# felipeagc/sycl-ray-tracer

Measured on AMD Instinct MI355X. Metric: Mrays/s, higher is better.
Workload: dtype f32

## Files before the change

### sycl-ray-tracer_amd/csrc/rt_abi.hip

```cpp
#include "bvh_quantise.h"
#include "rt_internal.h"

namespace rtlib {
thread_local std::string g_err;

int copy_out(const rt_renderer* r, int rc, float* rgba_f32, uint8_t* rgba_u8) {
    if (rc != RT_OK) return rc;
    if (rgba_f32 && r->n_local) HIPCHK(hipMemcpy(rgba_f32, r->d_f32, (size_t)r->n_local * 16, hipMemcpyDeviceToHost));
    if (rgba_u8 && r->n_local) HIPCHK(hipMemcpy(rgba_u8, r->d_u8, (size_t)r->n_local * 4, hipMemcpyDeviceToHost));
    return RT_OK;
}
}

extern "C" {

const char* rt_last_error(void) { return g_err.c_str(); }
int rt_abi_version(void) { return RT_ABI_VERSION; }

int rt_device_count(void) {
    int n = 0;
    hipError_t e = hipGetDeviceCount(&n);
    if (e != hipSuccess) return fail(RT_ERR_NO_DEVICE, std::string("hipGetDeviceCount: ") + hipGetErrorString(e));
    return n;
}

int rt_camera_init(rt_camera* out, int32_t width, int32_t height, const float center[3], const float dir_in[3],
                   float focal_length) {
    if (!out || !center || !dir_in || width <= 0 || height <= 0) return fail(RT_ERR_INVALID, "bad camera arguments");
    auto norm = [](const float v[3], float o[3]) {
        float inv = 1.0f / std::sqrt((v[0] * v[0] + v[1] * v[1]) + v[2] * v[2]);
        o[0] = v[0] * inv, o[1] = v[1] * inv, o[2] = v[2] * inv;
    };
    auto cross = [](const float a[3], const float b[3], float o[3]) {
        o[0] = a[1] * b[2] - a[2] * b[1], o[1] = a[2] * b[0] - a[0] * b[2], o[2] = a[0] * b[1] - a[1] * b[0];
    };
    float dir[3], right[3], up[3], tmp[3];
    const float world_up[3] = {0.0f, 1.0f, 0.0f};
    norm(dir_in, dir);
    cross(dir, world_up, tmp), norm(tmp, right);
    cross(right, dir, tmp), norm(tmp, up);
    const float vp0 = 1.0f * ((float)width / (float)height), vp1 = 1.0f;
    const float du_div = (float)width / (vp0 * 2.0f), dv_div = (float)height / (vp1 * 2.0f);
    for (int a = 0; a < 3; ++a) {
        const float viewport_u = (-right[a]) * vp0, viewport_v = up[a] * vp1;
        out->center[a] = center[a];
        out->pixel00[a] = ((center[a] + viewport_u) + viewport_v) + dir[a] * focal_length;
        out->delta_u[a] = right[a] / du_div;
        out->delta_v[a] = (-up[a]) / dv_div;
    }
    out->width = width, out->height = height;
    return RT_OK;
}

int rt_scene_create(const rt_scene_desc* desc, int device, int bvh_kind, rt_scene** out) { return rt_scene_create_ex(desc, device, bvh_kind, 0u, out); }

int rt_scene_create_ex(const rt_scene_desc* desc, int device, int bvh_kind, uint32_t flags, rt_scene** out) {
    if (!out) return fail(RT_ERR_INVALID, "null output pointer");
    *out = nullptr;
    if (flags & ~(RT_SCENE_UPDATABLE | RT_SCENE_KEEP_PREVIOUS)) return fail(RT_ERR_INVALID, "unknown scene flags");
    if ((flags & RT_SCENE_KEEP_PREVIOUS) && !(flags & RT_SCENE_UPDATABLE)) return fail(RT_ERR_INVALID, "RT_SCENE_KEEP_PREVIOUS is a flag of updatable scenes: pass RT_SCENE_UPDATABLE with it");
    if (bvh_kind != RT_BVH_DEFAULT && bvh_kind != RT_BVH_LBVH && bvh_kind != RT_BVH_SAH && bvh_kind != RT_BVH_LBVH_GPU)
        return fail(RT_ERR_INVALID, "unknown bvh_kind");
    if (bvh_kind == RT_BVH_LBVH_GPU) {
        if (device < 0) return fail(RT_ERR_NO_DEVICE, "RT_BVH_LBVH_GPU needs a device (device >= 0)");
        int rc0 = device_ok(device);
        if (rc0 != RT_OK) return rc0;
    }
    rt_scene* s = new (std::nothrow) rt_scene();
    if (!s) return fail(RT_ERR_OOM, "host allocation failed");
    std::string err;
    int rc = RT_OK;
    try {
        rc = build_host_scene(desc, bvh_kind, s->hs, err);
    } catch (const std::bad_alloc&) {
        delete s;
        return fail(RT_ERR_OOM, "host allocation failed while building the scene");
    } catch (const std::exception& e) {
        delete s;
        return fail(RT_ERR_INVALID, std::string("scene build failed: ") + e.what());
    }
    if (rc != RT_OK) {
        delete s;
        return fail(rc, err);
    }
    s->device = device;
    if (device >= 0) {
        rc = device_ok(device);
        if (rc == RT_OK) {
            if (s->hs.nodes.size() > (size_t)(0x7FFFFFFF / 64)) {
                rt_scene_destroy(s);
                return fail(RT_ERR_INVALID, "BVH too large for 32-bit node offsets");
            }
            std::vector<BvhNode> dn(s->hs.nodes);
            for (BvhNode& n : dn)
                for (int k = 0; k < 4; ++k)
                    if (n.child[k] >= 0) n.child[k] *= 64;
            rc = upload(dn, &s->dev.nodes, s->device_bytes);
        }
        if (rc == RT_OK) {
            std::vector<uint8_t> packed(s->hs.tris.size() * (size_t)kTriBytes + 48, 0);
            for (size_t i = 0; i < s->hs.tris.size(); ++i) std::memcpy(packed.data() + i * kTriBytes, &s->hs.tris[i], std::min<size_t>(kTriBytes, sizeof(TriRec)));
            rc = upload(packed, &s->dev.tris, s->device_bytes);
        }
        if (rc == RT_OK) rc = upload(s->hs.shade, &s->dev.shade, s->device_bytes);
        if (rc == RT_OK) {
            std::vector<InstRec> rows(s->hs.inst);
            if (flags & RT_SCENE_UPDATABLE) rows.resize(std::max<size_t>(rows.size(), desc->n_instances));
            rc = upload(rows, &s->dev.inst, s->device_bytes);
        }
        if (rc == RT_OK) rc = upload(s->hs.mats, &s->dev.mats, s->device_bytes);
        if (rc == RT_OK) rc = upload(s->hs.tex, &s->dev.tex, s->device_bytes);
        if (rc == RT_OK && hipMalloc((void**)&s->d_query_cursor, kQueryCursorBytes) != hipSuccess)
            rc = fail(RT_ERR_OOM, "device allocation failed (the ray-query cursors)");
        if (rc != RT_OK) {
            rt_scene_destroy(s);
            return rc;
        }
        s->dev.n_nodes = (uint32_t)s->hs.nodes.size();
        s->dev.n_tris = (uint32_t)(s->hs.wverts.size() / 9);
        std::memcpy(s->dev.sky, s->hs.sky, 12);
        s->dev.packed_mat = s->hs.packed_mat ? 1u : 0u;
        const bool stage = s->hs.packed_mat && s->hs.n_layers <= 65536u;
        s->dev.lds_nm = stage ? (uint32_t)std::min<size_t>(s->hs.inst.size(), kLdsNm) : 0u;
        s->dev.lds_mats = stage ? (uint32_t)std::min<size_t>(s->hs.mats.size(), kLdsMats) : 0u;
        scene_cells(s->hs, s->dev);
    }
    if (flags & RT_SCENE_UPDATABLE) {
        rc = no_throw([&] { return init_scene_update(s, desc, (flags & RT_SCENE_KEEP_PREVIOUS) != 0); });
        if (rc != RT_OK) {
            rt_scene_destroy(s);
            return rc;
        }
    }
    *out = s;
    return RT_OK;
}

void rt_scene_destroy(rt_scene* s) {
    if (!s) return;
    if (s->device >= 0 && hipSetDevice(s->device) == hipSuccess) {
        for (auto& se : s->ev_gbuffer) (void)hipEventSynchronize(se.second), (void)hipEventDestroy(se.second);
        (void)hipFree((void*)s->dev.nodes), (void)hipFree((void*)s->dev.tris), (void)hipFree((void*)s->dev.shade);
        (void)hipFree((void*)s->dev.inst), (void)hipFree((void*)s->dev.mats), (void)hipFree((void*)s->dev.tex);
        (void)hipFree((void*)s->d_query_cursor);
    }
    free_scene_update(s);
    delete s;
}

int rt_scene_info(const rt_scene* s, rt_scene_info_t* out) {
    if (!s || !out) return fail(RT_ERR_INVALID, "null argument");
    if (const int rc = sync_host_copy(s)) return rc;
    out->n_triangles = (uint32_t)(s->hs.wverts.size() / 9);
    out->n_nodes = (uint32_t)s->hs.nodes.size();
    out->max_depth = s->hs.max_depth;
    out->max_leaf_tris = s->hs.max_leaf_tris;
    std::memcpy(out->bounds_lo, s->hs.bounds_lo, 12), std::memcpy(out->bounds_hi, s->hs.bounds_hi, 12);
    out->sah_cost = s->hs.sah_cost;
    out->device_bytes = s->device_bytes;
    out->n_leaf_records = (uint32_t)s->hs.tris.size();
    out->n_split_triangles = s->hs.n_split_triangles;
    return RT_OK;
}

int rt_scene_check_bvh(const rt_scene* s) {
    if (!s) return fail(RT_ERR_INVALID, "null scene");
    if (const int rc0 = sync_host_copy(s)) return rc0;
    std::string err;
    int rc = check_bvh(s->hs, err);
    return rc == RT_OK ? RT_OK : fail(rc, err);
}

int rt_scene_count_visits(const rt_scene* s, uint32_t n, const float* org, const float* dir, int mode, uint64_t* node_visits, uint64_t* tri_tests,
                          float* t, uint32_t* tri) {
    if (!s || (n && (!org || !dir))) return fail(RT_ERR_INVALID, "null argument");
    if (const int rc0 = sync_host_copy(s)) return rc0;
    std::string err;
    const int rc = no_throw([&] { return count_visits(s->hs, n, org, dir, mode, node_visits, tri_tests, t, tri, err); });
    return rc == RT_OK ? RT_OK : fail(rc, err.empty() ? g_err : err);
}

int rt_renderer_create(int kind, rt_scene* scene, int32_t width, int32_t height, uint32_t max_depth,
                       uint32_t sample_count, uint32_t seed_mode, rt_renderer** out) {
    if (!out) return fail(RT_ERR_INVALID, "null output pointer");
    *out = nullptr;
    if (!scene) return fail(RT_ERR_INVALID, "null scene");
    if (kind != RT_RENDERER_MEGAKERNEL && kind != RT_RENDERER_WAVEFRONT) return fail(RT_ERR_INVALID, "unknown renderer kind");
    if (width <= 0 || height <= 0 || (int64_t)width * height > (int64_t)1 << 30) return fail(RT_ERR_INVALID, "bad image size");
    if (sample_count == 0) return fail(RT_ERR_INVALID, "sample_count must be >= 1");
    if (seed_mode > RT_SEED_MEGAKERNEL) return fail(RT_ERR_INVALID, "unknown seed mode");
    if ((uint64_t)sample_count * ((uint64_t)max_depth + 1) > (1ull << 26)) return fail(RT_ERR_INVALID, "sample_count * max_depth too large");
    if (scene->device < 0) return fail(RT_ERR_NO_DEVICE, "scene was built host-only (device < 0)");
    int rc = device_ok(scene->device);
    if (rc != RT_OK) return rc;
    rt_renderer* r = new (std::nothrow) rt_renderer();
    if (!r) return fail(RT_ERR_OOM, "host allocation failed");
    r->kind = kind, r->scene = scene, r->width = width, r->height = height;
    r->scene_gen = scene->generation;
    r->max_depth = max_depth, r->spp = sample_count;
    r->seed_mode = seed_mode != RT_SEED_DEFAULT ? seed_mode
                   : (kind == RT_RENDERER_MEGAKERNEL ? RT_SEED_MEGAKERNEL : RT_SEED_WAVEFRONT);
    r->hw_queues = hw_queues_from_env();
    const char* prof = std::getenv("RT_PROFILE_KERNELS");
    r->profile_kernels = prof && prof[0] == '1';
    if (const char* e = dev_knob("RT_MEGA_LDS_PAD")) r->mega_lds_pad = (uint32_t)std::max(0, std::min(100 * 1024, std::atoi(e)));
    if (const char* e = dev_knob("RT_MEGA_OCC")) r->mega_occ = (uint32_t)std::max(1, std::min((int)kMegaWaves, std::atoi(e)));
    auto bail = [&](int code) {
        rt_renderer_destroy(r);
        return code;
    };
    {
        hipStream_t s0 = nullptr;
        bool owned = false;
        if (lane_stream_of(scene->device, 0, &s0, &owned) != hipSuccess) return bail(fail(RT_ERR_HIP, "cannot create the stream-lane pool"));
    }
    hipDeviceProp_t prop;
    if (hipGetDeviceProperties(&prop, scene->device) == hipSuccess && prop.multiProcessorCount > 0) r->n_cus = prop.multiProcessorCount;
    if (hipStreamCreateWithFlags(&r->stream, hipStreamNonBlocking) != hipSuccess) return bail(fail(RT_ERR_HIP, "hipStreamCreate failed"));
    if (hipEventCreate(&r->ev_begin) != hipSuccess || hipEventCreate(&r->ev_end) != hipSuccess ||
        hipEventCreateWithFlags(&r->ev_fork, hipEventDisableTiming) != hipSuccess || hipEventCreateWithFlags(&r->ev_tile_read, hipEventDisableTiming) != hipSuccess)
        return bail(fail(RT_ERR_HIP, "hipEventCreate failed"));
    if (hipMalloc((void**)&r->d_frame, sizeof(MegaFrame)) != hipSuccess || hipHostMalloc((void**)&r->h_frame, sizeof(MegaFrame)) != hipSuccess)
        return bail(fail(RT_ERR_OOM, "frame constant buffer allocation failed"));
    if (kind == RT_RENDERER_WAVEFRONT) {
        if (hipMalloc((void**)&r->d_cam, sizeof(CameraDev)) != hipSuccess || hipHostMalloc((void**)&r->h_cam, sizeof(CameraDev)) != hipSuccess)
            return bail(fail(RT_ERR_OOM, "camera buffer allocation failed"));
        rt_schedule& sc = r->sched;
        if (const char* e = dev_knob("RT_WF_GRAPH")) sc.hip_graph = e[0] == '1';
        if (const char* e = dev_knob("RT_WF_FINISH_DEPTH")) sc.finish_depth = (uint32_t)std::max(0, std::atoi(e));
        if (const char* e = dev_knob("RT_WF_SAMPLES_PER_LAUNCH")) sc.samples_per_launch = (uint32_t)std::max(0, std::atoi(e));
        if (const char* e = dev_knob("RT_WF_REQUEUE")) sc.requeue = e[0] != '0' ? 1 : 0;
        if (const char* e = dev_knob("RT_WF_STREAMS")) sc.stream_lanes = (uint32_t)std::max(1, std::min(8, std::atoi(e)));
        if ((dev_knob("RT_WF_REQUEUE") || dev_knob("RT_WF_STREAMS")) && sc.samples_per_launch == 0) sc.samples_per_launch = 1;
        if (const char* e = dev_knob("RT_WF_LPT")) sc.cost_order = e[0] == '0' ? 0 : (e[0] == '2' ? 1 : -1);
        if (const char* e = dev_knob("RT_WF_EXTEND_OCC")) r->wf_extend_occ = (uint32_t)std::max(1, std::min((int)kExtendWaves, std::atoi(e)));
        if (const char* e = dev_knob("RT_WF_FINISH_OCC")) r->wf_finish_occ = (uint32_t)std::max(1, std::min((int)kMegaWaves, std::atoi(e)));
        if (const char* e = dev_knob("RT_WF_SHOOT_CHUNK")) r->wf_shoot_chunk = (uint32_t)std::max(16, std::min(1024, std::atoi(e)));
        if (const char* e = dev_knob("RT_WF_SHOOT_TAIL")) r->wf_shoot_tail = e[0] == '1';
        if (const char* e = dev_knob("RT_WF_SHOOT_STATIC_PCT")) r->wf_shoot_static_pct = (uint32_t)std::max(0, std::min(100, std::atoi(e)));
        if (const char* e = dev_knob("RT_WF_REORDER")) sc.reorder = e[0] == '1';
        if (const char* e = dev_knob("RT_WF_MATSORT")) sc.matsort = e[0] == '1';
        if (const char* e = dev_knob("RT_WF_FUSED_BOUNCE")) sc.fused_bounce = e[0] == '1';
    }
    rc = no_throw([&] { return alloc_tile_buffers(r); });
    if (rc != RT_OK) return bail(rc);
    *out = r;
    return RT_OK;
}

void rt_renderer_destroy(rt_renderer* r) {
    if (!r) return;
    if (r->scene && r->frame_pending && r->scene->frames_pending) r->scene->frames_pending--;
    if (r->scene && hipSetDevice(r->scene->device) == hipSuccess) {
        drain_streams(r, r->pending.stream);
        free_tile_buffers(r);
        if (r->d_cam) (void)hipFree(r->d_cam);
        if (r->h_cam) (void)hipHostFree(r->h_cam);
        if (r->d_frame) (void)hipFree(r->d_frame);
        if (r->h_frame) (void)hipHostFree(r->h_frame);
        for (hipEvent_t e : r->ev_pool) (void)hipEventDestroy(e);
        if (r->ev_begin) (void)hipEventDestroy(r->ev_begin);
        if (r->ev_end) (void)hipEventDestroy(r->ev_end);
        if (r->ev_fork) (void)hipEventDestroy(r->ev_fork);
        if (r->ev_tile_read) (void)hipEventDestroy(r->ev_tile_read);
        if (r->stream) (void)hipStreamDestroy(r->stream);
    }
    delete r;
}

int rt_renderer_set_tile(rt_renderer* r, uint32_t rank, uint32_t world, uint32_t strip_rows) {
    if (!r) return fail(RT_ERR_INVALID, "null renderer");
    if (world == 0 || rank >= world || strip_rows == 0) return fail(RT_ERR_INVALID, "bad tile split");
    if (r->frame_pending) return fail(RT_ERR_INVALID, "a frame is in flight (rt_render_frame_end first)");
    HIPCHK(hipSetDevice(r->scene->device));
    drain_streams(r, r->pending.stream);
    const TileDev old = r->tile;
    r->tile.rank = rank, r->tile.world = world, r->tile.strip_rows = strip_rows;
    const int rc = no_throw([&] { return alloc_tile_buffers(r); });
    if (rc != RT_OK) r->tile.rank = old.rank, r->tile.world = old.world, r->tile.strip_rows = old.strip_rows;
    return rc;
}

int32_t rt_renderer_local_rows(const rt_renderer* r) { return r ? r->tile.local_rows : 0; }

int32_t rt_renderer_global_row(const rt_renderer* r, int32_t local_row) {
    if (!r || local_row < 0 || local_row >= r->tile.local_rows) return -1;
    const uint32_t strip = (uint32_t)local_row / r->tile.strip_rows, within = (uint32_t)local_row % r->tile.strip_rows;
    return (int32_t)((strip * r->tile.world + r->tile.rank) * r->tile.strip_rows + within);
}

int rt_renderer_set_profiling(rt_renderer* r, int enable) {
    if (!r) return fail(RT_ERR_INVALID, "null renderer");
    r->profile_kernels = enable != 0;
    return RT_OK;
}

int rt_renderer_set_russian_roulette(rt_renderer* r, uint32_t start_bounce) {
// ... 35 lines not shown
    const rt_schedule old = r->sched;
    r->sched = *s;
    const int rc = no_throw([&] { return alloc_tile_buffers(r); });
    if (rc != RT_OK) r->sched = old;
    return rc;
}

int rt_render_frame(rt_renderer* r, const rt_camera* cam, float* rgba_f32, uint8_t* rgba_u8, rt_stats* stats) {
    if (!r) return fail(RT_ERR_INVALID, "null renderer");
    return copy_out(r, no_throw([&] { return render_impl(r, cam, rgba_f32 ? r->d_f32 : nullptr, rgba_u8 ? r->d_u8 : nullptr, r->stream, stats); }), rgba_f32, rgba_u8);
}

int rt_render_frame_device(rt_renderer* r, const rt_camera* cam, void* d_rgba_f32, void* d_rgba_u8, void* stream,
                           rt_stats* stats) {
    if (!r) return fail(RT_ERR_INVALID, "null renderer");
    return no_throw([&] { return render_impl(r, cam, (float*)d_rgba_f32, (uint8_t*)d_rgba_u8, stream ? (hipStream_t)stream : r->stream, stats); });
}

int rt_renderer_set_progressive(rt_renderer* r, int enable) {
    if (!r) return fail(RT_ERR_INVALID, "null renderer");
    if (r->frame_pending) return fail(RT_ERR_INVALID, "a frame is in flight (rt_render_frame_end first)");
    HIPCHK(hipSetDevice(r->scene->device));
    drop_graph(r);
    r->progressive = enable != 0;
    const int rc = no_throw([&] { return alloc_carry(r); });
    if (rc != RT_OK) r->progressive = false;
    return rc;
}

int rt_render_frame_continue(rt_renderer* r, uint32_t samples, float* rgba_f32, uint8_t* rgba_u8, rt_stats* stats) {
    if (!r) return fail(RT_ERR_INVALID, "null renderer");
    return copy_out(r, no_throw([&] { return continue_impl(r, samples, rgba_f32 ? r->d_f32 : nullptr, rgba_u8 ? r->d_u8 : nullptr, r->stream, stats); }), rgba_f32, rgba_u8);
}

int rt_render_frame_continue_device(rt_renderer* r, uint32_t samples, void* d_rgba_f32, void* d_rgba_u8, void* stream, rt_stats* stats) {
    if (!r) return fail(RT_ERR_INVALID, "null renderer");
    return no_throw([&] { return continue_impl(r, samples, (float*)d_rgba_f32, (uint8_t*)d_rgba_u8, stream ? (hipStream_t)stream : r->stream, stats); });
}

int rt_renderer_accumulated_samples(const rt_renderer* r, uint32_t* out) {
    if (!r || !out) return fail(RT_ERR_INVALID, "null argument");
    *out = carry_is_current(r) ? r->carry_samples : 0u;
    return RT_OK;
}

int rt_renderer_block_grid(const rt_renderer* r, uint32_t* blocks_x, uint32_t* blocks_y) {
    if (!r || !blocks_x || !blocks_y) return fail(RT_ERR_INVALID, "null argument");
    *blocks_x = ((uint32_t)r->width + 7u) / 8u, *blocks_y = ((uint32_t)r->tile.local_rows + 7u) / 8u;
    return RT_OK;
}

int rt_renderer_block_samples(const rt_renderer* r, uint32_t* out) {
    if (!r || !out) return fail(RT_ERR_INVALID, "null argument");
    const size_t nb = (size_t)(((uint32_t)r->width + 7u) / 8u) * (((uint32_t)r->tile.local_rows + 7u) / 8u);
    if (r->carry_samples == 0 || !carry_is_current(r) || r->h_block_count.size() != nb) std::memset(out, 0, nb * 4);
    else std::memcpy(out, r->h_block_count.data(), nb * 4);
    return RT_OK;
}

int rt_renderer_block_errors(const rt_renderer* r, float* out) {
    if (!r || !out) return fail(RT_ERR_INVALID, "null argument");
    return no_throw([&] { return block_errors(r, out); });
}

int rt_render_frame_continue_blocks(rt_renderer* r, uint32_t samples, const uint32_t* blocks, uint32_t n_blocks, float* rgba_f32, uint8_t* rgba_u8,
                                    rt_stats* stats) {
    if (!r) return fail(RT_ERR_INVALID, "null renderer");
    return copy_out(r, no_throw([&] { return continue_blocks_impl(r, samples, blocks, n_blocks, rgba_f32 ? r->d_f32 : nullptr, rgba_u8 ? r->d_u8 : nullptr, r->stream, stats); }), rgba_f32, rgba_u8);
}

int rt_render_frame_continue_blocks_device(rt_renderer* r, uint32_t samples, const uint32_t* blocks, uint32_t n_blocks, void* d_rgba_f32, void* d_rgba_u8,
                                           void* stream, rt_stats* stats) {
    if (!r) return fail(RT_ERR_INVALID, "null renderer");
    return no_throw([&] {
        return continue_blocks_impl(r, samples, blocks, n_blocks, (float*)d_rgba_f32, (uint8_t*)d_rgba_u8, stream ? (hipStream_t)stream : r->stream, stats);
    });
}

int rt_renderer_adapt(rt_renderer* r, float threshold, uint32_t min_samples, uint32_t* blocks_out, uint32_t* n_out) {
    if (!r || !n_out) return fail(RT_ERR_INVALID, "null argument");
    return no_throw([&]() -> int {
        std::vector<uint32_t> blocks;
        const int rc = adapt_impl(r, threshold, min_samples, blocks);
        if (rc != RT_OK) return rc;
        if (!blocks.empty() && !blocks_out) return fail(RT_ERR_INVALID, "null block list");
        if (!blocks.empty()) std::memcpy(blocks_out, blocks.data(), blocks.size() * 4);
        *n_out = (uint32_t)blocks.size();
        return (int)RT_OK;
    });
}

int rt_render_frame_continue_adaptive(rt_renderer* r, uint32_t samples, float threshold, uint32_t min_samples, float* rgba_f32, uint8_t* rgba_u8,
                                      rt_stats* stats, uint32_t* n_blocks_out) {
    if (!r) return fail(RT_ERR_INVALID, "null renderer");
    return copy_out(r, no_throw([&] {
        return continue_adaptive_impl(r, samples, threshold, min_samples, rgba_f32 ? r->d_f32 : nullptr, rgba_u8 ? r->d_u8 : nullptr, r->stream, stats,
                                      n_blocks_out);
    }), rgba_f32, rgba_u8);
}

int rt_render_frame_continue_adaptive_device(rt_renderer* r, uint32_t samples, float threshold, uint32_t min_samples, void* d_rgba_f32, void* d_rgba_u8,
                                             void* stream, rt_stats* stats, uint32_t* n_blocks_out) {
    if (!r) return fail(RT_ERR_INVALID, "null renderer");
    return no_throw([&] {
        return continue_adaptive_impl(r, samples, threshold, min_samples, (float*)d_rgba_f32, (uint8_t*)d_rgba_u8, stream ? (hipStream_t)stream : r->stream,
                                      stats, n_blocks_out);
    });
}

int rt_render_frame_begin(rt_renderer* r, const rt_camera* cam, void* d_rgba_f32, void* d_rgba_u8, void* stream) {
    if (!r) return fail(RT_ERR_INVALID, "null renderer");
    return no_throw([&] { return frame_begin(r, cam, (float*)d_rgba_f32, (uint8_t*)d_rgba_u8, stream ? (hipStream_t)stream : r->stream); });
}

int rt_render_frame_end(rt_renderer* r, rt_stats* stats) {
    if (!r) return fail(RT_ERR_INVALID, "null renderer");
    return no_throw([&] { return frame_end(r, stats); });
}

}

#ifdef RT_DEVELOPER_KNOBS
extern "C" {

int rt_dev_scene_tables(const rt_scene* s, uint32_t* packed_mat, uint32_t* lds_nm, uint32_t* lds_mats, uint32_t* n_rows, float* rows,
                        uint32_t capacity, uint32_t* words) {
    if (!s || !packed_mat || !lds_nm || !lds_mats || !n_rows) return fail(RT_ERR_INVALID, "null argument");
    if (const int rc = sync_host_copy(s)) return rc;
    *packed_mat = s->hs.packed_mat ? 1u : 0u;
    *lds_nm = s->dev.lds_nm, *lds_mats = s->dev.lds_mats;
    *n_rows = (uint32_t)s->hs.inst.size();
    if (rows)
        for (size_t k = 0; k < std::min<size_t>(capacity, s->hs.inst.size()); ++k) std::memcpy(rows + 9 * k, s->hs.inst[k].normal_mat, 36);
    if (words)
        for (size_t t = 0; t < s->hs.shade.size(); ++t) words[t] = s->hs.shade[t].instance;
    return RT_OK;
}

int rt_dev_scene_tree(const rt_scene* s, uint32_t* n_nodes, uint32_t* n_tris, uint32_t* n_wverts, uint32_t* stack_need, int32_t* built_by,
                      float* pad, float* bounds, void* nodes, uint32_t* global_index, float* wverts, uint32_t capacity) {
    if (!s || !n_nodes || !n_tris || !n_wverts || !stack_need || !built_by || !pad || !bounds) return fail(RT_ERR_INVALID, "null argument");
    if (const int rc = sync_host_copy(s)) return rc;
    const HostScene& hs = s->hs;
    *n_nodes = (uint32_t)hs.nodes.size(), *n_tris = (uint32_t)hs.tris.size(), *n_wverts = (uint32_t)hs.wverts.size();
    *stack_need = hs.stack_need, *built_by = hs.built_by, *pad = hs.pad;
    for (int a = 0; a < 3; ++a) bounds[a] = hs.bounds_lo[a], bounds[3 + a] = hs.bounds_hi[a];
    if (nodes) std::memcpy(nodes, hs.nodes.data(), std::min<size_t>(capacity, hs.nodes.size()) * sizeof(BvhNode));
    if (global_index)
        for (size_t t = 0; t < std::min<size_t>(capacity, hs.tris.size()); ++t) global_index[t] = hs.tris[t].global_index;
    if (wverts) std::memcpy(wverts, hs.wverts.data(), std::min<size_t>(capacity, hs.wverts.size()) * sizeof(float));
    return RT_OK;
}

int rt_dev_renderer_graph_captures(const rt_renderer* r, uint32_t* out) {
    if (!r || !out) return fail(RT_ERR_INVALID, "null argument");
    *out = r->graph_captures;
    return RT_OK;
}

int rt_dev_quantise_node(uint32_t count, const int32_t* nk, const float* klo, const float* khi, void* nodes_out, uint8_t* ok) {
    if (!nk || !klo || !khi || !nodes_out || !ok) return fail(RT_ERR_INVALID, "null argument");
    BvhNode* out = static_cast<BvhNode*>(nodes_out);
    for (uint32_t i = 0; i < count; ++i) {
        if (nk[i] < 1 || nk[i] > 4) return fail(RT_ERR_INVALID, "nk must be 1..4");
        Box3 kb[4];
        for (int k = 0; k < 4; ++k) std::memcpy(kb[k].lo, klo + 12 * (size_t)i + 3 * k, 12), std::memcpy(kb[k].hi, khi + 12 * (size_t)i + 3 * k, 12);
        out[i] = empty_node();
        ok[i] = quantise_node(out[i], nk[i], kb, 0.0f) ? 1 : 0;
    }
    return RT_OK;
}

}
#endif
```

### sycl-ray-tracer_amd/csrc/rt_bounce.h

```cpp
#pragma once
#include "rt_device.h"

namespace rt {

RT_DEV f3 ray_dir(const RayState& r) { return mk3(h2f(r.dir[0]), h2f(r.dir[1]), h2f(r.dir[2])); }

template <bool FROM_TRAV = false, class Sink = NoSink>
RT_DEV bool shade_bounce(const SceneDev& S, uint32_t& rng, RayState& r, const Hit& h, f3& result, const Trav* T = nullptr, const ShadeTables* tab = nullptr,
                         long long* ck = nullptr, const Sink& sink = Sink{}) {
    f3 org = FROM_TRAV ? T->o : r.org;
    f3 dir = FROM_TRAV ? T->d : ray_dir(r);
    f3 att = mk3(h2f(r.att[0]), h2f(r.att[1]), h2f(r.att[2]));
    f3 rad = mk3(h2f(r.rad[0]), h2f(r.rad[1]), h2f(r.rad[2]));
    const bool done = FROM_TRAV ? shade_hit<true>(S, *tab, rng, h, org, dir, att, rad, result, ck, sink) : shade_hit<false>(S, ShadeTables{}, rng, h, org, dir, att, rad, result, nullptr, sink);
    r.org = org;
    r.dir[0] = f2h(dir.x), r.dir[1] = f2h(dir.y), r.dir[2] = f2h(dir.z);
    r.att[0] = f2h(att.x), r.att[1] = f2h(att.y), r.att[2] = f2h(att.z);
    r.rad[0] = f2h(rad.x), r.rad[1] = f2h(rad.y), r.rad[2] = f2h(rad.z);
    return done;
}

RT_DEV bool roulette(uint32_t& rng, RayState& r) {
    const float qx = h2f(r.att[0]), qy = h2f(r.att[1]), qz = h2f(r.att[2]);
    const float p = __builtin_fminf(__builtin_fmaxf(__builtin_fmaxf(qx, __builtin_fmaxf(qy, qz)), 0.05f), 1.0f);
    const float u = rng_next(rng);
    if (!(u < p)) return false;
    r.att[0] = f2h(qx / p), r.att[1] = f2h(qy / p), r.att[2] = f2h(qz / p);
    return true;
}

}
```

### sycl-ray-tracer_amd/csrc/rt_device.h

```cpp
#pragma once
#include <hip/hip_runtime.h>

#include "../../include/rt_mi355x.h"
#include "rt_types.h"

namespace rt {

#define RT_DEV __device__ __forceinline__

struct f3 {
    float x, y, z;
};
RT_DEV f3 mk3(float x, float y, float z) { return f3{x, y, z}; }
RT_DEV f3 operator+(f3 a, f3 b) { return mk3(a.x + b.x, a.y + b.y, a.z + b.z); }
RT_DEV f3 operator-(f3 a, f3 b) { return mk3(a.x - b.x, a.y - b.y, a.z - b.z); }
RT_DEV f3 operator-(f3 a) { return mk3(-a.x, -a.y, -a.z); }
RT_DEV f3 operator*(f3 a, f3 b) { return mk3(a.x * b.x, a.y * b.y, a.z * b.z); }
RT_DEV f3 operator*(float s, f3 a) { return mk3(s * a.x, s * a.y, s * a.z); }
RT_DEV f3 operator*(f3 a, float s) { return mk3(a.x * s, a.y * s, a.z * s); }
RT_DEV float dot3(f3 a, f3 b) { return (a.x * b.x + a.y * b.y) + a.z * b.z; }
RT_DEV f3 cross3(f3 a, f3 b) {
    return mk3(a.y * b.z - a.z * b.y, a.z * b.x - a.x * b.z, a.x * b.y - a.y * b.x);
}
RT_DEV float rcp_rn(float x) {
// ... 16 lines not shown
        const float y = __builtin_amdgcn_rcpf(s);
        return __builtin_fmaf(__builtin_fmaf(-s, y, 1.0f), y, y);
    }
    return 1.0f / __builtin_sqrtf(x);
}
RT_DEV f3 normalize3(f3 a) {
    const float inv = inv_sqrt2(dot3(a, a));
    return mk3(a.x * inv, a.y * inv, a.z * inv);
}
RT_DEV float clamp01(float x) { return __builtin_fminf(__builtin_fmaxf(x, 0.0f), 1.0f); }

RT_DEV uint16_t f2h(float f) {
    asm("" : "+v"(f));
    _Float16 h = (_Float16)f;
    return __builtin_bit_cast(uint16_t, h);
}
RT_DEV float h2f(uint16_t b) { return (float)__builtin_bit_cast(_Float16, b); }

RT_DEV float rng_next(uint32_t& a) {
    uint32_t x = a;
    x ^= x << 13;
    x ^= x >> 17;
    x ^= x << 5;
    a = x;
    return (float)x * (1.0f / 4294967296.0f);
}
RT_DEV float rng_range(uint32_t& a, float mn, float mx) { return mn + (mx - mn) * rng_next(a); }
RT_DEV f3 rng_unit_vector(uint32_t& a) {
    float x = rng_range(a, -1.0f, 1.0f);
    float y = rng_range(a, -1.0f, 1.0f);
    float z = rng_range(a, -1.0f, 1.0f);
    return normalize3(mk3(x, y, z));
}

RT_DEV uint32_t pixel_seed(int x, int y, int w, int h, uint32_t seed_mode) {
    if (seed_mode == RT_SEED_MEGAKERNEL) {
        uint32_t h8 = (uint32_t)((h + 7) / 8) * 8u;
        return (uint32_t)x * h8 + (uint32_t)y;
    }
    return (uint32_t)x + (uint32_t)y * (uint32_t)w;
}

RT_DEV int tile_global_row(const TileDev& t, int local_row) {
    uint32_t strip = (uint32_t)local_row / t.strip_rows;
    uint32_t within = (uint32_t)local_row % t.strip_rows;
    return (int)((strip * t.world + t.rank) * t.strip_rows + within);
}

struct RayState {
    f3 org;
    uint16_t dir[3], att[3], rad[3];
};

RT_DEV RayState camera_ray(const CameraDev& c, int x, int y, uint32_t& rng) {
    f3 p00 = mk3(c.pixel00[0], c.pixel00[1], c.pixel00[2]);
    f3 du = mk3(c.du[0], c.du[1], c.du[2]);
    f3 dv = mk3(c.dv[0], c.dv[1], c.dv[2]);
    f3 center = mk3(c.center[0], c.center[1], c.center[2]);
    f3 pixel_center = (p00 + ((float)x * du)) + ((float)y * dv);
    float px = -0.5f + rng_next(rng);
    float py = -0.5f + rng_next(rng);
    f3 jitter = (px * du) + (py * dv);
    f3 pixel_sample = pixel_center + jitter;
    f3 d = pixel_sample - center;
    RayState r;
    r.org = center;
    r.dir[0] = f2h(d.x), r.dir[1] = f2h(d.y), r.dir[2] = f2h(d.z);
    r.att[0] = r.att[1] = r.att[2] = 0x3C00;
    r.rad[0] = r.rad[1] = r.rad[2] = 0;
    return r;
}

struct Hit {
    float t, u, v;
    uint32_t tri;
};

RT_DEV float dot3f(f3 a, f3 b) { return __builtin_fmaf(a.z, b.z, __builtin_fmaf(a.y, b.y, a.x * b.x)); }
RT_DEV f3 cross3f(f3 a, f3 b) {
    return mk3(__builtin_fmaf(a.y, b.z, -(a.z * b.y)), __builtin_fmaf(a.z, b.x, -(a.x * b.z)), __builtin_fmaf(a.x, b.y, -(a.y * b.x)));
}
RT_DEV void tri_test_regs(float4 a, float4 b, float2 c, f3 o, f3 d, Hit& best) {
    const f3 v0 = mk3(a.x, a.y, a.z), e1 = mk3(a.w, b.x, b.y), e2 = mk3(b.z, b.w, c.x);
    const uint32_t gidx = __float_as_uint(c.y);
    const f3 p = cross3f(d, e2);
    const float det = dot3f(e1, p);
    if (!(det != 0.0f)) return;
    const f3 tv = o - v0;
    const f3 q = cross3f(tv, e1);
    const float sgn = det < 0.0f ? -1.0f : 1.0f;
    const float un0 = dot3f(tv, p), vn0 = dot3f(d, q);
    const float un = un0 * sgn, vn = vn0 * sgn;
    if (!(un >= 0.0f && vn >= 0.0f && un + vn <= __builtin_fabsf(det))) return;
    const float inv = rcp_rn(det);
    const float t = dot3f(e2, q) * inv;
    if (!(t > kTNear)) return;
    if (t < best.t || (t == best.t && gidx < best.tri)) {
        best.t = t;
        best.u = un0 * inv;
        best.v = vn0 * inv;
        best.tri = gidx;
    }
}
typedef float f4a8 __attribute__((ext_vector_type(4), aligned(8)));
typedef float f2a8 __attribute__((ext_vector_type(2), aligned(8)));
RT_DEV float4 tri_ld4(const uint8_t* p) {
    const f4a8 v = *reinterpret_cast<const f4a8*>(p);
    return make_float4(v.x, v.y, v.z, v.w);
}
RT_DEV float2 tri_ld2(const uint8_t* p) {
    const f2a8 v = *reinterpret_cast<const f2a8*>(p);
    return make_float2(v.x, v.y);
}
RT_DEV void tri_test(const uint8_t* __restrict__ tr, f3 o, f3 d, Hit& best) {
    tri_test_regs(tri_ld4(tr), tri_ld4(tr + 16), tri_ld2(tr + 32), o, d, best);
}

constexpr int32_t kTravDone = (int32_t)0x80000000;
struct Trav {
    f3 o, d;
    float ix, iy, iz;
    float ox, oy, oz;
    Hit best;
    int32_t cur;
    uint32_t sp;
};

struct TravStack;
RT_DEV uint32_t stack_base(const TravStack& st);
RT_DEV void trav_begin(Trav& T, f3 o, f3 d, const TravStack& st) {
    T.o = o, T.d = d;
    T.best.t = __builtin_huge_valf();
    T.best.u = T.best.v = 0.0f;
    T.best.tri = kNoTri;
    const float kTiny = 1e-30f;
    const float dx = __builtin_fabsf(d.x) < kTiny ? __builtin_copysignf(kTiny, d.x) : d.x;
    const float dy = __builtin_fabsf(d.y) < kTiny ? __builtin_copysignf(kTiny, d.y) : d.y;
    const float dz = __builtin_fabsf(d.z) < kTiny ? __builtin_copysignf(kTiny, d.z) : d.z;
    T.ix = __builtin_amdgcn_rcpf(dx), T.iy = __builtin_amdgcn_rcpf(dy), T.iz = __builtin_amdgcn_rcpf(dz);
    T.ox = -o.x * T.ix, T.oy = -o.y * T.iy, T.oz = -o.z * T.iz;
    T.cur = 0;
    T.sp = stack_base(st);
}

constexpr int kLdsStack = 12;
typedef __attribute__((address_space(3))) int32_t lds_i32;
struct TravStack {
    uint32_t base;
    int32_t* spill;
    uint32_t pitch;
};
RT_DEV uint32_t stack_base(const TravStack& st) { return st.base + st.pitch; }
RT_DEV lds_i32* lds_at(uint32_t addr) { return (lds_i32*)(size_t)addr; }
RT_DEV bool stack_shallow(const TravStack& st, const Trav& T, uint32_t pushes) { return T.sp <= st.base + ((uint32_t)kLdsStack - pushes) * st.pitch; }
RT_DEV void trav_pop_lds(Trav& T, const TravStack& st) {
    T.sp -= st.pitch;
    T.cur = *lds_at(T.sp);
}
RT_DEV void stk_push(const TravStack& st, Trav& T, int32_t v) {
    const uint32_t e = (T.sp - st.base) / st.pitch;
    if (e < (uint32_t)kLdsStack) *lds_at(T.sp) = v;
    else st.spill[e - (uint32_t)kLdsStack] = v;
    T.sp += st.pitch;
}
RT_DEV void trav_pop(Trav& T, const TravStack& st) {
    T.sp -= st.pitch;
    const uint32_t e = (T.sp - st.base) / st.pitch;
    T.cur = e < (uint32_t)kLdsStack ? *lds_at(T.sp) : st.spill[e - (uint32_t)kLdsStack];
}

typedef uint32_t u32x4 __attribute__((ext_vector_type(4)));
typedef uint32_t u32x2 __attribute__((ext_vector_type(2)));
typedef __attribute__((address_space(3))) u32x4 lds_u32x4;
struct TopTree {
    lds_u32x4* w0;
    lds_u32x4* w1;
    lds_u32x4* w2;
    lds_u32x4* ch;
    int32_t count;
};
RT_DEV void top_tree_fill(const SceneDev& S, u32x4* w0, u32x4* w1, u32x4* w2, u32x4* ch, int32_t count) {
    for (int32_t i = (int32_t)threadIdx.x; i < count; i += (int32_t)blockDim.x) {
        const u32x4* np = reinterpret_cast<const u32x4*>(S.nodes + i);
        w0[i] = np[0];
        w1[i] = np[1];
        w2[i] = np[2];
        ch[i] = np[3];
    }
}

typedef unsigned long long lmask;
RT_DEV lmask lanes(bool c) { return __builtin_amdgcn_ballot_w64(c); }
RT_DEV uint32_t lane_rank(lmask m) { return __builtin_amdgcn_mbcnt_hi((uint32_t)(m >> 32), __builtin_amdgcn_mbcnt_lo((uint32_t)m, 0u)); }
RT_DEV float sel(lmask m, float a, float b) {
    float d;
    asm("v_cndmask_b32_e64 %0, %1, %2, %3" : "=v"(d) : "v"(a), "v"(b), "s"(m));
    return d;
}
RT_DEV uint32_t sel(lmask m, uint32_t a, uint32_t b) {
    uint32_t d;
    asm("v_cndmask_b32_e64 %0, %1, %2, %3" : "=v"(d) : "v"(a), "v"(b), "s"(m));
    return d;
}
RT_DEV int32_t sel(lmask m, int32_t a, int32_t b) { return (int32_t)sel(m, (uint32_t)a, (uint32_t)b); }

struct TravSigns {
    lmask nx, ny, nz;
};

RT_DEV float ub0(uint32_t w) { return (float)(w & 0xffu); }
RT_DEV float ub1(uint32_t w) { return (float)((w >> 8) & 0xffu); }
RT_DEV float ub2(uint32_t w) { return (float)((w >> 16) & 0xffu); }
RT_DEV float ub3(uint32_t w) { return (float)(w >> 24); }

struct WaveStats {
    uint32_t inner_steps = 0, inner_lanes = 0, leaf_steps = 0, leaf_lanes = 0;
    uint32_t shade_rounds = 0, shade_lanes = 0, live_lane_steps = 0, top_lanes = 0;
};
RT_DEV TravSigns trav_signs(const Trav& T) { return TravSigns{lanes(T.ix < 0.0f), lanes(T.iy < 0.0f), lanes(T.iz < 0.0f)}; }
RT_DEV void trav_inner(const SceneDev& S, Trav& T, const TravStack& stack, const TopTree& top, const TravSigns& sg) {
    const float inf = __builtin_huge_valf();
    float k0, k1, k2, k3;
    u32x4 w0, w1, w2, chw;
    if (T.cur < top.count * 64) {
        const uint32_t o = (uint32_t)T.cur >> 2;
        w0 = *(lds_u32x4*)(size_t)((uint32_t)(size_t)top.w0 + o), w1 = *(lds_u32x4*)(size_t)((uint32_t)(size_t)top.w1 + o);
        w2 = *(lds_u32x4*)(size_t)((uint32_t)(size_t)top.w2 + o), chw = *(lds_u32x4*)(size_t)((uint32_t)(size_t)top.ch + o);
    } else {
        asm volatile("global_load_dwordx4 %0, %4, %5\n\t"
                     "global_load_dwordx4 %1, %4, %5 offset:16\n\t"
                     "global_load_dwordx4 %2, %4, %5 offset:32\n\t"
                     "global_load_dwordx4 %3, %4, %5 offset:48"
                     : "=&v"(w0), "=&v"(w1), "=&v"(w2), "=&v"(chw)
                     : "v"((uint32_t)T.cur), "s"(S.nodes)
                     : "memory");
    }
    asm volatile("s_waitcnt vmcnt(1)" : "+v"(w0), "+v"(w1), "+v"(w2));
    const float ax = __uint_as_float(w0.w) * T.ix;
    const float ay = __uint_as_float(w2.z) * T.iy;
    const float az = __uint_as_float(w2.w) * T.iz;
    const float bx = __builtin_fmaf(__uint_as_float(w0.x), T.ix, T.ox);
    const float by = __builtin_fmaf(__uint_as_float(w0.y), T.iy, T.oy);
    const float bz = __builtin_fmaf(__uint_as_float(w0.z), T.iz, T.oz);
    const lmask nx = sg.nx, ny = sg.ny, nz = sg.nz;
    const uint32_t qnx = sel(nx, w1.x, w1.y), qfx = sel(nx, w1.y, w1.x);
    const uint32_t qny = sel(ny, w1.z, w1.w), qfy = sel(ny, w1.w, w1.z);
    const uint32_t qnz = sel(nz, w2.x, w2.y), qfz = sel(nz, w2.y, w2.x);
#define RT_CHILD(K, CVT)                                                                                  \
    {                                                                                                    \
        const float tn = __builtin_fmaxf(__builtin_fmaxf(__builtin_fmaf(CVT(qnx), ax, bx), __builtin_fmaf(CVT(qny), ay, by)), \
                                         __builtin_fmaxf(__builtin_fmaf(CVT(qnz), az, bz), 0.0f));       \
        const float tf = __builtin_fminf(__builtin_fminf(__builtin_fmaf(CVT(qfx), ax, bx), __builtin_fmaf(CVT(qfy), ay, by)), \
                                         __builtin_fminf(__builtin_fmaf(CVT(qfz), az, bz), T.best.t));   \
        K = sel(lanes(tn <= tf), inf, tn);                                                               \
    }
    RT_CHILD(k0, ub0)
    RT_CHILD(k1, ub1)
    RT_CHILD(k2, ub2)
    RT_CHILD(k3, ub3)
#undef RT_CHILD
#define RT_CE(KA, CA, KB, CB)                                                        \
    {                                                                               \
        const lmask sw = lanes(KB < KA);                                            \
        const float ka = sel(sw, KA, KB), kb = sel(sw, KB, KA);                     \
        const int32_t ca = sel(sw, CA, CB), cb = sel(sw, CB, CA);                   \
        KA = ka, KB = kb, CA = ca, CB = cb;                                         \
    }
    asm volatile("s_waitcnt vmcnt(0)" : "+v"(chw));
    int32_t c0 = (int32_t)chw.x, c1 = (int32_t)chw.y, c2 = (int32_t)chw.z, c3 = (int32_t)chw.w;
    RT_CE(k0, c0, k1, c1)
    RT_CE(k2, c2, k3, c3)
    RT_CE(k0, c0, k2, c2)
#undef RT_CE
    const bool descend = k0 < inf;
    if (lanes(!stack_shallow(stack, T, 3u)) == 0ull) {
        *lds_at(T.sp) = c3;
        T.sp = sel(lanes(k3 < inf), T.sp, T.sp + stack.pitch);
        *lds_at(T.sp) = c2;
        T.sp = sel(lanes(k2 < inf), T.sp, T.sp + stack.pitch);
        *lds_at(T.sp) = c1;
        T.sp = sel(lanes(k1 < inf), T.sp, T.sp + stack.pitch);
        if (descend) T.cur = c0;
        else trav_pop_lds(T, stack);
    } else {
        if (k3 < inf) stk_push(stack, T, c3);
        if (k2 < inf) stk_push(stack, T, c2);
        if (k1 < inf) stk_push(stack, T, c1);
        if (descend) T.cur = c0;
        else trav_pop(T, stack);
    }
}

template <bool BATCH>
RT_DEV void trav_leaf(const SceneDev& S, Trav& T, const TravStack& stack) {
    const uint32_t code = (uint32_t)~T.cur;
    const uint32_t first = code >> 2, rem = code & 3u;
    if (BATCH) {
        static_assert(kMaxLeafTris == 2 && kTriBytes == 40, "the whole-leaf step reads a leaf as 80 contiguous bytes");
        const uint8_t* p4 = S.tris + (size_t)first * kTriBytes;
        const float4 l0 = tri_ld4(p4), l1 = tri_ld4(p4 + 16), l2 = tri_ld4(p4 + 32), l3 = tri_ld4(p4 + 48), l4 = tri_ld4(p4 + 64);
        const bool two = rem != 0u;
        tri_test_regs(l0, l1, make_float2(l2.x, l2.y), T.o, T.d, T.best);
        if (__ballot(two) != 0ull) {
            if (two) tri_test_regs(make_float4(l2.z, l2.w, l3.x, l3.y), make_float4(l3.z, l3.w, l4.x, l4.y), make_float2(l4.z, l4.w), T.o, T.d, T.best);
        }
        if (lanes(!stack_shallow(stack, T, 0u)) == 0ull) trav_pop_lds(T, stack);
        else trav_pop(T, stack);
    } else {
        tri_test(S.tris + (size_t)first * kTriBytes, T.o, T.d, T.best);
        if (rem) T.cur = ~(int32_t)(((first + 1u) << 2) | (rem - 1u));
        else trav_pop(T, stack);
    }
}

template <bool STATS = false, bool LEAF_BATCH = false>
RT_DEV uint32_t trav_step_wave(const SceneDev& S, Trav& T, const TravStack& stack, const TopTree& top, const TravSigns& sg, WaveStats* ws = nullptr) {
    const bool inner = T.cur >= 0;
    const bool leaf = T.cur < 0 && T.cur != kTravDone;
    const uint32_t ni = (uint32_t)__popcll(__ballot(inner)), nl = (uint32_t)__popcll(__ballot(leaf));
    if (ni * 3u >= nl * 4u && !(LEAF_BATCH && nl >= 64u)) {
        if (STATS && ni) ws->inner_steps++, ws->inner_lanes += ni, ws->top_lanes += (uint32_t)__popcll(__ballot(inner && T.cur < kTopNodes * 64));
        if (inner) trav_inner(S, T, stack, top, sg);
    } else {
        if (STATS) ws->leaf_steps++, ws->leaf_lanes += (uint32_t)__popcll(__ballot(leaf));
        if (leaf) trav_leaf<LEAF_BATCH>(S, T, stack);
    }
    return ni + nl;
}

RT_DEV Hit intersect(const SceneDev& S, f3 o, f3 d, const TravStack& stack, const TopTree& top) {
    Trav T;
    trav_begin(T, o, d, stack);
    const TravSigns sg = trav_signs(T);
    while (trav_step_wave(S, T, stack, top, sg)) {}
    return T.best;
}

RT_DEV bool near_zero3(f3 e) {
    const float s = 1e-8f;
    return (__builtin_fabsf(e.x) < s) && (__builtin_fabsf(e.y) < s) && (__builtin_fabsf(e.z) < s);
}
RT_DEV float length_squared3(f3 v) {
    float l = __builtin_sqrtf(dot3(v, v));
    return l * l;
}
RT_DEV f3 reflect3(f3 v, f3 n) { return v - (2.0f * dot3(v, n)) * n; }
RT_DEV f3 refract3(f3 uv, f3 n, float etai_over_etat) {
    float cos_theta = __builtin_fminf(dot3(-uv, n), 1.0f);
    f3 r_out_perp = etai_over_etat * (uv + cos_theta * n);
    f3 r_out_parallel = (-__builtin_sqrtf(__builtin_fabsf(1.0f - length_squared3(r_out_perp)))) * n;
    return r_out_perp + r_out_parallel;
}
RT_DEV float schlick(float cosine, float ref_idx) {
    float r0 = (1.0f - ref_idx) / (1.0f + ref_idx);
    r0 = r0 * r0;
    float x = 1.0f - cosine;
    float x2 = x * x;
    float x5 = (x2 * x2) * x;
    return r0 + (1.0f - r0) * x5;
}
RT_DEV float unorm8_to_float(uint32_t b) {
    const float x = (float)b, r = 1.0f / 255.0f;
    const float q = x * r;
    return __builtin_fmaf(__builtin_fmaf(-q, 255.0f, x), r, q);
}

RT_DEV bool albedo_is_texture(const MatRec& m) { return (m.type == RT_MAT_DIFFUSE || m.type == RT_MAT_METALLIC) && m.tex_kind != RT_TEX_COLOR; }
RT_DEV uint32_t albedo_fetch(const SceneDev& S, const MatRec& m, float u, float v) {
    float fu = u - __builtin_floorf(u);
    float fv = v - __builtin_floorf(v);
    int iu = (int)__builtin_floorf(fu * 512.0f);
    int iv = (int)__builtin_floorf(fv * 512.0f);
    iu = iu < 0 ? 0 : (iu > 511 ? 511 : iu);
    iv = iv < 0 ? 0 : (iv > 511 ? 511 : iv);
    return *reinterpret_cast<const uint32_t*>(S.tex + (((size_t)m.tex_layer * 512u + (size_t)iv) * 512u + (size_t)iu) * 4u);
}
RT_DEV f3 albedo_decode(uint32_t texel) {
    return mk3(unorm8_to_float(texel & 0xffu), unorm8_to_float((texel >> 8) & 0xffu), unorm8_to_float((texel >> 16) & 0xffu));
}
RT_DEV f3 albedo(const SceneDev& S, const MatRec& m, float u, float v) {
    if (m.tex_kind == RT_TEX_COLOR) return mk3(m.color[0], m.color[1], m.color[2]);
    float fu = u - __builtin_floorf(u);
    float fv = v - __builtin_floorf(v);
    int iu = (int)__builtin_floorf(fu * 512.0f);
    int iv = (int)__builtin_floorf(fv * 512.0f);
    iu = iu < 0 ? 0 : (iu > 511 ? 511 : iu);
    iv = iv < 0 ? 0 : (iv > 511 ? 511 : iv);
    const uint32_t texel = *reinterpret_cast<const uint32_t*>(
        S.tex + (((size_t)m.tex_layer * 512u + (size_t)iv) * 512u + (size_t)iu) * 4u);
    return mk3(unorm8_to_float(texel & 0xffu), unorm8_to_float((texel >> 8) & 0xffu), unorm8_to_float((texel >> 16) & 0xffu));
}

template <bool PRE = false>
RT_DEV bool scatter(const SceneDev& S, const MatRec& m, uint32_t& rng, f3 dir, f3 normal, float u, float v,
                    f3& out_dir, f3& out_att, uint32_t texel = 0) {
    if (m.type == RT_MAT_DIFFUSE || m.type == RT_MAT_METALLIC) {
        const bool diffuse = m.type == RT_MAT_DIFFUSE;
        const f3 unit = rng_unit_vector(rng);
        const f3 reflected = reflect3(dir, normal);
        const f3 base = diffuse ? normal : reflected;
        const f3 offs = diffuse ? unit : m.roughness * unit;
        out_dir = base + offs;
        if (diffuse && near_zero3(dir)) out_dir = normal;
        if (PRE) out_att = m.tex_kind == RT_TEX_COLOR ? mk3(m.color[0], m.color[1], m.color[2]) : albedo_decode(texel);
        else out_att = albedo(S, m, u, v);
        return diffuse ? true : dot3(out_dir, normal) > 0.0f;
    }
    if (m.type == RT_MAT_DIELECTRIC) {
        out_att = mk3(1.0f, 1.0f, 1.0f);
        bool front_face = dot3(dir, normal) < 0.0f;
        f3 n = front_face ? normal : -normal;
        float ratio = front_face ? (1.0f / m.ior) : m.ior;
        f3 unit_direction = normalize3(dir);
        float cos_theta = __builtin_fminf(dot3(-unit_direction, n), 1.0f);
        float sin_theta = __builtin_sqrtf(1.0f - cos_theta * cos_theta);
        bool reflect_it = ratio * sin_theta > 1.0f;
        if (!reflect_it) reflect_it = schlick(cos_theta, ratio) > rng_range(rng, 0.0f, 1.0f);
        out_dir = reflect_it ? reflect3(unit_direction, n) : refract3(unit_direction, n, ratio);
        return true;
    }
    out_dir = mk3(0.0f, 0.0f, 0.0f);
    out_att = mk3(0.0f, 0.0f, 0.0f);
    return false;
}

struct ShadeTables {
    lds_u32x4* nm;
    lds_u32x4* mat;
    uint32_t n_nm, n_mat;
};
RT_DEV void shade_tables_fill(const SceneDev& S, u32x4* nm, u32x4* mat) {
    const u32x4* in = reinterpret_cast<const u32x4*>(S.inst);
    for (uint32_t i = threadIdx.x; i < S.lds_nm * 3u; i += blockDim.x) nm[i] = in[i];
    for (uint32_t i = threadIdx.x; i < S.lds_mats; i += blockDim.x) {
        const u32x4* mp = reinterpret_cast<const u32x4*>(S.mats + i);
        const u32x4 m0 = mp[0], m1 = mp[1], m2 = mp[2];
        u32x4 a, b;
        a.x = m0.x | (m0.y << 8) | (m1.y << 16), a.y = m0.z, a.z = m0.w, a.w = m1.x;
        b.x = m1.z, b.y = m1.w, b.z = m2.x, b.w = m0.x == RT_MAT_DIELECTRIC ? m2.z : m2.y;
        mat[2u * i] = a, mat[2u * i + 1u] = b;
    }
}

#ifdef RT_ROUND_STAMPS
#define RT_STAMP_AFTER(ck, i, VAL)                                                     \
    do {                                                                              \
        if (ck) {                                                                     \
            asm volatile("" ::"v"(VAL));                                              \
            const long long n_ = (long long)__builtin_readcyclecounter();             \
            (ck)[i] += n_ - (ck)[7];                                                  \
            (ck)[7] = n_;                                                             \
        }                                                                             \
    } while (0)
#else
#define RT_STAMP_AFTER(ck, i, VAL) do { } while (0)
#endif
struct NoSink {};
template <class Sink> struct is_no_sink { static constexpr bool value = false; };
template <> struct is_no_sink<NoSink> { static constexpr bool value = true; };
template <bool USE_TAB = false, class Sink = NoSink>
RT_DEV bool shade_hit(const SceneDev& S, const ShadeTables& tab, uint32_t& rng, const Hit& h, f3& org, f3& dir, f3& att, f3& rad, f3& result,
                      long long* ck = nullptr, const Sink& sink = Sink{}) {
    if (h.tri == kNoTri) {
        if constexpr (is_no_sink<Sink>::value) result = att * (mk3(S.sky[0], S.sky[1], S.sky[2]) + rad);
        else sink(att * (mk3(S.sky[0], S.sky[1], S.sky[2]) + rad));
        return true;
    }
    const float4* sp = reinterpret_cast<const float4*>(S.shade + h.tri);
    const float4 s0 = sp[0], s1 = sp[1], s2 = sp[2], s3 = sp[3];
    const f3 d = normalize3(dir);
    const f3 n0 = mk3(s0.x, s0.y, s0.z), n1 = mk3(s0.w, s1.x, s1.y), n2 = mk3(s1.z, s1.w, s2.x);
    const float uv0x = s2.y, uv0y = s2.z, uv1x = s2.w, uv1y = s3.x, uv2x = s3.y, uv2y = s3.z;
    const uint32_t iw = __float_as_uint(s3.w);
    RT_STAMP_AFTER(ck, 1, iw);
    bool lds = false;
    if (USE_TAB) lds = __builtin_amdgcn_ballot_w64(!((iw & kPackedInstMask) < tab.n_nm && (iw >> kPackedInstBits) < tab.n_mat)) == 0ull;
    MatRec mat;
    if (USE_TAB && __builtin_expect(lds, 1)) {
        const uint32_t at = (iw >> kPackedInstBits) * 2u;
        const u32x4 a = tab.mat[at], b = tab.mat[at + 1u];
        mat.type = a.x & 0xffu, mat.tex_kind = (a.x >> 8) & 0xffu, mat.tex_layer = a.x >> 16;
        mat.color[0] = __uint_as_float(a.y), mat.color[1] = __uint_as_float(a.z), mat.color[2] = __uint_as_float(a.w);
        mat.emissive[0] = __uint_as_float(b.x), mat.emissive[1] = __uint_as_float(b.y), mat.emissive[2] = __uint_as_float(b.z);
        mat.roughness = mat.ior = __uint_as_float(b.w);
    } else {
        const InstRec* inst = S.inst + (S.packed_mat ? (iw & kPackedInstMask) : iw);
        const u32x4* mp = reinterpret_cast<const u32x4*>(S.mats + (S.packed_mat ? (iw >> kPackedInstBits) : inst->material));
        const u32x4 m0 = mp[0], m1 = mp[1], m2 = mp[2];
        mat.type = m0.x, mat.tex_kind = m0.y, mat.color[0] = __uint_as_float(m0.z), mat.color[1] = __uint_as_float(m0.w);
        mat.color[2] = __uint_as_float(m1.x), mat.tex_layer = m1.y, mat.emissive[0] = __uint_as_float(m1.z), mat.emissive[1] = __uint_as_float(m1.w);
        mat.emissive[2] = __uint_as_float(m2.x), mat.roughness = __uint_as_float(m2.y), mat.ior = __uint_as_float(m2.z);
    }
    const float bx = h.u, by = h.v;
    const float w = (1.0f - bx) - by;
    const float tu = (w * uv0x + bx * uv1x) + by * uv2x;
    const float tv = (w * uv0y + bx * uv1y) + by * uv2y;
    uint32_t texel;
    {
        float fu = tu - __builtin_floorf(tu);
        float fv = tv - __builtin_floorf(tv);
        int iu = (int)__builtin_floorf(fu * 512.0f);
        int iv = (int)__builtin_floorf(fv * 512.0f);
        iu = iu < 0 ? 0 : (iu > 511 ? 511 : iu);
        iv = iv < 0 ? 0 : (iv > 511 ? 511 : iv);
        const uint8_t* ta = S.tex + (((size_t)mat.tex_layer * 512u + (size_t)iv) * 512u + (size_t)iu) * 4u;
        if (!albedo_is_texture(mat)) ta = reinterpret_cast<const uint8_t*>(sp);
        texel = *reinterpret_cast<const uint32_t*>(ta);
        RT_STAMP_AFTER(ck, 2, ta);
    }
    const bool emits = mat.type == RT_MAT_DIFFUSE || mat.type == RT_MAT_METALLIC;
    rad = rad + (emits ? mk3(mat.emissive[0], mat.emissive[1], mat.emissive[2]) : mk3(0.0f, 0.0f, 0.0f));
    const f3 vn = normalize3((w * n0 + bx * n1) + by * n2);
    float nm[9];
    if (USE_TAB && __builtin_expect(lds, 1)) {
        const uint32_t at = (iw & kPackedInstMask) * 3u;
        const u32x4 a = tab.nm[at], b = tab.nm[at + 1u];
        const uint32_t c = *reinterpret_cast<__attribute__((address_space(3))) const uint32_t*>(tab.nm + at + 2u);
        nm[0] = __uint_as_float(a.x), nm[1] = __uint_as_float(a.y), nm[2] = __uint_as_float(a.z), nm[3] = __uint_as_float(a.w);
        nm[4] = __uint_as_float(b.x), nm[5] = __uint_as_float(b.y), nm[6] = __uint_as_float(b.z), nm[7] = __uint_as_float(b.w);
        nm[8] = __uint_as_float(c);
    } else {
        const InstRec* inst = S.inst + (S.packed_mat ? (iw & kPackedInstMask) : iw);
        u32x4 a, b;
        uint32_t c;
        asm volatile("global_load_dwordx4 %0, %3, off\n\t"
                     "global_load_dwordx4 %1, %3, off offset:16\n\t"
                     "global_load_dword %2, %3, off offset:32\n\t"
                     "s_waitcnt vmcnt(0)"
                     : "=&v"(a), "=&v"(b), "=&v"(c)
                     : "v"(inst)
                     : "memory");
        nm[0] = __uint_as_float(a.x), nm[1] = __uint_as_float(a.y), nm[2] = __uint_as_float(a.z), nm[3] = __uint_as_float(a.w);
        nm[4] = __uint_as_float(b.x), nm[5] = __uint_as_float(b.y), nm[6] = __uint_as_float(b.z), nm[7] = __uint_as_float(b.w);
        nm[8] = __uint_as_float(c);
    }
    const f3 g = mk3((nm[0] * vn.x + nm[3] * vn.y) + nm[6] * vn.z, (nm[1] * vn.x + nm[4] * vn.y) + nm[7] * vn.z,
                     (nm[2] * vn.x + nm[5] * vn.y) + nm[8] * vn.z);
    const f3 normal = normalize3(g);
    RT_STAMP_AFTER(ck, 3, normal.x);
    f3 sdir, satt;
#ifdef RT_SCATTER_PRIO
    __builtin_amdgcn_s_setprio(RT_SCATTER_PRIO);
#endif
    const bool scattered = scatter<true>(S, mat, rng, d, normal, tu, tv, sdir, satt, texel);
    RT_STAMP_AFTER(ck, 4, satt.x);
    if (scattered) {
        org = mk3(org.x + dir.x * h.t, org.y + dir.y * h.t, org.z + dir.z * h.t);
        dir = sdir;
        att = att * satt;
        return false;
    }
    if constexpr (is_no_sink<Sink>::value) result = att * rad;
    else sink(att * rad);
    return true;
}

RT_DEV uint8_t to_unorm8(float c) { return (uint8_t)__builtin_rintf(clamp01(c) * 255.0f); }

#define RT_TRAVERSAL_LDS(BLOCK)                                                                        \
    __shared__ u32x4 top_all[4 * kTopNodes];  \
    u32x4 *const top_w0 = top_all, *const top_w1 = top_all + kTopNodes, *const top_w2 = top_all + 2 * kTopNodes, *const top_ch = top_all + 3 * kTopNodes; \
    __shared__ int32_t lds_stack[kLdsStack * (BLOCK)];                                                 \
    int32_t spill[kStackSize - kLdsStack];                                                             \
    const int32_t top_count = (int32_t)S.n_nodes < kTopNodes ? (int32_t)S.n_nodes : kTopNodes;         \
    top_tree_fill(S, top_w0, top_w1, top_w2, top_ch, top_count);                                       \
    __syncthreads();                                                                                   \
    const TopTree top{(lds_u32x4*)top_w0, (lds_u32x4*)top_w1, (lds_u32x4*)top_w2, (lds_u32x4*)top_ch, top_count}; \
    const TravStack stack{(uint32_t)(size_t)(lds_i32*)(lds_stack + threadIdx.x), spill, 4u * (BLOCK)}; \
    lds_stack[threadIdx.x] = kTravDone;

#define RT_SHADE_LDS                                                                                   \
    __shared__ u32x4 shade_nm[3 * kLdsNm], shade_mat[2 * kLdsMats];                                    \
    shade_tables_fill(S, shade_nm, shade_mat);                                                         \
    const ShadeTables tab{(lds_u32x4*)shade_nm, (lds_u32x4*)shade_mat, S.lds_nm, S.lds_mats};


}
```

### sycl-ray-tracer_amd/csrc/rt_kernels.h

```cpp
#pragma once
#include <cstddef>

#include "rt_bounce.h"
#include "rt_device.h"
#include "rt_launch.h"

namespace rt {

RT_DEV void queue_store(const QueueDev& q, uint32_t slot, uint32_t id, const RayState& r) {
    q.org_id[slot] = make_float4(r.org.x, r.org.y, r.org.z, __uint_as_float(id));
    q.a[slot] = make_uint2((uint32_t)r.dir[0] | ((uint32_t)r.dir[1] << 16), (uint32_t)r.dir[2] | ((uint32_t)r.att[0] << 16));
    q.b[slot] = make_uint2((uint32_t)r.att[1] | ((uint32_t)r.att[2] << 16), (uint32_t)r.rad[0] | ((uint32_t)r.rad[1] << 16));
    q.c[slot] = r.rad[2];
}
RT_DEV uint32_t queue_load(const QueueDev& q, uint32_t slot, RayState& r) {
    const float4 o = q.org_id[slot];
    const uint2 a = q.a[slot], b = q.b[slot];
    const uint16_t c = q.c[slot];
    r.org = mk3(o.x, o.y, o.z);
    r.dir[0] = (uint16_t)a.x, r.dir[1] = (uint16_t)(a.x >> 16), r.dir[2] = (uint16_t)a.y;
    r.att[0] = (uint16_t)(a.y >> 16), r.att[1] = (uint16_t)b.x, r.att[2] = (uint16_t)(b.x >> 16);
    r.rad[0] = (uint16_t)b.y, r.rad[1] = (uint16_t)(b.y >> 16), r.rad[2] = c;
    return __float_as_uint(o.w);
}
// ... 29 lines not shown
#endif
constexpr int kMegaUnroll = 3;
#ifndef RT_MEGA_SHADE_PCT
#define RT_MEGA_SHADE_PCT 75
#endif
constexpr uint32_t kMegaShadePct = RT_MEGA_SHADE_PCT;
constexpr uint32_t kMegaRefill = 1;
struct RefillPolicy {
    uint32_t w = (kMegaRefill - 1u) << 28;
    RT_DEV uint32_t threshold() const { return (w >> 28) + 1u; }
    RT_DEV void stepped() {
        if (((w >> 17) & 0x7FFu) != 0x7FFu) w += 1u << 17;
    }
    RT_DEV void round(bool finished) {
        w += ((uint32_t)__popcll(__ballot(finished)) << 5) + 1u;
        if ((w & 31u) == 0u) {
            const uint32_t ended = ((w >> 5) & 0xFFFu) - 1u, steps = ((w >> 17) & 0x7FFu) * kMegaUnroll;
            const uint32_t num = 320u * ended, den = 160u + steps;
            const uint32_t t = num < 4u * den ? 1u : num < 9u * den ? 2u : num < 16u * den ? 3u : num < 25u * den ? 4u : num < 36u * den ? 5u
                               : num < 64u * den ? 6u : num < 100u * den ? 8u : num < 144u * den ? 10u : num < 256u * den ? 12u : 16u;
            w = (t - 1u) << 28;
        }
    }
};
template <uint32_t OFF> RT_DEV uint32_t frame_u32(const MegaFrame* f) {
    uint32_t v;
    asm volatile("s_load_dword %0, %1, %2\n\t"
                 "s_waitcnt lgkmcnt(0)"
                 : "=&s"(v)
                 : "s"(f), "i"(OFF));
    return v;
}
template <uint32_t OFF> RT_DEV unsigned long long frame_u64(const MegaFrame* f) {
    unsigned long long v;
    asm volatile("s_load_dwordx2 %0, %1, %2\n\t"
                 "s_waitcnt lgkmcnt(0)"
                 : "=&s"(v)
                 : "s"(f), "i"(OFF));
    return v;
}
RT_DEV CameraDev frame_camera(const MegaFrame* f, int32_t width, int32_t height) {
    static_assert(offsetof(MegaFrame, cam) == 0 && offsetof(CameraDev, dv) + sizeof(CameraDev::dv) == 48, "the camera's twelve floats lead MegaFrame");
    u32x4 a, b, c;
    asm volatile("s_load_dwordx4 %0, %3, 0x0\n\t"
                 "s_load_dwordx4 %1, %3, 0x10\n\t"
                 "s_load_dwordx4 %2, %3, 0x20\n\t"
                 "s_waitcnt lgkmcnt(0)"
                 : "=&s"(a), "=&s"(b), "=&s"(c)
                 : "s"(f));
    CameraDev cam;
    cam.center[0] = __uint_as_float(a.x), cam.center[1] = __uint_as_float(a.y), cam.center[2] = __uint_as_float(a.z);
    cam.pixel00[0] = __uint_as_float(a.w), cam.pixel00[1] = __uint_as_float(b.x), cam.pixel00[2] = __uint_as_float(b.y);
    cam.du[0] = __uint_as_float(b.z), cam.du[1] = __uint_as_float(b.w), cam.du[2] = __uint_as_float(c.x);
    cam.dv[0] = __uint_as_float(c.y), cam.dv[1] = __uint_as_float(c.z), cam.dv[2] = __uint_as_float(c.w);
    cam.width = width, cam.height = height;
    return cam;
}
RT_DEV CameraDev frame_camera_and_seed(const MegaFrame* f, int32_t width, int32_t height, uint32_t& seed_add) {
    u32x4 a, b, c;
    uint32_t s;
    asm volatile("s_load_dwordx4 %0, %4, 0x0\n\t"
                 "s_load_dwordx4 %1, %4, 0x10\n\t"
                 "s_load_dwordx4 %2, %4, 0x20\n\t"
                 "s_load_dword %3, %4, %5\n\t"
                 "s_waitcnt lgkmcnt(0)"
                 : "=&s"(a), "=&s"(b), "=&s"(c), "=&s"(s)
                 : "s"(f), "i"((uint32_t)offsetof(MegaFrame, seed_add)));
    CameraDev cam;
    cam.center[0] = __uint_as_float(a.x), cam.center[1] = __uint_as_float(a.y), cam.center[2] = __uint_as_float(a.z);
    cam.pixel00[0] = __uint_as_float(a.w), cam.pixel00[1] = __uint_as_float(b.x), cam.pixel00[2] = __uint_as_float(b.y);
    cam.du[0] = __uint_as_float(b.z), cam.du[1] = __uint_as_float(b.w), cam.du[2] = __uint_as_float(c.x);
    cam.dv[0] = __uint_as_float(c.y), cam.dv[1] = __uint_as_float(c.z), cam.dv[2] = __uint_as_float(c.w);
    cam.width = width, cam.height = height;
    seed_add = s;
    return cam;
}
struct SliceNow {
    u32x4 head;
    u32x2 cuts;
};
RT_DEV SliceNow frame_slices(const MegaFrame* f) {
    static_assert(offsetof(SliceDev, tag0) == offsetof(SliceDev, state) + 8 && offsetof(SliceDev, shift) == offsetof(SliceDev, state) + 12, "SliceNow::head");
    SliceNow n;
    asm volatile("s_load_dwordx4 %0, %2, %3\n\t"
                 "s_load_dwordx2 %1, %2, %4\n\t"
                 "s_waitcnt lgkmcnt(0)"
                 : "=&s"(n.head), "=&s"(n.cuts)
                 : "s"(f), "i"((uint32_t)offsetof(MegaFrame, sl.state)), "i"((uint32_t)offsetof(MegaFrame, sl.cuts)));
    return n;
}
RT_DEV uint32_t frame_slice_bound(const MegaFrame* f, uint32_t j) {
    uint32_t v;
    const uint32_t at = (uint32_t)__builtin_amdgcn_readfirstlane((int)((uint32_t)offsetof(MegaFrame, sl.bound) + 4u * j));
    asm volatile("s_load_dword %0, %1, %2\n\t"
                 "s_waitcnt lgkmcnt(0)"
                 : "=&s"(v)
                 : "s"(f), "s"(at));
    return v;
}
RT_DEV u32x4* frame_carry(const MegaFrame* f) { return (u32x4*)frame_u64<offsetof(MegaFrame, carry)>(f); }
RT_DEV uint32_t frame_carry_total(const MegaFrame* f) { return frame_u32<offsetof(MegaFrame, carry_total)>(f); }
RT_DEV uint32_t frame_n_blocks(const MegaFrame* f) { return frame_u32<offsetof(MegaFrame, n_blocks)>(f); }
RT_DEV const uint32_t* frame_blocks(const MegaFrame* f) { return (const uint32_t*)frame_u64<offsetof(MegaFrame, blocks)>(f); }
RT_DEV const uint32_t* frame_block_count(const MegaFrame* f) { return (const uint32_t*)frame_u64<offsetof(MegaFrame, block_count)>(f); }
RT_DEV uint32_t frame_slice_wait_cap(const MegaFrame* f) { return frame_u32<offsetof(MegaFrame, sl.wait_cap)>(f); }
RT_DEV u32x4 carry_word(float r, float g, float b, uint32_t rng) {
    u32x4 w;
    w.x = __float_as_uint(r), w.y = __float_as_uint(g), w.z = __float_as_uint(b), w.w = rng;
    return w;
}
typedef __attribute__((address_space(3))) uint32_t lds_u32_word;
RT_DEV bool slice_wait_count(lds_u32_word* looks, const MegaFrame* f) {
    __builtin_amdgcn_s_sleep(127);
    const uint32_t n = *looks + 1u;
    *looks = n;
    return n == frame_slice_wait_cap(f) + 1u;
}
RT_DEV bool slice_wait_over(const lds_u32_word* looks, const MegaFrame* f) { return *looks > frame_slice_wait_cap(f); }
RT_DEV lds_u32_word* slice_looks_word(const void __attribute__((address_space(3))) * lane_slot, const void __attribute__((address_space(3))) * planes) {
    uint32_t a = (uint32_t)(size_t)lane_slot;
    asm volatile("" : "+v"(a));
    const uint32_t base = (uint32_t)(size_t)planes;
    return (lds_u32_word*)(size_t)(base + 3u * kMegaBlock * 4u + (((a - base) >> 6) & ~3u));
}
template <int STATS, bool SLICED, int CARRY = 0>
__global__ void __launch_bounds__(kMegaBlock, kMegaWaves) k_megakernel(SceneDev S, const MegaFrame* frame, int32_t width, int32_t height, TileDev tile,
                                                    uint32_t max_depth, uint32_t spp, uint32_t seed_mode, uint32_t rr_start, float* __restrict__ out_f32,
                                                    uint8_t* __restrict__ out_u8,
                                                    unsigned long long* __restrict__ ray_counter,
                                                    unsigned long long* __restrict__ stats_out, uint32_t n_slices) {
    WaveStats ws;
    long long t_begin = 0, t_mark = 0, t_trav = 0, t_shade = 0;
    long long ck[8] = {0, 0, 0, 0, 0, 0, 0, 0};
    if (STATS) t_begin = t_mark = (long long)__builtin_readcyclecounter();
    unsigned long long wall_begin = 0, wall_exhausted = 0;
    if (STATS >= 2) wall_begin = wall_clock64();
    const uint32_t tiles_x = (uint32_t)(width + 7) >> 3, tiles_y = (uint32_t)(tile.local_rows + 7) >> 3;
    const uint32_t n_slots = (CARRY == 3 ? frame_n_blocks(frame) : tiles_x * tiles_y) * 64u;
    const int lane = (int)(threadIdx.x & 63u);
    uint32_t* pixel_cursor = reinterpret_cast<uint32_t*>(ray_counter + 1);
    int x = 0, gy = 0;
    uint32_t pix = 0;
    uint32_t rng = 0, s = 0, depth = 0;
    unsigned long long wave_rays = 0;
    __shared__ float color_lds[3 * kMegaBlock + (SLICED ? kMegaBlock / 64 : 0)];
    typedef __attribute__((address_space(3))) float lds_f32;
    lds_f32* const color_r = (lds_f32*)color_lds + threadIdx.x;
    lds_f32* const color_g = color_r + kMegaBlock;
    lds_f32* const color_b = color_g + kMegaBlock;
    RayState r{};
    Trav T;
    if (SLICED) *slice_looks_word(color_r, (lds_f32*)color_lds) = 0u;
    RT_SHADE_LDS
    RT_TRAVERSAL_LDS(kMegaBlock)
    T.cur = kTravDone;
    constexpr uint32_t kPend = 0x40000000u;
    bool live = false;
    RefillPolicy refill;
    bool exhausted = false;
    uint32_t slice_j = 0;
    auto state_rsrc = [&](const SliceNow& n) {
        return __builtin_amdgcn_make_buffer_rsrc((void*)(((unsigned long long)n.head.y << 32) | n.head.x), 0, (int)((uint32_t)tile.local_rows * (uint32_t)width * 32u), 0x00020000);
    };
    auto take_slot = [&](uint32_t p, uint32_t first) {
        uint32_t t = p >> 6;
        if constexpr (CARRY == 3) t = frame_blocks(frame)[t];
        x = (int)((t % tiles_x) * 8u + (p & 7u));
        const int ly = (int)((t / tiles_x) * 8u + ((p >> 3) & 7u));
        gy = tile_global_row(tile, ly);
        pix = (uint32_t)ly * (uint32_t)width + (uint32_t)x;
        if (x < width && ly < tile.local_rows && gy < height) {
            s = first;
            if (!SLICED || first == 0) {
                depth = 0;
                if constexpr (CARRY >= 2) {
                    const u32x4 c = frame_carry(frame)[pix];
                    rng = c.w;
                    *color_r = __uint_as_float(c.x), *color_g = __uint_as_float(c.y), *color_b = __uint_as_float(c.z);
                    r = camera_ray(frame_camera(frame, width, height), x, gy, rng);
                } else {
                    uint32_t seed_add;
                    const CameraDev cam = frame_camera_and_seed(frame, width, height, seed_add);
                    rng = pixel_seed(x, gy, width, height, seed_mode) + seed_add;
                    *color_r = 0.0f, *color_g = 0.0f, *color_b = 0.0f;
                    r = camera_ray(cam, x, gy, rng);
                }
                trav_begin(T, r.org, ray_dir(r), stack);
            } else {
                depth = kPend;
            }
            live = true;
        }
    };
    {
        const uint32_t n_waves = gridDim.x * (kMegaBlock / 64u);
        if (n_slots <= n_waves * 64u && n_slices == 1u) {
            const uint32_t p = (uint32_t)lane * n_waves + blockIdx.x * (kMegaBlock / 64u) + (threadIdx.x >> 6);
            if (p < n_slots) take_slot(p, 0u);
            exhausted = true;
            if (STATS >= 2) wall_exhausted = wall_clock64();
        }
    }
    for (;;) {
        if (!exhausted) {
            const unsigned long long idle_m = __ballot(!live);
            const uint32_t cnt = (uint32_t)__popcll(idle_m);
            if (cnt >= refill.threshold()) {
                const uint32_t w = SLICED ? SliceCursor::claim_width(cnt, n_slots) : cnt;
                uint32_t base = 0;
                if (lane == 0) base = atomicAdd(pixel_cursor, w);
                base = (uint32_t)__builtin_amdgcn_readfirstlane((int)base);
                uint32_t first_here = 0, first_next = 0;
                if (SLICED) {
                    slice_j = SliceCursor::advance(slice_j, n_slices, base, n_slots);
                    if (slice_j) first_here = frame_slice_bound(frame, slice_j - 1u);
                    first_next = frame_slice_bound(frame, slice_j);
                }
                const uint32_t total_slots = SLICED ? n_slots * n_slices : n_slots;
                const uint32_t rank = __builtin_amdgcn_mbcnt_hi((uint32_t)(idle_m >> 32), __builtin_amdgcn_mbcnt_lo((uint32_t)idle_m, 0u));
                const uint32_t q = base + rank;
                if (!live && q < total_slots && rank < w) {
                    const SliceSlot m = SLICED ? SliceCursor::map(q, slice_j, n_slots, first_here, first_next) : SliceSlot{q, 0u};
                    take_slot(m.slot, m.first);
                }
                if (base + w >= total_slots) {
                    exhausted = true;
                    if (STATS >= 2) wall_exhausted = wall_clock64();
                }
            }
        }
        const uint32_t n_live = (uint32_t)__popcll(__ballot(live));
        if (n_live == 0) {
            if (exhausted) break;
            continue;
        }
        if (STATS) t_mark = (long long)__builtin_readcyclecounter();
        const TravSigns sg = trav_signs(T);
        const uint32_t n_rays = SLICED ? (uint32_t)__popcll(__ballot(live && depth < kPend)) : n_live;
        const uint32_t shade_at = n_rays * kMegaShadePct + (n_live - n_rays) * 100u;
        for (;;) {
            const bool waiting = live && T.cur == kTravDone;
            if ((uint32_t)__popcll(__ballot(waiting)) * 100u >= shade_at) break;
            if (STATS >= 2) ws.live_lane_steps += n_live;
            if (STATS == 1) ws.inner_steps += (uint32_t)kMegaUnroll;
            refill.stepped();
            (void)trav_step_wave<(STATS >= 2), true>(S, T, stack, top, sg, &ws);
#pragma unroll
            for (int k = 1; k < kMegaUnroll; ++k) {
                if (STATS >= 2) ws.live_lane_steps += n_live;
                (void)trav_step_wave<(STATS >= 2), true>(S, T, stack, top, sg, &ws);
            }
        }
        if (STATS) {
            ws.shade_rounds++;
            if (STATS >= 2) ws.shade_lanes += (uint32_t)__popcll(__ballot(live && T.cur == kTravDone));
            const long long now = (long long)__builtin_readcyclecounter();
            t_trav += now - t_mark, t_mark = now;
        }
        __builtin_amdgcn_s_setprio(RT_ROUND_PRIO);
#ifdef RT_ROUND_STAMPS
        if (STATS >= 2) ck[7] = (long long)__builtin_readcyclecounter();
#endif
        bool pixel_finished = false;
        {
            const unsigned long long traced = __ballot(live && T.cur == kTravDone && depth < kPend);
            wave_rays += (unsigned long long)__popcll(traced);
            if (SLICED && traced == 0ull && __ballot(live && depth < kPend) == 0ull && slice_wait_count(slice_looks_word(color_r, (lds_f32*)color_lds), frame) && lane == 0) atomicMax(ray_counter + 2, 1ull);
        }
        if (live && T.cur == kTravDone) {
            bool start = false;
            if (SLICED && depth >= kPend) {
                const SliceNow sn = frame_slices(frame);
                const auto rsrc = state_rsrc(sn);
                const uint32_t at = pix * 32u, tag = sn.head.z + s;
                const u32x4 w0 = __builtin_amdgcn_raw_buffer_load_b128(rsrc, (int)at, 0, 16 );
                const u32x4 w1 = __builtin_amdgcn_raw_buffer_load_b128(rsrc, (int)(at + 16u), 0, 16 );
                if ((w0.y == tag && w0.w == tag && w1.y == tag && w1.w == tag) || slice_wait_over(slice_looks_word(color_r, (lds_f32*)color_lds), frame)) {
                    *color_r = __uint_as_float(w0.x), *color_g = __uint_as_float(w0.z), *color_b = __uint_as_float(w1.x);
                    rng = w1.z;
                    start = true;
                }
            } else {
                f3 res;
                const auto add = [color_r, color_g, color_b](const f3& c) { *color_r = *color_r + c.x, *color_g = *color_g + c.y, *color_b = *color_b + c.z; };
                bool done;
                if (SLICED) {
                    done = shade_bounce<true>(S, rng, r, T.best, res, &T, &tab, STATS >= 2 ? ck : nullptr, add);
                } else {
                    done = shade_bounce<true>(S, rng, r, T.best, res, &T, &tab, STATS >= 2 ? ck : nullptr);
                    if (done) add(res);
                }
#ifdef RT_TAIL_PRIO
                __builtin_amdgcn_s_setprio(RT_TAIL_PRIO);
#endif
                depth++;
                bool killed = false;
                if (rr_start && !done && depth >= rr_start && depth < max_depth) killed = !roulette(rng, r);
                if (done || killed || depth == max_depth) {
                    s++;
                    bool handed = false;
                    SliceNow sn{};
                    if (SLICED) {
                        sn = frame_slices(frame);
                        const unsigned long long cuts = ((unsigned long long)sn.cuts.y << 32) | sn.cuts.x;
                        const uint32_t sh = sn.head.w;
                        handed = s < spp && (s & ((1u << sh) - 1u)) == 0u && ((cuts >> (s >> sh)) & 1ull) != 0ull;
                    }
                    if (SLICED && handed) {
                        live = false, pixel_finished = true;
                        const auto rsrc = state_rsrc(sn);
                        const uint32_t at = pix * 32u, tag = sn.head.z + s;
                        u32x4 w0, w1;
                        w0.x = __float_as_uint(*color_r), w0.y = tag, w0.z = __float_as_uint(*color_g), w0.w = tag;
                        w1.x = __float_as_uint(*color_b), w1.y = tag, w1.z = rng, w1.w = tag;
                        __builtin_amdgcn_raw_buffer_store_b128(w0, rsrc, (int)at, 0, 16 );
                        __builtin_amdgcn_raw_buffer_store_b128(w1, rsrc, (int)(at + 16u), 0, 16 );
                    } else if (s < spp) {
                        start = true;
                    } else {
                        live = false, pixel_finished = true;
                        float n;
                        if constexpr (CARRY == 3)
                            n = (float)frame_block_count(frame)[(pix / (uint32_t)width >> 3) * tiles_x + ((uint32_t)x >> 3)];
                        else
                            n = (float)(CARRY == 2 ? frame_carry_total(frame) : spp);
                        pixel_end(color_r, color_g, color_b, n, pix, out_f32, out_u8);
                        if constexpr (CARRY != 0) frame_carry(frame)[pix] = carry_word(*color_r, *color_g, *color_b, rng);
                    }
                }
            }
            if (start) {
                depth = 0;
                int cx = x, cy = gy;
                asm volatile("" : "+v"(cx), "+v"(cy));
                r = camera_ray(frame_camera(frame, width, height), cx, cy, rng);
            }
            if (live && depth < kPend) trav_begin(T, r.org, ray_dir(r), stack);
            RT_STAMP_AFTER((STATS >= 2 ? ck : nullptr), 5, T.ox);
        }
        refill.round(pixel_finished);
        if (STATS) t_shade += (long long)__builtin_readcyclecounter() - t_mark;
        __builtin_amdgcn_s_setprio(2);
    }
    if (lane == 0 && wave_rays) atomicAdd(ray_counter, wave_rays);
    if (STATS && lane == 0) {
        wave_stats_flush(ws, stats_out);
        const unsigned long long dur = (unsigned long long)((long long)__builtin_readcyclecounter() - t_begin);
        atomicAdd(stats_out + 8, dur), atomicMax(stats_out + 9, dur), atomicAdd(stats_out + 10, 1ull);
        atomicAdd(stats_out + 11, (unsigned long long)t_trav), atomicAdd(stats_out + 12, (unsigned long long)t_shade);
        if (STATS >= 2) {
            atomicMin(stats_out + 13, wall_begin);
            if (wall_exhausted) atomicMin(stats_out + 14, wall_exhausted);
            atomicMax(stats_out + 15, (unsigned long long)wall_clock64());
        }
#ifdef RT_ROUND_STAMPS
        for (int i = 1; i <= 5; ++i) atomicAdd(stats_out + 15 + i, (unsigned long long)ck[i]);
#endif
    }
}

__global__ void __launch_bounds__(256) k_fill_black(uint32_t n_local, float* __restrict__ out_f32, uint8_t* __restrict__ out_u8) {
    const uint32_t i = blockIdx.x * 256u + threadIdx.x;
    if (i >= n_local) return;
    if (out_f32) reinterpret_cast<float4*>(out_f32)[i] = make_float4(0.0f, 0.0f, 0.0f, 1.0f);
    if (out_u8) reinterpret_cast<uint32_t*>(out_u8)[i] = 0xff000000u;
}

__global__ void __launch_bounds__(256) k_wf_init(const CameraDev* __restrict__ camp, TileDev tile, uint32_t seed_mode, uint32_t seed_add, uint32_t n_local,
                                                  uint32_t* __restrict__ rng, float4* __restrict__ accum) {
    const uint32_t i = blockIdx.x * 256u + threadIdx.x;
    if (i >= n_local) return;
    const CameraDev cam = *camp;
    const int x = (int)(i % (uint32_t)cam.width), ly = (int)(i / (uint32_t)cam.width);
    const int gy = tile_global_row(tile, ly);
    rng[i] = pixel_seed(x, gy, cam.width, cam.height, seed_mode) + seed_add;
    accum[i] = make_float4(0.0f, 0.0f, 0.0f, 0.0f);
}
__global__ void __launch_bounds__(256) k_wf_init_carry(uint32_t n_local, uint32_t width, uint32_t strip_rows, uint32_t n_lanes, uint32_t lane_index,
                                                        const u32x4* __restrict__ carry, uint32_t* __restrict__ rng, float4* __restrict__ accum) {
    const uint32_t i = blockIdx.x * 256u + threadIdx.x;
    if (i >= n_local) return;
    const uint32_t x = i % width, row = stream_lane_row(i / width, strip_rows, n_lanes, lane_index);
    const u32x4 c = carry[(size_t)row * width + x];
    rng[i] = c.w;
    accum[i] = make_float4(__uint_as_float(c.x), __uint_as_float(c.y), __uint_as_float(c.z), 0.0f);
}

__global__ void __launch_bounds__(256) k_wf_generate(const CameraDev* __restrict__ camp, TileDev tile, uint32_t n_local,
                                                      uint32_t* __restrict__ rng, QueueDev q,
                                                      uint32_t* __restrict__ count_out, uint32_t spread, const uint32_t* __restrict__ tile_order) {
    const uint32_t i = blockIdx.x * 256u + threadIdx.x;
    if (i == 0) *count_out = n_local;
    if (i >= n_local) return;
    const CameraDev cam = *camp;
    const uint32_t nw = n_local >> 6;
    uint32_t id = spread && nw * 64u == n_local ? (i & 63u) * nw + (i >> 6) : i;
    if (tile_order) {
        const uint32_t t = tile_order[i >> 6], w = i & 63u, tiles_x = (uint32_t)cam.width >> 3;
        id = ((t / tiles_x) * 8u + (w >> 3)) * (uint32_t)cam.width + (t % tiles_x) * 8u + (w & 7u);
    }
    const int x = (int)(id % (uint32_t)cam.width), ly = (int)(id / (uint32_t)cam.width);
    const int gy = tile_global_row(tile, ly);
    uint32_t st = rng[id];
    const RayState r = gy < cam.height ? camera_ray(cam, x, gy, st) : RayState{};
    rng[id] = st;
    queue_store(q, i, id, r);
}

__global__ void __launch_bounds__(64) k_wf_tile_cost(const uint8_t* __restrict__ cost, uint32_t width, uint32_t n_tiles, uint32_t* __restrict__ key) {
    const uint32_t t = blockIdx.x, w = threadIdx.x, tiles_x = width >> 3;
    if (t >= n_tiles) return;
    uint32_t v = cost[((t / tiles_x) * 8u + (w >> 3)) * width + (t % tiles_x) * 8u + (w & 7u)];
#pragma unroll
    for (int off = 32; off > 0; off >>= 1) v += __shfl_down(v, off, 64);
    if (w == 0) key[t] = v >> 2;
}
constexpr uint32_t kOrderBins = 64u * 255u / 4u + 1u;
__global__ void __launch_bounds__(1024) k_wf_order_tiles(const uint32_t* __restrict__ key, uint32_t n_tiles, uint32_t* __restrict__ order) {
    __shared__ uint32_t bin[kOrderBins];
    for (uint32_t i = threadIdx.x; i < kOrderBins; i += 1024u) bin[i] = 0;
    __syncthreads();
    for (uint32_t t = threadIdx.x; t < n_tiles; t += 1024u) atomicAdd(&bin[key[t] < kOrderBins ? key[t] : kOrderBins - 1u], 1u);
    __syncthreads();
    if (threadIdx.x == 0) {
        uint32_t run = 0;
        for (uint32_t k = kOrderBins; k-- > 0;) {
            const uint32_t c = bin[k];
            bin[k] = run;
            run += c;
        }
    }
    __syncthreads();
    for (uint32_t t = threadIdx.x; t < n_tiles; t += 1024u) order[atomicAdd(&bin[key[t] < kOrderBins ? key[t] : kOrderBins - 1u], 1u)] = t;
}


constexpr uint32_t kExtendRefill = 16;
template <bool STATS>
__global__ void __launch_bounds__(kExtendBlock, kExtendWaves) k_wf_extend(SceneDev S, QueueDev qin, float4* __restrict__ hits,
                                                                    const uint32_t* __restrict__ count_in,
                                                                    uint32_t* __restrict__ cursor,
                                                                    unsigned long long* __restrict__ stats_out) {
    WaveStats ws;
    const uint32_t n = *count_in;
    const uint32_t lane = threadIdx.x & 63u;
    constexpr uint32_t kWavesPerBlock = kExtendBlock / 64;
    const uint32_t wave_id = blockIdx.x * kWavesPerBlock + (threadIdx.x >> 6);
    const uint32_t n_waves = gridDim.x * kWavesPerBlock;
    RT_TRAVERSAL_LDS(kExtendBlock)
    Trav T;
    T.cur = kTravDone;
    bool has = false;
    bool pending = false;
    float4 pend_o = make_float4(0.0f, 0.0f, 0.0f, 0.0f);
    uint2 pend_a = make_uint2(0u, 0u);
    uint32_t slot = 0;
    uint32_t chunk_pos = wave_id * kExtendChunk;
    uint32_t chunk_end = chunk_pos + kExtendChunk < n ? chunk_pos + kExtendChunk : n;
    bool exhausted = chunk_pos >= n;
    if (exhausted) return;
    TravSigns sg{0ull, 0ull, 0ull};
    for (;;) {
        const bool any_pending = __ballot(pending) != 0ull;
        if (pending) {
            const f3 d = mk3(h2f((uint16_t)pend_a.x), h2f((uint16_t)(pend_a.x >> 16)), h2f((uint16_t)pend_a.y));
            trav_begin(T, mk3(pend_o.x, pend_o.y, pend_o.z), d, stack);
            pending = false;
        }
        if (any_pending) sg = trav_signs(T);
        const bool need = T.cur == kTravDone;
        const unsigned long long need_m = __ballot(need);
        const uint32_t cnt = (uint32_t)__popcll(need_m);
        if (cnt >= kExtendRefill || cnt == 64u) {
            if (STATS) ws.shade_rounds++, ws.shade_lanes += cnt;
            if (need && has) {
                hits[slot] = make_float4(T.best.t, T.best.u, T.best.v, __uint_as_float(T.best.tri));
                has = false;
            }
            if (!exhausted) {
                if (chunk_pos == chunk_end) {
                    uint32_t base = 0;
                    if (lane == 0) base = atomicAdd(cursor, kExtendChunk);
                    base = (uint32_t)__builtin_amdgcn_readfirstlane((int)base) + n_waves * kExtendChunk;
                    if (base >= n) exhausted = true;
                    chunk_pos = base;
                    chunk_end = base + kExtendChunk < n ? base + kExtendChunk : n;
                }
                if (!exhausted) {
                    const uint32_t avail = chunk_end - chunk_pos;
                    const uint32_t take = cnt < avail ? cnt : avail;
// ... 21 lines not shown
}

RT_DEV uint32_t reorder_key(const SceneDev& S, const RayState& r) {
    auto cell = [&](float p, int a) {
        const int c = (int)((p - S.cell_lo[a]) * S.cell_scale[a]);
        return (uint32_t)(c < 0 ? 0 : (c > 3 ? 3 : c));
    };
    const uint32_t cx = cell(r.org.x, 0), cy = cell(r.org.y, 1), cz = cell(r.org.z, 2);
    const uint32_t morton = (cx & 1u) | ((cy & 1u) << 1) | ((cz & 1u) << 2) | ((cx >> 1) << 3) | ((cy >> 1) << 4) | ((cz >> 1) << 5);
    const uint32_t oct = ((uint32_t)(r.dir[0] >> 15) & 1u) | (((uint32_t)(r.dir[1] >> 15) & 1u) << 1) | (((uint32_t)(r.dir[2] >> 15) & 1u) << 2);
    return (oct << 6) | morton;
}

RT_DEV uint32_t block_scan_256(uint32_t v, uint32_t* wave_sums , uint32_t* total) {
    const uint32_t lane = threadIdx.x & 63u, wave = threadIdx.x >> 6;
    uint32_t incl = v;
#pragma unroll
    for (int off = 1; off < 64; off <<= 1) {
        const uint32_t o = __shfl_up(incl, off, 64);
        if ((int)lane >= off) incl += o;
    }
    if (lane == 63u) wave_sums[wave] = incl;
    __syncthreads();
    uint32_t base = 0;
    for (uint32_t w = 0; w < wave; ++w) base += wave_sums[w];
    *total = wave_sums[0] + wave_sums[1] + wave_sums[2] + wave_sums[3];
    return base + incl - v;
}

template <bool REORDER, bool MATSORT>
__global__ void __launch_bounds__(256) k_wf_shade(SceneDev S, QueueDev qin, QueueDev qout, const float4* __restrict__ hits,
                                                   uint32_t* __restrict__ rng, float4* __restrict__ accum,
                                                   const uint32_t* __restrict__ count_in,
                                                   uint32_t* __restrict__ count_out, int last_depth, int rr_active) {
    __shared__ uint32_t wave_total[4];
    __shared__ uint32_t block_base;
    __shared__ uint32_t bins[REORDER ? 512 : 1];
    __shared__ uint32_t perm[MATSORT ? 256 : 1];
    __shared__ uint32_t kind_count[MATSORT ? 8 : 1];
    const uint32_t n = *count_in;
    uint32_t i = blockIdx.x * 256u + threadIdx.x;
    if (blockIdx.x * 256u >= n) return;
    if (MATSORT) {
        uint32_t kind = 7u;
        if (i < n) {
            const uint32_t tri = __float_as_uint(hits[i].w);
            kind = 0u;
            if (tri != kNoTri) {
                const uint32_t iw = S.shade[tri].instance;
                kind = 1u + (S.mats[S.packed_mat ? (iw >> kPackedInstBits) : S.inst[iw].material].type & 3u);
            }
        }
        if (threadIdx.x < 8u) kind_count[threadIdx.x] = 0u;
        __syncthreads();
        const uint32_t rank_in_kind = atomicAdd(&kind_count[kind], 1u);
        __syncthreads();
        uint32_t before = 0;
        for (uint32_t k = 0; k < kind; ++k) before += kind_count[k];
        perm[before + rank_in_kind] = i;
        __syncthreads();
        i = perm[threadIdx.x];
    }
    bool survive = false;
    RayState r{};
    uint32_t id = 0;
    if (i < n) {
        id = queue_load(qin, i, r);
        const float4 hr = hits[i];
        Hit hit;
        hit.t = hr.x, hit.u = hr.y, hit.v = hr.z, hit.tri = __float_as_uint(hr.w);
        uint32_t st = rng[id];
        f3 res;
        const bool done = shade_bounce(S, st, r, hit, res);
        if (done) {
            float4 acc = accum[id];
            acc.x = acc.x + clamp01(res.x), acc.y = acc.y + clamp01(res.y), acc.z = acc.z + clamp01(res.z);
            accum[id] = acc;
        } else {
            survive = !last_depth;
            if (rr_active && survive) survive = roulette(st, r);
        }
        rng[id] = st;
    }
    if (REORDER) {
        bins[threadIdx.x] = 0u, bins[threadIdx.x + 256u] = 0u;
        __syncthreads();
        uint32_t key = 0, rank_in_bin = 0;
        if (survive) {
            key = reorder_key(S, r);
            rank_in_bin = atomicAdd(&bins[key], 1u);
        }
        __syncthreads();
        const uint32_t b0 = bins[2u * threadIdx.x], b1 = bins[2u * threadIdx.x + 1u];
        uint32_t total = 0;
        const uint32_t off = block_scan_256(b0 + b1, wave_total, &total);
        if (threadIdx.x == 0) block_base = total ? atomicAdd(count_out, total) : 0u;
        __syncthreads();
        bins[2u * threadIdx.x] = off, bins[2u * threadIdx.x + 1u] = off + b0;
        __syncthreads();
        if (survive) queue_store(qout, block_base + bins[key] + rank_in_bin, id, r);
        return;
    }
    const unsigned long long mask = __ballot(survive);
    const uint32_t lane = threadIdx.x & 63u, wave = threadIdx.x >> 6;
    const uint32_t prefix = lane_rank(mask);
    if (lane == 0) wave_total[wave] = (uint32_t)__popcll(mask);
    __syncthreads();
    if (threadIdx.x == 0) {
        const uint32_t total = wave_total[0] + wave_total[1] + wave_total[2] + wave_total[3];
        block_base = total ? atomicAdd(count_out, total) : 0u;
    }
    __syncthreads();
    if (survive) {
        uint32_t slot = block_base + prefix;
        for (uint32_t w = 0; w < wave; ++w) slot += wave_total[w];
        queue_store(qout, slot, id, r);
    }
}

constexpr uint32_t kRqIdleCap = 1u << 26;
constexpr uint32_t kNoRay = 0xFFFFFFFFu;
constexpr uint32_t kRqEmpty = 0xFFFFFFFFu, kRqStage = 96u, kRqFlush = 32u, kRqClaim = 16u;
static_assert(kRqFlush + 64u <= kRqStage, "a whole wave of new entries must fit behind an unflushed stage");
RT_DEV unsigned long long rq_load64(const unsigned long long* p) { return __hip_atomic_load(p, __ATOMIC_RELAXED, __HIP_MEMORY_SCOPE_AGENT); }
RT_DEV void rq_store64(unsigned long long* p, unsigned long long v) { __hip_atomic_store(p, v, __ATOMIC_RELAXED, __HIP_MEMORY_SCOPE_AGENT); }

template <bool STATS, bool REQ, bool LIMIT = false, bool SLICED = false, bool CARRY = false, bool BLOCKS = false>
__global__ void __launch_bounds__(kMegaBlock, kMegaWaves) k_wf_finish(SceneDev S, const CameraDev* __restrict__ camp, TileDev tile, QueueDev qin,
                                                                    const uint32_t* __restrict__ count_in, uint32_t* __restrict__ cursor,
                                                                    uint32_t* __restrict__ rng_buf, float4* __restrict__ accum,
                                                                    unsigned long long* __restrict__ extra_rays, uint32_t first_depth, uint32_t max_depth,
                                                                    uint32_t n_samples, uint32_t rr_start,
                                                                    unsigned long long* __restrict__ stats_out, FinishRequeue fq, uint32_t chunk_slots, uint8_t* __restrict__ cost_out,
                                                                    QueueDev qout = QueueDev{}, uint32_t* __restrict__ count_out = nullptr, uint32_t bounce_limit = 0,
                                                                    uint32_t qflags = 0, const MegaFrame* slices = nullptr, uint32_t n_slices = 1) {
    static_assert(!(REQ && LIMIT), "the dynamic queue and the per-bounce hand-over are different schedules");
    static_assert(!(SLICED && (REQ || LIMIT)), "pixel slices belong to the one-launch schedule");
    static_assert(!CARRY || SLICED, "only the sliced schedule keeps a pixel's sums outside the accumulator");
    static_assert(!BLOCKS || CARRY, "a block continuation is a continuation");
    constexpr uint32_t kPend = 0x40000000u;
    const bool holes = (qflags & 1u) != 0u;
    __shared__ unsigned long long out_word;
    __shared__ uint32_t out_exited;
    if (LIMIT && threadIdx.x == 0) out_word = (unsigned long long)kOutBlock, out_exited = 0u;
    __shared__ uint32_t slot_lost;
    if (SLICED && threadIdx.x == 0) slot_lost = 0u;
    WaveStats ws;
    const uint32_t n = *count_in;
    const uint32_t lane = threadIdx.x & 63u;
    constexpr uint32_t kWavesPerBlock = kMegaBlock / 64;
    const uint32_t wave_id = blockIdx.x * kWavesPerBlock + (threadIdx.x >> 6);
    const uint32_t n_waves = gridDim.x * kWavesPerBlock;
    RT_SHADE_LDS
    RT_TRAVERSAL_LDS(kMegaBlock)
    __shared__ unsigned long long rq_stage_mem[REQ ? kWavesPerBlock * kRqStage : 1u];
    typedef __attribute__((address_space(3))) unsigned long long lds_u64_t;
    lds_u64_t* stage = (lds_u64_t*)rq_stage_mem + (threadIdx.x >> 6) * kRqStage;
    uint32_t staged = 0, stale = 0;
    uint32_t idle_polls = 0;
    const uint32_t total_entries = REQ ? n * (n_samples - 1u) : 0u;
    const auto accum_rsrc = __builtin_amdgcn_make_buffer_rsrc((void*)accum, 0, (int)(n * 16u), 0x00020000);
    __shared__ uint32_t xg_lds[SLICED ? 1u : kMegaBlock];
    typedef __attribute__((address_space(3))) uint32_t lds_u32_t;
    auto xg_word = [&]() {
        uint32_t a = stack.base;
        asm volatile("" : "+v"(a));
        return (lds_u32_t*)(size_t)(a - (uint32_t)(size_t)(lds_i32*)lds_stack + (uint32_t)(size_t)(lds_u32_t*)xg_lds);
    };
    const bool xg_packed = !SLICED && camp->width < 65536 && camp->height < 65536;
    __shared__ float sum_lds[SLICED ? 3u * kMegaBlock + kMegaBlock / 64u : 1u];
    typedef __attribute__((address_space(3))) float lds_f32_t;
    lds_f32_t* const sum_r = (lds_f32_t*)sum_lds + (SLICED ? threadIdx.x : 0u);
    lds_f32_t* const sum_g = sum_r + (SLICED ? kMegaBlock : 0u);
    lds_f32_t* const sum_b = sum_g + (SLICED ? kMegaBlock : 0u);
    if (SLICED) *slice_looks_word(sum_r, (lds_f32_t*)sum_lds) = 0u;
    bool chunk_dq = false;
    bool drained = false;
    bool waiting = false;
    Trav T;
    T.cur = kTravDone;
    bool live = false;
    RefillPolicy refill;
    RayState r{};
    uint32_t id = 0, rng = 0, depth = 0;
    unsigned long long wave_rays = 0;
    uint32_t samples_left = 0;
    bool first_counted = false;
    const bool tail_guided = LIMIT && (chunk_slots >> 31) != 0u;
    const uint32_t static_pct = (chunk_slots >> 16) & 0x7Fu;
    chunk_slots &= 0xFFFFu;
    uint32_t first_slots = chunk_slots;
    if (SLICED) first_slots = 0;
    if (tail_guided) {
        const uint32_t per_wave = (uint32_t)(((unsigned long long)n * static_pct / 100u) / (n_waves ? n_waves : 1u));
        first_slots = per_wave < 64u ? 64u : (per_wave & ~63u);
    }
    uint32_t seen = n_waves * first_slots;
    const uint32_t inv_waves = tail_guided ? 0x10000u / (n_waves ? n_waves : 1u) + 1u : 0u;
    const uint32_t n_total = SLICED ? n * n_slices : n;
    uint32_t slice_j = 0;
    uint32_t chunk_pos = wave_id * first_slots;
    uint32_t chunk_end = chunk_pos + first_slots < n_total ? chunk_pos + first_slots : n_total;
    bool exhausted = chunk_pos >= n_total;
    auto state_rsrc = [&](const SliceNow& sn) {
        const uint32_t n_state = BLOCKS ? (uint32_t)tile.local_rows * (uint32_t)camp->width : n;
        return __builtin_amdgcn_make_buffer_rsrc((void*)(((unsigned long long)sn.head.y << 32) | sn.head.x), 0, (int)(n_state * 32u), 0x00020000);
    };
    auto leave = [&]() {
        if (!LIMIT) return;
        uint32_t order = 0;
        if (lane == 0) order = atomicAdd(&out_exited, 1u);
        order = (uint32_t)__builtin_amdgcn_readfirstlane((int)order);
        if (order + 1u != kWavesPerBlock) return;
        const unsigned long long w = out_word;
        const uint32_t used = (uint32_t)w, base = (uint32_t)(w >> 32);
        for (uint32_t i = used + lane; i < kOutBlock; i += 64u) qout.org_id[base + i] = make_float4(0.0f, 0.0f, 0.0f, __uint_as_float(kNoRay));
    };
    if (exhausted) {
        if (!REQ) {
            leave();
            return;
        }
        chunk_pos = chunk_end = 0;
    }
    auto flush = [&]() {
        uint32_t t = 0;
        if (lane == 0) t = atomicAdd(fq.ctl + 0, staged);
        t = (uint32_t)__builtin_amdgcn_readfirstlane((int)t);
        asm volatile("s_waitcnt vmcnt(0)" ::: "memory");
        for (uint32_t i = lane; i < staged; i += 64u)
            if (t + i < fq.capacity) rq_store64(fq.entries + t + i, stage[i]);
        if (lane == 0 && t + staged > fq.capacity) __hip_atomic_store(fq.error, 2u, __ATOMIC_RELAXED, __HIP_MEMORY_SCOPE_AGENT);
        staged = 0;
    };
    for (;;) {
        if (REQ && waiting && samples_left != kRqEmpty) {
            const uint32_t e = samples_left;
            id = e & 0xFFFFFFu, samples_left = (e >> 24) + 1u;
            const CameraDev cam = *camp;
            const int x = (int)(id % (uint32_t)cam.width), ly = (int)(id / (uint32_t)cam.width);
            r = camera_ray(cam, x, tile_global_row(tile, ly), rng);
            depth = 0, first_counted = false;
            trav_begin(T, r.org, ray_dir(r), stack);
            live = true, waiting = false;
        }
        if (!(REQ ? drained : exhausted)) {
            const unsigned long long idle_m = __ballot(!live && !waiting);
            const uint32_t cnt = (uint32_t)__popcll(idle_m);
            if (cnt >= refill.threshold()) {
                if (chunk_pos == chunk_end) {
                    if (!exhausted) {
                        uint32_t w = SLICED ? SliceCursor::claim_width(cnt, n) : !REQ && n_samples > 1u ? cnt : chunk_slots;
                        if (tail_guided) {
                            const uint32_t left = n > seen ? n - seen : 0u;
                            const uint32_t share = (uint32_t)(((unsigned long long)left * inv_waves) >> 16);
                            const uint32_t least = cnt > 16u ? cnt : 16u;
                            if (share < w) w = share > least ? share : least;
                        }
                        uint32_t base = 0;
                        if (lane == 0) base = atomicAdd(cursor, w);
                        base = (uint32_t)__builtin_amdgcn_readfirstlane((int)base) + n_waves * first_slots;
                        seen = base + w;
                        if (base >= n_total) {
                            exhausted = true;
                        } else {
                            chunk_pos = base;
                            chunk_end = base + w < n_total ? base + w : n_total;
                        }
                    }
                    if (REQ && exhausted) {
                        const uint32_t w = cnt > kRqClaim ? cnt : kRqClaim;
                        uint32_t h = 0;
                        if (lane == 0) h = atomicAdd(fq.ctl + 32, w);
                        h = (uint32_t)__builtin_amdgcn_readfirstlane((int)h);
                        if (h >= total_entries) {
                            drained = true;
                        } else {
                            chunk_pos = h;
                            chunk_end = h + w < total_entries ? h + w : total_entries;
                            chunk_dq = true;
                        }
                    }
                }
                if (chunk_pos != chunk_end) {
                    const uint32_t avail = chunk_end - chunk_pos;
                    const uint32_t take = cnt < avail ? cnt : avail;
                    const uint32_t rank = lane_rank(idle_m);
                    uint32_t first_here = 0, first_next = 0;
                    if (SLICED) {
                        slice_j = SliceCursor::advance(slice_j, n_slices, chunk_pos, n);
                        if (slice_j) first_here = frame_slice_bound(slices, slice_j - 1u);
                        first_next = frame_slice_bound(slices, slice_j);
                    }
                    if (!live && !waiting && rank < take) {
                        if (REQ && chunk_dq) {
                            id = chunk_pos + rank;
                            waiting = true;
                        } else {
                            uint32_t slot = chunk_pos + rank, first = 0;
                            if (SLICED) {
                                const SliceSlot m = SliceCursor::map(slot, slice_j, n, first_here, first_next);
                                slot = m.slot, first = m.first;
                            }
                            if (SLICED && slot >= n) {
                                slot_lost = 1u;
                            } else {
                                id = queue_load(qin, slot, r);
                                if (SLICED && first != 0u) {
                                    depth = kPend;
                                    samples_left = n_samples - first, first_counted = false;
                                    live = true;
                                } else if (!(holes && id == kNoRay)) {
                                    rng = rng_buf[id];
                                    depth = first_depth;
                                    samples_left = n_samples, first_counted = !holes;
                                    if (SLICED && CARRY) {
                                        const float4 a = accum[id];
                                        *sum_r = a.x, *sum_g = a.y, *sum_b = a.z;
                                    } else if (SLICED) {
                                        *sum_r = 0.0f, *sum_g = 0.0f, *sum_b = 0.0f;
                                    }
                                    if (!REQ && n_samples > 1u && xg_packed) {
                                        const uint32_t w = (uint32_t)camp->width;
                                        *xg_word() = (id % w) | ((uint32_t)tile_global_row(tile, (int)(id / w)) << 16);
                                    }
                                    trav_begin(T, r.org, ray_dir(r), stack);
                                    live = true;
                                }
                            }
                        }
                    }
                    chunk_pos += take;
                }
            }
        }
        const unsigned long long wait_m = REQ ? __ballot(waiting) : 0ull;
        if (REQ && waiting) {
            const unsigned long long e64 = rq_load64(fq.entries + id);
            samples_left = (uint32_t)e64, rng = (uint32_t)(e64 >> 32);
        }
        const uint32_t n_live = (uint32_t)__popcll(__ballot(live));
        if (n_live == 0) {
            if (!REQ) {
                if (exhausted) break;
                continue;
            }
            if (staged) flush();
            if (wait_m != 0ull) {
                if (++idle_polls > kRqIdleCap) {
                    if (lane == 0) __hip_atomic_store(fq.error, 1u, __ATOMIC_RELAXED, __HIP_MEMORY_SCOPE_AGENT);
                    break;
                }
                __builtin_amdgcn_s_sleep(8);
                continue;
            }
            if (drained) break;
            continue;
        }
        idle_polls = 0;
        const TravSigns sg = trav_signs(T);
        const uint32_t n_rays = SLICED ? (uint32_t)__popcll(__ballot(live && depth < kPend)) : n_live;
        const uint32_t shade_at = n_rays * kMegaShadePct + (n_live - n_rays) * 100u;
        for (;;) {
            const bool done_trav = live && T.cur == kTravDone;
            if ((uint32_t)__popcll(__ballot(done_trav)) * 100u >= shade_at) break;
            if (STATS) ws.live_lane_steps += n_live * kMegaUnroll;
            refill.stepped();
            (void)trav_step_wave<STATS, true>(S, T, stack, top, sg, &ws);
#pragma unroll
            for (int k = 1; k < kMegaUnroll; ++k) (void)trav_step_wave<STATS, true>(S, T, stack, top, sg, &ws);
        }
        if (STATS) ws.shade_rounds++, ws.shade_lanes += (uint32_t)__popcll(__ballot(live && T.cur == kTravDone));
        __builtin_amdgcn_s_setprio(0);
        bool requeue = false, slot_finished = false, hand_on = false;
        {
            const unsigned long long traced = __ballot(live && T.cur == kTravDone && !(SLICED && depth >= kPend));
            wave_rays += (unsigned long long)__popcll(__ballot(live && T.cur == kTravDone && !(first_counted && depth == first_depth) && !(SLICED && depth >= kPend)));
            if (SLICED && traced == 0ull && __ballot(live && depth < kPend) == 0ull && slice_wait_count(slice_looks_word(sum_r, (lds_f32_t*)sum_lds), slices) && lane == 0 && fq.error)
                __hip_atomic_store(fq.error, 4u, __ATOMIC_RELAXED, __HIP_MEMORY_SCOPE_AGENT);
        }
        if (SLICED && live && T.cur == kTravDone && depth >= kPend) {
            const SliceNow sn = frame_slices(slices);
            const auto rsrc = state_rsrc(sn);
            const uint32_t at = id * 32u, tag = sn.head.z + (n_samples - samples_left);
            const u32x4 w0 = __builtin_amdgcn_raw_buffer_load_b128(rsrc, (int)at, 0, 16 );
            const u32x4 w1 = __builtin_amdgcn_raw_buffer_load_b128(rsrc, (int)(at + 16u), 0, 16 );
            if ((w0.y == tag && w0.w == tag && w1.y == tag && w1.w == tag) || slice_wait_over(slice_looks_word(sum_r, (lds_f32_t*)sum_lds), slices)) {
                *sum_r = __uint_as_float(w0.x), *sum_g = __uint_as_float(w0.z), *sum_b = __uint_as_float(w1.x);
                rng = w1.z;
                const CameraDev cam = *camp;
                int x, gy;
                if (xg_packed) {
                    const uint32_t xg = *xg_word();
                    x = (int)(xg & 0xFFFFu), gy = (int)(xg >> 16);
                } else {
                    x = (int)(id % (uint32_t)cam.width), gy = tile_global_row(tile, (int)(id / (uint32_t)cam.width));
                }
                r = camera_ray(cam, x, gy, rng);
                depth = 0;
                trav_begin(T, r.org, ray_dir(r), stack);
            }
        } else if (live && T.cur == kTravDone) {
            f3 res;
            const bool done = shade_bounce<true>(S, rng, r, T.best, res, &T, &tab);
            depth++;
            bool ends = done;
            if (SLICED && done) {
                *sum_r = *sum_r + clamp01(res.x), *sum_g = *sum_g + clamp01(res.y), *sum_b = *sum_b + clamp01(res.z);
            } else if (done) {
                float4 acc;
                if (REQ) {
                    const u32x4 a = __builtin_amdgcn_raw_buffer_load_b128(accum_rsrc, (int)(id * 16u), 0, 16 );
                    acc = make_float4(__uint_as_float(a.x), __uint_as_float(a.y), __uint_as_float(a.z), __uint_as_float(a.w));
                } else {
                    acc = accum[id];
                }
                acc.x = acc.x + clamp01(res.x), acc.y = acc.y + clamp01(res.y), acc.z = acc.z + clamp01(res.z);
                if (REQ) {
                    u32x4 a;
                    a.x = __float_as_uint(acc.x), a.y = __float_as_uint(acc.y), a.z = __float_as_uint(acc.z), a.w = __float_as_uint(acc.w);
                    __builtin_amdgcn_raw_buffer_store_b128(a, accum_rsrc, (int)(id * 16u), 0, 16 );
                } else {
                    accum[id] = acc;
                }
            } else if (depth == max_depth) {
                ends = true;
            } else if (rr_start && depth >= rr_start) {
                ends = !roulette(rng, r);
            }
            bool handed = false;
            if (SLICED && ends && samples_left > 1u) {
                const SliceNow sn = frame_slices(slices);
                const unsigned long long cuts = ((unsigned long long)sn.cuts.y << 32) | sn.cuts.x;
                const uint32_t sh = sn.head.w, s_next = n_samples - (samples_left - 1u);
                handed = (s_next & ((1u << sh) - 1u)) == 0u && ((cuts >> (s_next >> sh)) & 1ull) != 0ull;
                if (handed) {
                    const auto rsrc = state_rsrc(sn);
                    const uint32_t at = id * 32u, tag = sn.head.z + s_next;
                    u32x4 w0, w1;
                    w0.x = __float_as_uint(*sum_r), w0.y = tag, w0.z = __float_as_uint(*sum_g), w0.w = tag;
                    w1.x = __float_as_uint(*sum_b), w1.y = tag, w1.z = rng, w1.w = tag;
                    __builtin_amdgcn_raw_buffer_store_b128(w0, rsrc, (int)at, 0, 16 );
                    __builtin_amdgcn_raw_buffer_store_b128(w1, rsrc, (int)(at + 16u), 0, 16 );
                }
            }
            if (!REQ && ends && !handed && --samples_left) {
                const CameraDev cam = *camp;
                int x, gy;
                if (xg_packed) {
                    const uint32_t xg = *xg_word();
                    x = (int)(xg & 0xFFFFu), gy = (int)(xg >> 16);
                } else {
                    x = (int)(id % (uint32_t)cam.width), gy = tile_global_row(tile, (int)(id / (uint32_t)cam.width));
                }
                r = camera_ray(cam, x, gy, rng);
                depth = 0, first_counted = false;
                ends = false;
            }
            if (ends && !handed && cost_out) cost_out[id] = (uint8_t)(depth < 255u ? depth : 255u);
            if (SLICED && ends && !handed) accum[id] = make_float4(*sum_r, *sum_g, *sum_b, 0.0f);
            if (ends) {
                live = false, slot_finished = true;
                if (REQ) requeue = samples_left > 1u;
                if (!requeue && !handed) rng_buf[id] = rng;
            } else if (LIMIT && depth - first_depth >= bounce_limit) {
                hand_on = true, live = false, slot_finished = true;
            } else {
                trav_begin(T, r.org, ray_dir(r), stack);
            }
        }
        if (LIMIT) {
            const unsigned long long hm = __ballot(hand_on);
            if (hm != 0ull) {
                const uint32_t n_req = (uint32_t)__popcll(hm);
                uint32_t b0 = 0, c0 = 0, b1 = 0;
                if (lane == 0) {
                    for (;;) {
                        const unsigned long long old = atomicAdd(&out_word, (unsigned long long)n_req);
                        const uint32_t used = (uint32_t)old, base = (uint32_t)(old >> 32);
                        if (used + n_req <= kOutBlock) {
                            b0 = base + used, c0 = n_req;
                            break;
                        }
                        if (used <= kOutBlock) {
                            b0 = base + used, c0 = kOutBlock - used;
                            b1 = atomicAdd(count_out, kOutBlock);
                            __hip_atomic_store(&out_word, ((unsigned long long)b1 << 32) | (unsigned long long)(n_req - c0), __ATOMIC_RELAXED, __HIP_MEMORY_SCOPE_WORKGROUP);
                            break;
                        }
                        uint32_t polls = 0;
                        while ((uint32_t)__hip_atomic_load(&out_word, __ATOMIC_RELAXED, __HIP_MEMORY_SCOPE_WORKGROUP) > kOutBlock && ++polls < kRqIdleCap)
                            __builtin_amdgcn_s_sleep(1);
                        if (polls >= kRqIdleCap) {
                            if (fq.error) __hip_atomic_store(fq.error, 3u, __ATOMIC_RELAXED, __HIP_MEMORY_SCOPE_AGENT);
                            b0 = 0, c0 = n_req;
                            break;
                        }
                    }
                }
                b0 = (uint32_t)__builtin_amdgcn_readfirstlane((int)b0), c0 = (uint32_t)__builtin_amdgcn_readfirstlane((int)c0);
                b1 = (uint32_t)__builtin_amdgcn_readfirstlane((int)b1);
                const uint32_t rank = lane_rank(hm);
                if (hand_on) {
                    queue_store(qout, rank < c0 ? b0 + rank : b1 + (rank - c0), id, r);
                    rng_buf[id] = rng;
                }
            }
        }
        refill.round(slot_finished);
        if (REQ) {
            const unsigned long long rq_m = __ballot(requeue);
            const uint32_t n_rq = (uint32_t)__popcll(rq_m);
            if (n_rq) {
                const uint32_t rank = lane_rank(rq_m);
                if (requeue) stage[staged + rank] = (unsigned long long)(id | ((samples_left - 2u) << 24)) | ((unsigned long long)rng << 32);
                staged += n_rq;
            }
            stale = staged ? stale + 1u : 0u;
            if (staged >= kRqFlush || (staged && (wait_m != 0ull || stale >= 4u))) flush(), stale = 0;
        }
        __builtin_amdgcn_s_setprio(2);
    }
    if (SLICED && lane == 0 && slot_lost && fq.error) __hip_atomic_store(fq.error, 5u, __ATOMIC_RELAXED, __HIP_MEMORY_SCOPE_AGENT);
    if (lane == 0 && wave_rays) atomicAdd(extra_rays, wave_rays);
    if (STATS && lane == 0) wave_stats_flush(ws, stats_out);
    leave();
}

template <bool CARRY = false>
__global__ void __launch_bounds__(256) k_wf_resolve(uint32_t n_local, uint32_t spp, uint32_t width, uint32_t strip_rows,
                                                     uint32_t n_lanes, uint32_t lane_index, const float4* __restrict__ accum,
                                                     float* __restrict__ out_f32, uint8_t* __restrict__ out_u8,
                                                     const uint32_t* __restrict__ rng, u32x4* __restrict__ carry) {
    const uint32_t i = blockIdx.x * 256u + threadIdx.x;
    if (i >= n_local) return;
    const float4 a = accum[i];
    const uint32_t x = i % width, row = stream_lane_row(i / width, strip_rows, n_lanes, lane_index);
    const size_t o = (size_t)row * width + x;
    pixel_end(&a.x, &a.y, &a.z, (float)spp, o, out_f32, out_u8);
    if (CARRY) carry[o] = carry_word(a.x, a.y, a.z, rng[i]);
}


__global__ void __launch_bounds__(256) k_blocks_begin(const uint32_t* __restrict__ list, uint32_t n_blocks, uint32_t blocks_x, uint32_t width,
                                                       uint32_t local_rows, uint32_t samples, const u32x4* __restrict__ carry, u32x4* __restrict__ snap,
                                                       uint32_t* __restrict__ count, uint32_t* __restrict__ snap_count) {
    const uint32_t i = blockIdx.x * 4u + (threadIdx.x >> 6), w = threadIdx.x & 63u;
    if (i >= n_blocks) return;
    const uint32_t b = list ? list[i] : i;
    const uint32_t x = (b % blocks_x) * 8u + (w & 7u), ly = (b / blocks_x) * 8u + (w >> 3);
    if (x < width && ly < local_rows) snap[(size_t)ly * width + x] = carry[(size_t)ly * width + x];
    if (w == 0) {
        const uint32_t c = count[b];
        snap_count[b] = c;
        count[b] = c + samples;
    }
}

__global__ void __launch_bounds__(256) k_blocks_resolve(uint32_t n_local, uint32_t width, uint32_t blocks_x, const u32x4* __restrict__ carry,
                                                         const uint32_t* __restrict__ count, float* __restrict__ out_f32, uint8_t* __restrict__ out_u8) {
    const uint32_t i = blockIdx.x * 256u + threadIdx.x;
    if (i >= n_local) return;
    const uint32_t x = i % width, ly = i / width;
    const u32x4 a = carry[i];
    const float sr = __uint_as_float(a.x), sg = __uint_as_float(a.y), sb = __uint_as_float(a.z);
    pixel_end(&sr, &sg, &sb, (float)count[(ly >> 3) * blocks_x + (x >> 3)], i, out_f32, out_u8);
}

__global__ void __launch_bounds__(256) k_wf_generate_blocks(const CameraDev* __restrict__ camp, TileDev tile, const uint32_t* __restrict__ list,
                                                             uint32_t n_blocks, uint32_t tile_rows, uint32_t strip_rows, uint32_t n_lanes,
                                                             uint32_t lane_index, uint32_t* __restrict__ rng, QueueDev q,
                                                             uint32_t* __restrict__ count_out) {
    const uint32_t i = blockIdx.x * 256u + threadIdx.x;
    const CameraDev cam = *camp;
    const uint32_t width = (uint32_t)cam.width, blocks_x = (width + 7u) >> 3;
    bool take = false;
    uint32_t id = 0;
    if (i < n_blocks * 64u) {
        const uint32_t b = list[i >> 6], w = i & 63u;
        const uint32_t x = (b % blocks_x) * 8u + (w & 7u), row = (b / blocks_x) * 8u + (w >> 3);
        const uint32_t strip = row / strip_rows;
        if (x < width && row < tile_rows && strip % n_lanes == lane_index) {
            id = ((strip / n_lanes) * strip_rows + row % strip_rows) * width + x;
            take = true;
        }
    }
    const unsigned long long m = __ballot(take);
    if (m == 0ull) return;
    uint32_t base = 0;
    if ((threadIdx.x & 63u) == 0u) base = atomicAdd(count_out, (uint32_t)__popcll(m));
    base = (uint32_t)__builtin_amdgcn_readfirstlane((int)base);
    if (!take) return;
    const uint32_t rank = lane_rank(m);
    const int x = (int)(id % width), gy = tile_global_row(tile, (int)(id / width));
    uint32_t st = rng[id];
    const RayState r = gy < cam.height ? camera_ray(cam, x, gy, st) : RayState{};
    rng[id] = st;
    queue_store(q, base + rank, id, r);
}

__global__ void __launch_bounds__(256) k_wf_resolve_blocks(uint32_t n_local, uint32_t width, uint32_t strip_rows, uint32_t n_lanes, uint32_t lane_index,
                                                            const uint32_t* __restrict__ count, const float4* __restrict__ accum,
                                                            float* __restrict__ out_f32, uint8_t* __restrict__ out_u8,
                                                            const uint32_t* __restrict__ rng, u32x4* __restrict__ carry) {
    const uint32_t i = blockIdx.x * 256u + threadIdx.x;
    if (i >= n_local) return;
    const float4 a = accum[i];
    const uint32_t x = i % width, row = stream_lane_row(i / width, strip_rows, n_lanes, lane_index);
    const size_t o = (size_t)row * width + x;
    pixel_end(&a.x, &a.y, &a.z, (float)count[(row >> 3) * ((width + 7u) >> 3) + (x >> 3)], o, out_f32, out_u8);
    carry[o] = carry_word(a.x, a.y, a.z, rng[i]);
}

constexpr float kAdaptEps = 1e-4f;
__global__ void __launch_bounds__(256) k_adapt_errors(uint32_t n_blocks, uint32_t blocks_x, uint32_t width, uint32_t local_rows,
                                                       const u32x4* __restrict__ carry, const u32x4* __restrict__ snap,
                                                       const uint32_t* __restrict__ count, const uint32_t* __restrict__ snap_count, float threshold,
                                                       uint32_t min_samples, float* __restrict__ err, uint32_t* __restrict__ active) {
    const uint32_t b = blockIdx.x * 4u + (threadIdx.x >> 6), w = threadIdx.x & 63u;
    if (b >= n_blocks) return;
    const uint32_t n = count[b], n0 = snap_count[b];
// ... 47 lines not shown
```

### sycl-ray-tracer_amd/csrc/rt_types.h

```cpp
#pragma once
#include <cstdint>

namespace rt {

#ifdef __HIPCC__
#define RT_HD __host__ __device__ inline
#else
#define RT_HD inline
#endif
struct alignas(64) BvhNode {
    float origin[3];
    float scale_x;
    uint32_t q[6];
    float scale_y, scale_z;
    int32_t child[4];
    RT_HD float scale(int a) const { const float s = a == 0 ? scale_x : (a == 1 ? scale_y : scale_z); return s < 0.0f ? -s : s; }
    RT_HD void set_scale(int a, float s) { (a == 0 ? scale_x : (a == 1 ? scale_y : scale_z)) = s; }
};
static_assert(sizeof(BvhNode) == 64, "BvhNode must be 64 bytes");
constexpr int32_t kChildEmpty = (int32_t)0x80000000;
struct Box3 {
    float lo[3], hi[3];
};

RT_HD void clear_planes(BvhNode& n) {
    n.scale_x = n.scale_y = n.scale_z = 1.0f;
    n.origin[0] = n.origin[1] = n.origin[2] = 0.0f;
    for (int i = 0; i < 6; ++i) n.q[i] = (i & 1) ? 0u : 0xFFFFFFFFu;
}
RT_HD BvhNode empty_node() {
    BvhNode n;
    clear_planes(n);
    for (int k = 0; k < 4; ++k) n.child[k] = kChildEmpty;
    return n;
}
struct LeafRange {
    uint32_t first, count;
};
RT_HD LeafRange leaf_range(int32_t child) {
    const uint32_t code = (uint32_t)~child;
    return {code >> 2, (code & 3u) + 1u};
}
RT_HD int32_t leaf_child(uint32_t first, uint32_t count) { return ~(int32_t)((first << 2) | (count - 1)); }
RT_HD float child_plane(const BvhNode& n, int k, int a, int side) { return n.origin[a] + (float)((n.q[2 * a + side] >> (8 * k)) & 0xffu) * n.scale(a); }
RT_HD Box3 child_box(const BvhNode& n, int k) {
    Box3 b;
    for (int a = 0; a < 3; ++a) b.lo[a] = child_plane(n, k, a, 0), b.hi[a] = child_plane(n, k, a, 1);
    return b;
}

constexpr int kMaxLeafTris = 2;
constexpr int kTopNodes = 341;
constexpr int kStackSize = 64;
constexpr uint32_t kNoTri = 0xFFFFFFFFu;
constexpr float kTNear = 0.0001f;

struct ContractRange {
    float lo[3], hi[3];
    float limit;
    uint32_t finite_only;
};
RT_HD float contract_max(float a, float b) { return a < b ? b : a; }
RT_HD bool in_contract_range(const ContractRange& r, float ox, float oy, float oz) {
    if (r.finite_only) return __builtin_isfinite(ox) && __builtin_isfinite(oy) && __builtin_isfinite(oz);
    const float o[3] = {ox, oy, oz};
    for (int a = 0; a < 3; ++a) {
        const float outside = contract_max(contract_max(r.lo[a] - o[a], o[a] - r.hi[a]), 0.0f);
        if (!(outside <= r.limit)) return false;
    }
    return true;
}

struct alignas(16) TriRec {
    float v0[3];
    float e1[3];
    float e2[3];
    uint32_t global_index;
    uint32_t pad[2];
};
static_assert(sizeof(TriRec) == 48, "TriRec must be 48 bytes");
constexpr uint32_t kTriBytes = 40;

constexpr uint32_t kPackedInstBits = 20, kPackedInstMask = (1u << kPackedInstBits) - 1u;
struct alignas(64) ShadeRec {
    float n0[3], n1[3], n2[3];
    float uv0[2], uv1[2], uv2[2];
    uint32_t instance;
};
static_assert(sizeof(ShadeRec) == 64, "ShadeRec must be 64 bytes");

constexpr uint32_t kLdsNm = 8, kLdsMats = 24;
struct alignas(16) InstRec {
    float normal_mat[9];
    uint32_t material;
    uint32_t pad[2];
};
static_assert(sizeof(InstRec) == 48, "InstRec must be 48 bytes");

struct alignas(16) MatRec {
    uint32_t type;
    uint32_t tex_kind;
    float color[3];
    uint32_t tex_layer;
    float emissive[3];
    float roughness;
    float ior;
    uint32_t pad;
};
static_assert(sizeof(MatRec) == 48, "MatRec must be 48 bytes");

struct SceneDev {
    const BvhNode* nodes;
    const uint8_t* tris;
    const ShadeRec* shade;
    const InstRec* inst;
    const MatRec* mats;
    const uint8_t* tex;
    uint32_t n_nodes;
    uint32_t n_tris;
    float sky[3];
    float cell_lo[3], cell_scale[3];
    uint32_t packed_mat;
    uint32_t lds_nm, lds_mats;
};

struct CameraDev {
    float center[3], pixel00[3], du[3], dv[3];
    int32_t width, height;
};

struct TileDev {
    uint32_t rank, world, strip_rows;
    int32_t local_rows;
};

}
```

### sycl-ray-tracer_amd/csrc/scene_build.cpp

```cpp
#include "scene_build.h"
#include "bvh_quantise.h"
#include "rt_knobs.h"

#include <algorithm>
#include <array>
#include <cmath>
#include <cstdio>
#include <cstdlib>
#include <cstring>
#include <limits>
#include <map>
#include <memory>
#include <deque>
#include <queue>

namespace rt {
namespace {

struct GNode {
    float lo[3], hi[3];
    int32_t left = -1, right = -1;
    uint32_t first = 0, count = 0;
    uint32_t depth = 0;
};
// ... 772 lines not shown
}

bool world_bounds(const std::vector<float>& wv, float lo[3], float hi[3], float& pad, std::string& err) {
    for (float v : wv)
        if (!std::isfinite(v)) { err = "non-finite world-space vertex"; return false; }
    for (int a = 0; a < 3; ++a) lo[a] = INFINITY, hi[a] = -INFINITY;
    for (size_t i = 0; i < wv.size(); ++i) {
        const int a = (int)(i % 3);
        lo[a] = std::min(lo[a], wv[i]), hi[a] = std::max(hi[a], wv[i]);
    }
    return scene_padding(lo, hi, pad, err);
}

void scene_cells(const HostScene& hs, SceneDev& dev) {
    for (int a = 0; a < 3; ++a) {
        const float ext = hs.bounds_hi[a] - hs.bounds_lo[a];
        dev.cell_lo[a] = hs.bounds_lo[a];
        dev.cell_scale[a] = ext > 0.0f && std::isfinite(ext) ? 4.0f / ext : 0.0f;
    }
}

void shading_rows(const rt_instance* inst, uint32_t n, const std::vector<uint64_t>& use, bool packed, std::vector<InstRec>& out,
                  std::vector<uint32_t>& slot) {
    slot.assign(n, 0);
    if (packed) {
        std::map<std::array<uint32_t, 9>, uint32_t> seen;
        std::vector<std::array<uint32_t, 9>> rows;
        std::vector<uint64_t> row_use;
        for (uint32_t i = 0; i < n; ++i) {
            std::array<uint32_t, 9> key;
            std::memcpy(key.data(), inst[i].normal_mat, 36);
            auto it = seen.find(key);
            if (it == seen.end()) {
                it = seen.emplace(key, (uint32_t)rows.size()).first;
                rows.push_back(key), row_use.push_back(0);
            }
            slot[i] = it->second;
            row_use[it->second] += use[i];
        }
        std::vector<uint32_t> order(rows.size()), rank(rows.size());
        for (uint32_t k = 0; k < order.size(); ++k) order[k] = k;
        std::stable_sort(order.begin(), order.end(), [&](uint32_t a, uint32_t b) { return row_use[a] > row_use[b]; });
        for (uint32_t k = 0; k < order.size(); ++k) rank[order[k]] = k;
        out.assign(rows.size(), InstRec{});
        for (uint32_t k = 0; k < rows.size(); ++k) std::memcpy(out[rank[k]].normal_mat, rows[k].data(), 36);
        for (uint32_t i = 0; i < n; ++i) slot[i] = rank[slot[i]];
    } else {
        out.assign(n, InstRec{});
        for (uint32_t i = 0; i < n; ++i) {
            std::memcpy(out[i].normal_mat, inst[i].normal_mat, sizeof(float) * 9);
            out[i].material = inst[i].material;
            slot[i] = i;
        }
    }
}

bool scene_padding(const float lo[3], const float hi[3], float& pad, std::string& err) {
    float ext = 0.0f, amax = 0.0f;
    for (int a = 0; a < 3; ++a) {
        ext = std::max(ext, hi[a] - lo[a]);
        amax = std::max(amax, std::max(std::fabs(lo[a]), std::fabs(hi[a])));
    }
    pad = 2e-5f * std::max(ext, amax) + 1e-30f;
    bool finite = std::isfinite(ext) && std::isfinite(pad);
    for (int a = 0; a < 3; ++a) finite = finite && std::isfinite(lo[a] - pad) && std::isfinite(hi[a] + pad);
    if (!finite) { err = "scene extent overflows fp32 (the padded bounds are not finite)"; return false; }
    return true;
}

void node_levels(const std::vector<BvhNode>& nodes, std::vector<uint32_t>& level_nodes, std::vector<uint32_t>& level_start) {
    const size_t n = nodes.size();
    std::vector<uint32_t> height(n, 0), post;
    std::vector<uint32_t> st{0};
    post.reserve(n);
    while (!st.empty()) {
        const uint32_t i = st.back();
        st.pop_back();
        post.push_back(i);
        for (int k = 0; k < 4; ++k)
            if (nodes[i].child[k] >= 0) st.push_back((uint32_t)nodes[i].child[k]);
    }
    uint32_t top = 0;
    for (size_t q = post.size(); q-- > 0;) {
        const uint32_t i = post[q];
        uint32_t h = 0;
        for (int k = 0; k < 4; ++k)
            if (nodes[i].child[k] >= 0) h = std::max(h, height[(size_t)nodes[i].child[k]] + 1);
        height[i] = h, top = std::max(top, h);
    }
    level_start.assign((size_t)top + 2, 0);
    for (uint32_t i : post) level_start[(size_t)height[i] + 1]++;
    for (size_t h = 1; h < level_start.size(); ++h) level_start[h] += level_start[h - 1];
    level_nodes.assign(post.size(), 0);
    std::vector<uint32_t> at(level_start.begin(), level_start.end() - 1);
    std::vector<uint8_t> reached(n, 0);
    for (uint32_t i : post) reached[i] = 1;
    for (uint32_t i = 0; i < (uint32_t)n; ++i)
        if (reached[i]) level_nodes[at[height[i]]++] = i;
}

void record_boxes(HostScene& hs) {
    hs.rec_lo.assign(3 * hs.tris.size(), 0.0f), hs.rec_hi.assign(3 * hs.tris.size(), 0.0f);
    for (size_t r = 0; r < hs.tris.size(); ++r) {
        if (hs.tris[r].global_index == kNoTri) continue;
        const float* w = &hs.wverts[9 * (size_t)hs.tris[r].global_index];
        for (int a = 0; a < 3; ++a)
            hs.rec_lo[3 * r + a] = std::min(w[a], std::min(w[3 + a], w[6 + a])), hs.rec_hi[3 * r + a] = std::max(w[a], std::max(w[3 + a], w[6 + a]));
    }
}

Box3 leaf_bounds(const HostScene& hs, int32_t child) {
    const bool split = hs.rec_lo.size() == 3 * hs.tris.size() && hs.rec_hi.size() == 3 * hs.tris.size() && hs.n_split_triangles > 0;
    const LeafRange leaf = leaf_range(child);
    Box3 b{{INFINITY, INFINITY, INFINITY}, {-INFINITY, -INFINITY, -INFINITY}};
    for (uint32_t r = leaf.first; r < leaf.first + leaf.count; ++r) {
        if (split) {
            for (int a = 0; a < 3; ++a) b.lo[a] = std::min(b.lo[a], hs.rec_lo[3 * (size_t)r + a]), b.hi[a] = std::max(b.hi[a], hs.rec_hi[3 * (size_t)r + a]);
        } else {
            const float* w = &hs.wverts[9 * (size_t)hs.tris[r].global_index];
            for (int v = 0; v < 3; ++v)
                for (int a = 0; a < 3; ++a) b.lo[a] = std::min(b.lo[a], w[3 * v + a]), b.hi[a] = std::max(b.hi[a], w[3 * v + a]);
        }
    }
    return b;
}

bool refit_host(HostScene& hs, const std::vector<uint32_t>& level_nodes, std::vector<float>& box, std::string& err) {
    record_boxes(hs);
    for (TriRec& tr : hs.tris) {
        if (tr.global_index == kNoTri) continue;
        const float* w = &hs.wverts[9 * (size_t)tr.global_index];
        for (int a = 0; a < 3; ++a) tr.v0[a] = w[a], tr.e1[a] = w[3 + a] - w[a], tr.e2[a] = w[6 + a] - w[a];
    }
    box.assign(6 * hs.nodes.size(), 0.0f);
    for (uint32_t i : level_nodes) {
        BvhNode& n = hs.nodes[i];
        Box3 kb[4];
        int nk = 0;
        for (int k = 0; k < 4 && n.child[k] != kChildEmpty; ++k, ++nk) {
            if (n.child[k] >= 0) std::memcpy(&kb[k], &box[6 * (size_t)n.child[k]], sizeof(Box3));
            else kb[k] = leaf_bounds(hs, n.child[k]);
            float* b = &box[6 * (size_t)i];
            for (int a = 0; a < 3; ++a) b[a] = k ? std::min(b[a], kb[k].lo[a]) : kb[k].lo[a], b[3 + a] = k ? std::max(b[3 + a], kb[k].hi[a]) : kb[k].hi[a];
        }
        if (nk == 0) continue;
        BvhNode q = n;
        if (!quantise_node(q, nk, kb, hs.pad)) { err = "a refit node's child boxes could not be quantised"; return false; }
        std::memcpy(&n, &q, 48);
    }
    hs.sah_cost = refit_sah_cost(hs, box);
    return true;
}

}
```

### sycl-ray-tracer_amd/csrc/scene_build.h

```cpp
#pragma once
#include <cstdint>
#include <string>
#include <vector>

#include "../../include/rt_mi355x.h"
#include "rt_types.h"

namespace rt {

struct HostScene {
    std::vector<BvhNode> nodes;
    std::vector<TriRec> tris;
    std::vector<ShadeRec> shade;
    std::vector<InstRec> inst;
    std::vector<MatRec> mats;
    std::vector<uint8_t> tex;
    std::vector<float> wverts;
    std::vector<float> rec_lo, rec_hi;
    uint32_t n_split_triangles = 0;
    uint32_t n_layers = 0;
    bool packed_mat = false;
    int8_t built_by = -1;
    float sky[3] = {0.5f, 0.7f, 1.0f};
    float bounds_lo[3] = {0, 0, 0}, bounds_hi[3] = {0, 0, 0};
    float pad = 0.0f;
    uint32_t max_depth = 0, max_leaf_tris = 0, stack_need = 0;
    double sah_cost = 0.0;
};

constexpr int RT_BVH_MEDIAN_INTERNAL = 99;

int build_host_scene(const rt_scene_desc* desc, int bvh_kind, HostScene& out, std::string& err);

int build_lbvh_gpu(HostScene& hs, const std::vector<TriRec>& gtris, std::string& err);

void world_vertices(uint32_t n_tris, const uint32_t* indices, const uint32_t* tri_instance, const rt_instance* inst, const float* positions,
                    std::vector<float>& wv);
bool world_bounds(const std::vector<float>& wv, float lo[3], float hi[3], float& pad, std::string& err);
void scene_cells(const HostScene& hs, SceneDev& dev);
void record_boxes(HostScene& hs);
Box3 leaf_bounds(const HostScene& hs, int32_t child);
inline float half_area(const float* lo, const float* hi) {
    float dx = hi[0] - lo[0], dy = hi[1] - lo[1], dz = hi[2] - lo[2];
    if (!(dx >= 0 && dy >= 0 && dz >= 0)) return 0.0f;
    return dx * dy + dy * dz + dz * dx;
}

void shading_rows(const rt_instance* inst, uint32_t n, const std::vector<uint64_t>& use, bool packed, std::vector<InstRec>& rows,
                  std::vector<uint32_t>& slot);
bool scene_padding(const float lo[3], const float hi[3], float& pad, std::string& err);
void node_levels(const std::vector<BvhNode>& nodes, std::vector<uint32_t>& level_nodes, std::vector<uint32_t>& level_start);
bool refit_host(HostScene& hs, const std::vector<uint32_t>& level_nodes, std::vector<float>& box, std::string& err);
double refit_sah_cost(const HostScene& hs, const std::vector<float>& box);
double decoded_sah_cost(const HostScene& hs);

int check_bvh(const HostScene& hs, std::string& err);

int count_visits(const HostScene& hs, uint32_t n, const float* org, const float* dir, int mode, uint64_t* node_visits, uint64_t* tri_tests, float* t_out,
                 uint32_t* tri_out, std::string& err);

}
```

### sycl-ray-tracer_amd/csrc/scene_check.cpp

```cpp
#include "scene_build.h"

#include <algorithm>
#include <cmath>
#include <limits>

namespace rt {
namespace {

void grow(Box3& r, const Box3& c) {
    for (int a = 0; a < 3; ++a) r.lo[a] = std::min(r.lo[a], c.lo[a]), r.hi[a] = std::max(r.hi[a], c.hi[a]);
}

template <class Enter, class Visit>
bool exact_boxes(const HostScene& hs, int32_t child, uint32_t depth, Box3& r, Enter&& enter, Visit&& visit) {
    const float inf = std::numeric_limits<float>::infinity();
    r = Box3{{inf, inf, inf}, {-inf, -inf, -inf}};
    if (!enter(child, depth)) return false;
    if (child < 0) {
        r = leaf_bounds(hs, child);
        return true;
    }
    const BvhNode& n = hs.nodes[(size_t)child];
    for (int k = 0; k < 4; ++k) {
        if (n.child[k] == kChildEmpty) continue;
        Box3 c;
        if (!exact_boxes(hs, n.child[k], depth + 1, c, enter, visit) || !visit(child, k, c)) return false;
        grow(r, c);
    }
    return true;
}

}

double decoded_sah_cost(const HostScene& hs) {
    double cost = 0.0, root_area = 0.0;
    for (size_t i = 0; i < hs.nodes.size(); ++i) {
        const BvhNode& n = hs.nodes[i];
        Box3 nb{{INFINITY, INFINITY, INFINITY}, {-INFINITY, -INFINITY, -INFINITY}};
        for (int k = 0; k < 4; ++k) {
            if (n.child[k] == kChildEmpty) continue;
            const Box3 b = child_box(n, k);
            grow(nb, b);
            const double w = n.child[k] >= 0 ? 1.0 : (double)leaf_range(n.child[k]).count;
            cost += w * (double)half_area(b.lo, b.hi);
        }
        if (i == 0) root_area = (double)half_area(nb.lo, nb.hi);
    }
    return root_area > 0.0 ? 1.0 + cost / root_area : 0.0;
}

double refit_sah_cost(const HostScene& hs, const std::vector<float>& box) {
    if (hs.built_by == RT_BVH_LBVH_GPU) return decoded_sah_cost(hs);
    if (hs.nodes.empty() || box.size() < 6 * hs.nodes.size()) return 0.0;
    const double root_area = std::max(1e-30, (double)half_area(&box[0], &box[3]));
    double cost = 0.0;
    for (const BvhNode& n : hs.nodes)
        for (int k = 0; k < 4; ++k) {
            if (n.child[k] == kChildEmpty) continue;
            if (n.child[k] >= 0) {
                cost += (double)half_area(&box[6 * (size_t)n.child[k]], &box[6 * (size_t)n.child[k] + 3]) / root_area;
            } else {
                const Box3 b = leaf_bounds(hs, n.child[k]);
                cost += (double)half_area(b.lo, b.hi) / root_area * (double)leaf_range(n.child[k]).count;
            }
        }
    return 1.0 + cost;
}

int check_bvh(const HostScene& hs, std::string& err) {
    const size_t T = hs.wverts.size() / 9;
    if (hs.nodes.empty()) { err = "no root node"; return RT_ERR_INVALID; }
    std::vector<uint32_t> seen(T, 0);
    const bool split = hs.rec_lo.size() == 3 * hs.tris.size() && hs.rec_hi.size() == 3 * hs.tris.size() && hs.n_split_triangles > 0;
    std::vector<std::vector<uint32_t>> pieces(split ? T : 0);
    size_t visited = 0;
    auto fail = [&](const std::string& m) { err = m; return false; };
    auto enter = [&](int32_t child, uint32_t depth) {
        if (depth >= (uint32_t)kStackSize) return fail("tree deeper than traversal stack");
        if (child >= 0) {
            if ((size_t)child >= hs.nodes.size()) return fail("child index out of range");
            if (++visited > hs.nodes.size()) return fail("cycle in node graph");
            return true;
        }
        const LeafRange leaf = leaf_range(child);
        if ((size_t)leaf.first + leaf.count > hs.tris.size()) return fail("leaf range out of bounds");
        for (uint32_t k = 0; k < leaf.count; ++k) {
            const TriRec& tr = hs.tris[leaf.first + k];
            if (tr.global_index >= T) return fail("leaf triangle has bad global index");
            for (uint32_t j = 0; j < k; ++j)
                if (hs.tris[leaf.first + j].global_index == tr.global_index) return fail("triangle twice in one leaf");
            if (seen[tr.global_index]++ && !split) return fail("triangle appears in two leaves");
            const float* w = &hs.wverts[9 * (size_t)tr.global_index];
            if (tr.v0[0] != w[0] || tr.v0[1] != w[1] || tr.v0[2] != w[2]) return fail("leaf triangle data mismatch");
            if (split) pieces[tr.global_index].push_back(leaf.first + k);
        }
        return true;
    };
    auto contained = [&](int32_t node, int k, const Box3& c) {
        const Box3 d = child_box(hs.nodes[(size_t)node], k);
        for (int a = 0; a < 3; ++a)
            if (!(d.lo[a] <= c.lo[a] - 0.5f * hs.pad) || !(d.hi[a] >= c.hi[a] + 0.5f * hs.pad))
                return fail("decoded child box does not contain its subtree (node " + std::to_string(node) + ")");
        return true;
    };
    Box3 all;
    if (!exact_boxes(hs, 0, 0, all, enter, contained)) return RT_ERR_INVALID;
    for (size_t t = 0; t < T; ++t)
        if (!seen[t]) { err = "triangle " + std::to_string(t) + " is in no leaf"; return RT_ERR_INVALID; }
    if (split) {
        for (size_t t = 0; t < T; ++t) {
            if (pieces[t].size() < 2) continue;
            const float* w = &hs.wverts[9 * t];
            for (int i = 0; i <= 8; ++i)
                for (int j = 0; i + j <= 8; ++j) {
                    const double u = i / 8.0, v = j / 8.0, ww = 1.0 - u - v;
                    double p[3];
                    for (int a = 0; a < 3; ++a) p[a] = ww * w[a] + u * w[3 + a] + v * w[6 + a];
                    bool in = false;
                    for (uint32_t rec : pieces[t]) {
                        bool inside = true;
                        for (int a = 0; a < 3; ++a) {
                            const double tol = 1e-6 * (std::fabs(p[a]) + 1.0);
                            inside = inside && p[a] >= (double)hs.rec_lo[3 * (size_t)rec + a] - tol && p[a] <= (double)hs.rec_hi[3 * (size_t)rec + a] + tol;
                        }
                        in = in || inside;
                    }
                    if (!in) { err = "the pieces of split triangle " + std::to_string(t) + " do not cover it"; return RT_ERR_INVALID; }
                }
        }
    }
    return RT_OK;
}

int count_visits(const HostScene& hs, uint32_t n, const float* org, const float* dir, int mode, uint64_t* node_visits, uint64_t* tri_tests, float* t_out,
                 uint32_t* tri_out, std::string& err) {
    if (mode < 0 || mode > 2) { err = "mode: 0 quantised, 1 exact, 2 quantised with two more bits"; return RT_ERR_INVALID; }
    if (hs.nodes.empty()) { err = "no tree"; return RT_ERR_INVALID; }
    const float inf = std::numeric_limits<float>::infinity();
    std::vector<Box3> box(hs.nodes.size() * 4);
    auto tested = [&](int32_t node, int k, const Box3& c) {
        const BvhNode& nd = hs.nodes[(size_t)node];
        Box3& out = box[(size_t)node * 4 + k];
        if (mode == 0) out = child_box(nd, k);
        else for (int a = 0; a < 3; ++a) {
            if (mode == 1) {
                out.lo[a] = c.lo[a] - hs.pad, out.hi[a] = c.hi[a] + hs.pad;
            } else {
                const float q = nd.scale(a) * 0.25f;
                out.lo[a] = nd.origin[a] + std::floor((c.lo[a] - hs.pad - nd.origin[a]) / q) * q;
                out.hi[a] = nd.origin[a] + std::ceil((c.hi[a] + hs.pad - nd.origin[a]) / q) * q;
            }
        }
        return true;
    };
    Box3 all;
    (void)exact_boxes(hs, 0, 0, all, [](int32_t, uint32_t) { return true; }, tested);
    uint64_t visits = 0, tests = 0;
    for (uint32_t i = 0; i < n; ++i) {
        const float o[3] = {org[3 * i], org[3 * i + 1], org[3 * i + 2]}, d[3] = {dir[3 * i], dir[3 * i + 1], dir[3 * i + 2]};
        float inv[3];
        for (int a = 0; a < 3; ++a) inv[a] = 1.0f / (std::fabs(d[a]) < 1e-30f ? std::copysign(1e-30f, d[a]) : d[a]);
        float best = inf;
        uint32_t best_tri = kNoTri;
        int32_t stack[kStackSize * 4];
        int sp = 0;
        int32_t cur = 0;
        for (;;) {
            if (cur >= 0) {
                visits++;
                const BvhNode& nd = hs.nodes[(size_t)cur];
                float key[4];
                int32_t ch[4];
                int m = 0;
                for (int k = 0; k < 4; ++k) {
                    if (nd.child[k] == kChildEmpty) continue;
                    const Box3& b = box[(size_t)cur * 4 + k];
                    float tn = 0.0f, tf = best;
                    for (int a = 0; a < 3; ++a) {
                        const float t0 = (b.lo[a] - o[a]) * inv[a], t1 = (b.hi[a] - o[a]) * inv[a];
                        tn = std::max(tn, std::min(t0, t1)), tf = std::min(tf, std::max(t0, t1));
                    }
                    if (tn <= tf) key[m] = tn, ch[m] = nd.child[k], m++;
                }
                for (int a = 1; a < m; ++a)
                    for (int b = a; b > 0 && key[b] < key[b - 1]; --b) std::swap(key[b], key[b - 1]), std::swap(ch[b], ch[b - 1]);
                for (int a = m - 1; a >= 1; --a) stack[sp++] = ch[a];
                if (m) { cur = ch[0]; continue; }
            } else {
                const LeafRange leaf = leaf_range(cur);
                for (uint32_t k = 0; k < leaf.count; ++k) {
                    tests++;
                    const TriRec& tr = hs.tris[leaf.first + k];
                    const double e1[3] = {tr.e1[0], tr.e1[1], tr.e1[2]}, e2[3] = {tr.e2[0], tr.e2[1], tr.e2[2]};
                    const double p[3] = {d[1] * e2[2] - d[2] * e2[1], d[2] * e2[0] - d[0] * e2[2], d[0] * e2[1] - d[1] * e2[0]};
                    const double det = e1[0] * p[0] + e1[1] * p[1] + e1[2] * p[2];
                    if (det == 0.0) continue;
                    const double tv[3] = {o[0] - tr.v0[0], o[1] - tr.v0[1], o[2] - tr.v0[2]};
                    const double u = (tv[0] * p[0] + tv[1] * p[1] + tv[2] * p[2]) / det;
                    const double q[3] = {tv[1] * e1[2] - tv[2] * e1[1], tv[2] * e1[0] - tv[0] * e1[2], tv[0] * e1[1] - tv[1] * e1[0]};
                    const double v = (d[0] * q[0] + d[1] * q[1] + d[2] * q[2]) / det;
                    if (u < 0.0 || v < 0.0 || u + v > 1.0) continue;
                    const double t = (e2[0] * q[0] + e2[1] * q[1] + e2[2] * q[2]) / det;
                    if (t > (double)kTNear && (t < best || (t == best && tr.global_index < best_tri))) best = (float)t, best_tri = tr.global_index;
                }
            }
            if (sp == 0) break;
            cur = stack[--sp];
        }
        if (t_out) t_out[i] = best;
        if (tri_out) tri_out[i] = best_tri;
    }
    if (node_visits) *node_visits = visits;
    if (tri_tests) *tri_tests = tests;
    return RT_OK;
}

}
```

### sycl-ray-tracer_amd/rtamd/abi.py

```python
from __future__ import annotations

import ctypes as C
import os
from pathlib import Path

PKG_DIR = Path(__file__).resolve().parent.parent
REPO_DIR = PKG_DIR.parent
LIB_PATH = PKG_DIR / "csrc" / "build" / "librt_mi355x.so"

RT_OK = 0
RT_ERR_INVALID, RT_ERR_NO_DEVICE, RT_ERR_HIP, RT_ERR_OOM, RT_ERR_UNSUPPORTED = -1, -2, -3, -4, -5

RT_MAT_NONE, RT_MAT_DIFFUSE, RT_MAT_METALLIC, RT_MAT_DIELECTRIC = 0, 1, 2, 3
RT_TEX_COLOR, RT_TEX_IMAGE = 0, 1
RT_RENDERER_MEGAKERNEL, RT_RENDERER_WAVEFRONT = 0, 1
RT_SEED_DEFAULT, RT_SEED_WAVEFRONT, RT_SEED_MEGAKERNEL = 0, 1, 2
RT_BVH_DEFAULT, RT_BVH_LBVH, RT_BVH_SAH, RT_BVH_LBVH_GPU = 0, 1, 2, 3
RT_BVH_MEDIAN_INTERNAL = 99
RT_SCENE_UPDATABLE = 1
RT_SCENE_KEEP_PREVIOUS = 2
RT_TEX_SIZE = 512
RT_TEX_MAX_LAYERS = 128


# ... 255 lines not shown
    "rt_trace_paths": (C.c_int, [C.c_void_p, _P(rt_path_query)]),
    "rt_trace_paths_device": (C.c_int, [C.c_void_p, _P(rt_path_query), C.c_void_p]),
    "rt_gather_paths": (C.c_int, [C.c_void_p, _P(rt_gather_query)]),
    "rt_gather_paths_device": (C.c_int, [C.c_void_p, _P(rt_gather_query), C.c_void_p]),
    "rt_lightmap_create": (C.c_int, [C.c_void_p, C.c_int32, C.c_int32, C.c_uint32, _P(C.c_float), _P(C.c_void_p)]),
    "rt_lightmap_destroy": (None, [C.c_void_p]),
    "rt_lightmap_texels": (C.c_int, [C.c_void_p, _P(C.c_uint32), _P(C.c_float), _P(C.c_float)]),
    "rt_lightmap_texels_device": (C.c_int, [C.c_void_p, C.c_void_p, C.c_void_p, C.c_void_p, C.c_void_p]),
    "rt_lightmap_bake": (C.c_int, [C.c_void_p, _P(rt_lightmap_params), _P(C.c_float), _P(rt_lightmap_stats)]),
    "rt_lightmap_bake_device": (C.c_int, [C.c_void_p, _P(rt_lightmap_params), C.c_void_p, C.c_void_p, C.c_void_p]),
    "rt_renderer_create": (C.c_int, [C.c_int, C.c_void_p, C.c_int32, C.c_int32, C.c_uint32, C.c_uint32,
                                     C.c_uint32, _P(C.c_void_p)]),
    "rt_renderer_destroy": (None, [C.c_void_p]),
    "rt_renderer_set_tile": (C.c_int, [C.c_void_p, C.c_uint32, C.c_uint32, C.c_uint32]),
    "rt_renderer_local_rows": (C.c_int32, [C.c_void_p]),
    "rt_renderer_global_row": (C.c_int32, [C.c_void_p, C.c_int32]),
    "rt_renderer_set_profiling": (C.c_int, [C.c_void_p, C.c_int]),
    "rt_renderer_set_russian_roulette": (C.c_int, [C.c_void_p, C.c_uint32]),
    "rt_renderer_set_frame_seed": (C.c_int, [C.c_void_p, C.c_uint32]),
    "rt_renderer_set_schedule": (C.c_int, [C.c_void_p, _P(rt_schedule)]),
    "rt_renderer_get_schedule": (C.c_int, [C.c_void_p, _P(rt_schedule)]),
    "rt_render_frame_begin": (C.c_int, [C.c_void_p, C.POINTER(rt_camera), C.c_void_p, C.c_void_p, C.c_void_p]),
    "rt_render_frame_end": (C.c_int, [C.c_void_p, C.POINTER(rt_stats)]),
    "rt_render_frame": (C.c_int, [C.c_void_p, _P(rt_camera), _P(C.c_float), _P(C.c_uint8), _P(rt_stats)]),
    "rt_render_frame_device": (C.c_int, [C.c_void_p, _P(rt_camera), C.c_void_p, C.c_void_p, C.c_void_p,
                                         _P(rt_stats)]),
    "rt_renderer_set_progressive": (C.c_int, [C.c_void_p, C.c_int]),
    "rt_render_frame_continue": (C.c_int, [C.c_void_p, C.c_uint32, _P(C.c_float), _P(C.c_uint8), _P(rt_stats)]),
    "rt_render_frame_continue_device": (C.c_int, [C.c_void_p, C.c_uint32, C.c_void_p, C.c_void_p, C.c_void_p, _P(rt_stats)]),
    "rt_renderer_accumulated_samples": (C.c_int, [C.c_void_p, _P(C.c_uint32)]),
    "rt_renderer_block_grid": (C.c_int, [C.c_void_p, _P(C.c_uint32), _P(C.c_uint32)]),
    "rt_render_frame_continue_blocks": (C.c_int, [C.c_void_p, C.c_uint32, _P(C.c_uint32), C.c_uint32, _P(C.c_float), _P(C.c_uint8), _P(rt_stats)]),
    "rt_render_frame_continue_blocks_device": (C.c_int, [C.c_void_p, C.c_uint32, _P(C.c_uint32), C.c_uint32, C.c_void_p, C.c_void_p, C.c_void_p,
                                                         _P(rt_stats)]),
    "rt_renderer_block_samples": (C.c_int, [C.c_void_p, _P(C.c_uint32)]),
    "rt_renderer_adapt": (C.c_int, [C.c_void_p, C.c_float, C.c_uint32, _P(C.c_uint32), _P(C.c_uint32)]),
    "rt_render_frame_continue_adaptive": (C.c_int, [C.c_void_p, C.c_uint32, C.c_float, C.c_uint32, _P(C.c_float), _P(C.c_uint8), _P(rt_stats),
                                                    _P(C.c_uint32)]),
    "rt_render_frame_continue_adaptive_device": (C.c_int, [C.c_void_p, C.c_uint32, C.c_float, C.c_uint32, C.c_void_p, C.c_void_p, C.c_void_p,
                                                           _P(rt_stats), _P(C.c_uint32)]),
    "rt_renderer_block_errors": (C.c_int, [C.c_void_p, _P(C.c_float)]),
    "rt_scene_gbuffer": (C.c_int, [C.c_void_p, _P(rt_camera), _P(C.c_float), _P(C.c_float), _P(C.c_float)]),
    "rt_scene_gbuffer_device": (C.c_int, [C.c_void_p, _P(rt_camera), C.c_void_p, C.c_void_p, C.c_void_p, C.c_void_p]),
    "rt_scene_gbuffer_motion": (C.c_int, [C.c_void_p, _P(rt_camera), _P(C.c_float), _P(C.c_float), _P(C.c_float), _P(C.c_float)]),
    "rt_scene_gbuffer_motion_device": (C.c_int, [C.c_void_p, _P(rt_camera), C.c_void_p, C.c_void_p, C.c_void_p, C.c_void_p, C.c_void_p]),
    "rt_temporal_create": (C.c_int, [C.c_int, C.c_int32, C.c_int32, _P(C.c_void_p)]),
    "rt_temporal_destroy": (None, [C.c_void_p]),
    "rt_temporal_reset": (C.c_int, [C.c_void_p]),
    "rt_temporal_accumulate": (C.c_int, [C.c_void_p, _P(rt_temporal_params), _P(rt_camera), _P(C.c_float), _P(C.c_float), _P(C.c_float),
                                         _P(C.c_float), _P(C.c_float), _P(C.c_uint8), _P(C.c_float)]),
    "rt_temporal_accumulate_device": (C.c_int, [C.c_void_p, _P(rt_temporal_params), _P(rt_camera), C.c_void_p, C.c_void_p, C.c_void_p, C.c_void_p,
                                                C.c_void_p, C.c_void_p, C.c_void_p, C.c_void_p]),
    "rt_temporal_create_ex": (C.c_int, [C.c_int, C.c_int32, C.c_int32, C.c_uint32, _P(C.c_void_p)]),
    "rt_temporal_accumulate_moments": (C.c_int, [C.c_void_p, _P(rt_temporal_params), _P(rt_camera), _P(C.c_float), _P(C.c_float), _P(C.c_float),
                                                 _P(C.c_float), _P(C.c_float), _P(C.c_uint8), _P(C.c_float), _P(C.c_float)]),
    "rt_temporal_accumulate_moments_device": (C.c_int, [C.c_void_p, _P(rt_temporal_params), _P(rt_camera), C.c_void_p, C.c_void_p, C.c_void_p,
                                                        C.c_void_p, C.c_void_p, C.c_void_p, C.c_void_p, C.c_void_p, C.c_void_p]),
    "rt_denoiser_create": (C.c_int, [C.c_int, C.c_int32, C.c_int32, _P(C.c_void_p)]),
    "rt_denoiser_destroy": (None, [C.c_void_p]),
    "rt_denoise": (C.c_int, [C.c_void_p, _P(rt_denoise_params), _P(C.c_float), _P(C.c_float), _P(C.c_float), _P(C.c_float),
                             _P(C.c_float), _P(C.c_uint8)]),
    "rt_denoise_device": (C.c_int, [C.c_void_p, _P(rt_denoise_params), C.c_void_p, C.c_void_p, C.c_void_p, C.c_void_p, C.c_void_p,
                                    C.c_void_p, C.c_void_p]),
    "rt_denoiser_create_ex": (C.c_int, [C.c_int, C.c_int32, C.c_int32, C.c_uint32, _P(C.c_void_p)]),
    "rt_denoise_variance": (C.c_int, [C.c_void_p, _P(rt_denoise_var_params), _P(C.c_float), _P(C.c_float), _P(C.c_float), _P(C.c_float),
                                      _P(C.c_float), _P(C.c_float), _P(C.c_float)]),
    "rt_denoise_variance_device": (C.c_int, [C.c_void_p, _P(rt_denoise_var_params), C.c_void_p, C.c_void_p, C.c_void_p, C.c_void_p, C.c_void_p,
                                             C.c_void_p, C.c_void_p, C.c_void_p]),
    "rt_denoise_guided": (C.c_int, [C.c_void_p, _P(rt_denoise_var_params), _P(C.c_float), _P(C.c_float), _P(C.c_float), _P(C.c_float),
                                    _P(C.c_float), _P(C.c_float), _P(C.c_uint8), _P(C.c_float)]),
    "rt_denoise_guided_device": (C.c_int, [C.c_void_p, _P(rt_denoise_var_params), C.c_void_p, C.c_void_p, C.c_void_p, C.c_void_p, C.c_void_p,
                                           C.c_void_p, C.c_void_p, C.c_void_p, C.c_void_p]),
    "rt_comm_create": (C.c_int, [C.c_int, _P(C.c_int), _P(C.c_void_p)]),
    "rt_comm_destroy": (None, [C.c_void_p]),
    "rt_comm_uses_rccl": (C.c_int, [C.c_void_p]),
    "rt_renderer_tile_f32": (C.c_void_p, [C.c_void_p]),
    "rt_renderer_tile_u8": (C.c_void_p, [C.c_void_p]),
    "rt_frame_gather": (C.c_int, [C.c_void_p, _P(C.c_void_p), _P(C.c_float), _P(C.c_uint8), C.c_int, C.c_int]),
    "rt_frame_gather_begin": (C.c_int, [C.c_void_p, _P(C.c_void_p), C.c_int, C.c_int]),
    "rt_comm_wait": (C.c_int, [C.c_void_p, _P(C.c_float), _P(C.c_uint8)]),
    "rt_comm_size": (C.c_int, [C.c_void_p]),
    "rt_comm_frame_f32": (C.c_void_p, [C.c_void_p]),
    "rt_comm_frame_u8": (C.c_void_p, [C.c_void_p]),
    "rt_probe_xorshift": (C.c_int, [C.c_int, C.c_uint32, C.c_uint32, _P(C.c_float), _P(C.c_uint32)]),
    "rt_probe_half_roundtrip": (C.c_int, [C.c_int, C.c_uint32, _P(C.c_float), _P(C.c_float), _P(C.c_uint16)]),
    "rt_probe_scatter": (C.c_int, [C.c_void_p, C.c_uint32, C.c_uint32, _P(C.c_float), _P(C.c_float),
                                   _P(C.c_float), _P(C.c_uint32), _P(C.c_uint8), _P(C.c_float),
                                   _P(C.c_float), _P(C.c_uint32)]),
    "rt_last_error": (C.c_char_p, []),
    "rt_probe_rounding": (C.c_int, [C.c_int, _P(C.c_uint64)]),
    "rt_abi_version": (C.c_int, []),
    "rt_device_count": (C.c_int, []),
}

_lib = None


class RtError(RuntimeError):
    def __init__(self, status: int, msg: str):
        super().__init__(f"rt_status {status}: {msg}")
        self.status = status


def load_library(path: os.PathLike | None = None) -> C.CDLL:
    global _lib
    if _lib is not None and path is None:
        return _lib
    p = Path(path) if path else Path(os.environ.get("RT_MI355X_LIB", LIB_PATH))
    if not p.exists():
        raise FileNotFoundError(
            f"{p} is missing: build the HIP library first (python -c 'import __graft_entry__ as g; g.build()' "
            f"or make -C {PKG_DIR / 'csrc'}). There is no CPU fallback for the render path.")
    lib = C.CDLL(str(p), mode=C.RTLD_GLOBAL)
    for name, (res, args) in PROTOTYPES.items():
        fn = getattr(lib, name)
        fn.restype = res
        fn.argtypes = args
    if path is None:
        _lib = lib
    return lib


def check(status: int, lib: C.CDLL | None = None) -> None:
    if status != RT_OK:
        msg = (lib or load_library()).rt_last_error()
        raise RtError(status, msg.decode() if msg else "")


DEV_LIB_PATH = PKG_DIR / "csrc" / "build" / "librt_mi355x_dev.so"
_dev_lib = None


def load_developer_library() -> C.CDLL:
    global _dev_lib
    if _dev_lib is None:
        lib = load_library(DEV_LIB_PATH)
        for name, (res, args) in DEV_PROTOTYPES.items():
            fn = getattr(lib, name)
            fn.restype = res
            fn.argtypes = args
        _dev_lib = lib
    return _dev_lib


DEV_PROTOTYPES = {
    "rt_dev_slice_plan": (C.c_int, [C.c_uint32, C.c_int32, C.c_double, _P(C.c_uint32), _P(C.c_uint32), _P(C.c_uint64),
                                    _P(C.c_uint32)]),
    "rt_dev_slice_replay": (C.c_int, [C.c_uint32, C.c_uint32, _P(C.c_uint32), C.c_uint32, C.c_uint64, C.c_int,
                                      _P(C.c_uint32), _P(C.c_uint32), C.c_uint32, _P(C.c_uint32)]),
    "rt_dev_scene_tables": (C.c_int, [C.c_void_p, _P(C.c_uint32), _P(C.c_uint32), _P(C.c_uint32), _P(C.c_uint32), _P(C.c_float), C.c_uint32,
                                      _P(C.c_uint32)]),
    "rt_dev_scene_tree": (C.c_int, [C.c_void_p, _P(C.c_uint32), _P(C.c_uint32), _P(C.c_uint32), _P(C.c_uint32), _P(C.c_int32), _P(C.c_float),
                                    _P(C.c_float), C.c_void_p, _P(C.c_uint32), _P(C.c_float), C.c_uint32]),
    "rt_dev_renderer_graph_captures": (C.c_int, [C.c_void_p, _P(C.c_uint32)]),
    "rt_dev_quantise_node": (C.c_int, [C.c_uint32, _P(C.c_int32), _P(C.c_float), _P(C.c_float), C.c_void_p, _P(C.c_uint8)]),
}


def fptr(a):
    return a.ctypes.data_as(_P(C.c_float))


def u32ptr(a):
    return a.ctypes.data_as(_P(C.c_uint32))


def u8ptr(a):
    return a.ctypes.data_as(_P(C.c_uint8))


def i32ptr(a):
    return a.ctypes.data_as(_P(C.c_int32))
```

Before: 9823.

## Skip the coplanar origin subtree when tracing bounce rays

Builds a per-triangle origin-skip table on the host. Each entry names a small coplanar BVH subtree that contains the triangle, plus half-precision thresholds. At the start of each bounce ray the kernel computes a skip child word from that entry and stores it in an extra LDS slot. Inner traversal then culls that child, so rays leaving a flat surface no longer re-enter the subtree they started on. The cost is an extra table read per bounce, one more LDS word per thread, fewer top-tree nodes cached in LDS, and a conservative correctness argument that a host-side checker validates.

```diff
diff --git a/sycl-ray-tracer_amd/csrc/rt_abi.hip b/sycl-ray-tracer_amd/csrc/rt_abi.hip
--- a/sycl-ray-tracer_amd/csrc/rt_abi.hip
+++ b/sycl-ray-tracer_amd/csrc/rt_abi.hip
@@ -83,6 +83,15 @@
         delete s;
         return fail(rc, err);
     }
+    rc = no_throw([&] {
+        if ((flags & RT_SCENE_UPDATABLE) || s->hs.built_by == RT_BVH_LBVH_GPU) clear_skip_table(s->hs);
+        else build_skip_table(s->hs);
+        return (int)RT_OK;
+    });
+    if (rc != RT_OK) {
+        delete s;
+        return rc;
+    }
     s->device = device;
     if (device >= 0) {
         rc = device_ok(device);
@@ -103,6 +112,7 @@
             rc = upload(packed, &s->dev.tris, s->device_bytes);
         }
         if (rc == RT_OK) rc = upload(s->hs.shade, &s->dev.shade, s->device_bytes);
+        if (rc == RT_OK) rc = upload(s->hs.skip, &s->dev.skip, s->device_bytes);
         if (rc == RT_OK) {
             std::vector<InstRec> rows(s->hs.inst);
             if (flags & RT_SCENE_UPDATABLE) rows.resize(std::max<size_t>(rows.size(), desc->n_instances));
@@ -142,7 +152,7 @@
         for (auto& se : s->ev_gbuffer) (void)hipEventSynchronize(se.second), (void)hipEventDestroy(se.second);
         (void)hipFree((void*)s->dev.nodes), (void)hipFree((void*)s->dev.tris), (void)hipFree((void*)s->dev.shade);
         (void)hipFree((void*)s->dev.inst), (void)hipFree((void*)s->dev.mats), (void)hipFree((void*)s->dev.tex);
-        (void)hipFree((void*)s->d_query_cursor);
+        (void)hipFree((void*)s->d_query_cursor), (void)hipFree((void*)s->dev.skip);
     }
     free_scene_update(s);
     delete s;
@@ -484,6 +494,18 @@
     return RT_OK;
 }
 
+int rt_dev_scene_skip_table(rt_scene* s, uint32_t* n_entries, uint32_t* entries, uint32_t capacity, int write) {
+    if (!s || !n_entries) return fail(RT_ERR_INVALID, "null argument");
+    if (const int rc = sync_host_copy(s)) return rc;
+    *n_entries = (uint32_t)s->hs.skip.size();
+    const size_t n = std::min<size_t>(capacity, s->hs.skip.size());
+    if (entries && n) {
+        if (write) std::memcpy(s->hs.skip.data(), entries, n * sizeof(SkipRec));
+        else std::memcpy(entries, s->hs.skip.data(), n * sizeof(SkipRec));
+    }
+    return RT_OK;
+}
+
 int rt_dev_renderer_graph_captures(const rt_renderer* r, uint32_t* out) {
     if (!r || !out) return fail(RT_ERR_INVALID, "null argument");
     *out = r->graph_captures;
diff --git a/sycl-ray-tracer_amd/csrc/rt_bounce.h b/sycl-ray-tracer_amd/csrc/rt_bounce.h
--- a/sycl-ray-tracer_amd/csrc/rt_bounce.h
+++ b/sycl-ray-tracer_amd/csrc/rt_bounce.h
@@ -20,6 +20,18 @@
     return done;
 }
 
+RT_DEV void origin_skip_none(const TravStack& stack) { *lds_at(skip_word_addr(stack)) = (int32_t)kSkipNone; }
+RT_DEV void origin_skip(const SceneDev& S, uint32_t tri, const Trav& T, const TravStack& stack) {
+    const u32x4* ep = reinterpret_cast<const u32x4*>(S.skip + (tri == kNoTri ? 0u : tri));
+    const u32x4 a = ep[0], b = ep[1];
+    SkipRec e;
+    e.ref = a.x, e.n[0] = __uint_as_float(a.y), e.n[1] = __uint_as_float(a.z), e.n[2] = __uint_as_float(a.w);
+    e.p[0] = __uint_as_float(b.x), e.p[1] = __uint_as_float(b.y), e.p[2] = __uint_as_float(b.z), e.a = b.w;
+    const float o[3] = {T.o.x, T.o.y, T.o.z}, d[3] = {T.d.x, T.d.y, T.d.z};
+    const uint32_t w = origin_skip_word(e, o, d);
+    *lds_at(skip_word_addr(stack)) = (int32_t)(tri == kNoTri ? kSkipNone : w);
+}
+
 RT_DEV bool roulette(uint32_t& rng, RayState& r) {
     const float qx = h2f(r.att[0]), qy = h2f(r.att[1]), qz = h2f(r.att[2]);
     const float p = __builtin_fminf(__builtin_fmaxf(__builtin_fmaxf(qx, __builtin_fmaxf(qy, qz)), 0.05f), 1.0f);
diff --git a/sycl-ray-tracer_amd/csrc/rt_device.h b/sycl-ray-tracer_amd/csrc/rt_device.h
--- a/sycl-ray-tracer_amd/csrc/rt_device.h
+++ b/sycl-ray-tracer_amd/csrc/rt_device.h
@@ -192,6 +192,7 @@
 };
 RT_DEV uint32_t stack_base(const TravStack& st) { return st.base + st.pitch; }
 RT_DEV lds_i32* lds_at(uint32_t addr) { return (lds_i32*)(size_t)addr; }
+RT_DEV uint32_t skip_word_addr(const TravStack& st) { return st.base + (uint32_t)kLdsStack * st.pitch; }
 RT_DEV bool stack_shallow(const TravStack& st, const Trav& T, uint32_t pushes) { return T.sp <= st.base + ((uint32_t)kLdsStack - pushes) * st.pitch; }
 RT_DEV void trav_pop_lds(Trav& T, const TravStack& st) {
     T.sp -= st.pitch;
@@ -258,8 +259,11 @@
     uint32_t shade_rounds = 0, shade_lanes = 0, live_lane_steps = 0, top_lanes = 0;
 };
 RT_DEV TravSigns trav_signs(const Trav& T) { return TravSigns{lanes(T.ix < 0.0f), lanes(T.iy < 0.0f), lanes(T.iz < 0.0f)}; }
+template <bool SKIP = false>
 RT_DEV void trav_inner(const SceneDev& S, Trav& T, const TravStack& stack, const TopTree& top, const TravSigns& sg) {
     const float inf = __builtin_huge_valf();
+    uint32_t skip = kSkipNone;
+    if (SKIP) skip = (uint32_t)*lds_at(skip_word_addr(stack));
     float k0, k1, k2, k3;
     u32x4 w0, w1, w2, chw;
     if (T.cur < top.count * 64) {
@@ -286,18 +290,19 @@
     const uint32_t qnx = sel(nx, w1.x, w1.y), qfx = sel(nx, w1.y, w1.x);
     const uint32_t qny = sel(ny, w1.z, w1.w), qfy = sel(ny, w1.w, w1.z);
     const uint32_t qnz = sel(nz, w2.x, w2.y), qfz = sel(nz, w2.y, w2.x);
-#define RT_CHILD(K, CVT)                                                                                  \
+#define RT_CHILD(K, CVT, CW)                                                                              \
     {                                                                                                    \
         const float tn = __builtin_fmaxf(__builtin_fmaxf(__builtin_fmaf(CVT(qnx), ax, bx), __builtin_fmaf(CVT(qny), ay, by)), \
                                          __builtin_fmaxf(__builtin_fmaf(CVT(qnz), az, bz), 0.0f));       \
         const float tf = __builtin_fminf(__builtin_fminf(__builtin_fmaf(CVT(qfx), ax, bx), __builtin_fmaf(CVT(qfy), ay, by)), \
                                          __builtin_fminf(__builtin_fmaf(CVT(qfz), az, bz), T.best.t));   \
-        K = sel(lanes(tn <= tf), inf, tn);                                                               \
-    }
-    RT_CHILD(k0, ub0)
-    RT_CHILD(k1, ub1)
-    RT_CHILD(k2, ub2)
-    RT_CHILD(k3, ub3)
+        K = sel(SKIP ? (lanes(tn <= tf) & lanes(CW != skip)) : lanes(tn <= tf), inf, tn);                \
+    }
+    if (SKIP) asm volatile("s_waitcnt vmcnt(0)" : "+v"(chw));
+    RT_CHILD(k0, ub0, chw.x)
+    RT_CHILD(k1, ub1, chw.y)
+    RT_CHILD(k2, ub2, chw.z)
+    RT_CHILD(k3, ub3, chw.w)
 #undef RT_CHILD
 #define RT_CE(KA, CA, KB, CB)                                                        \
     {                                                                               \
@@ -306,7 +311,7 @@
         const int32_t ca = sel(sw, CA, CB), cb = sel(sw, CB, CA);                   \
         KA = ka, KB = kb, CA = ca, CB = cb;                                         \
     }
-    asm volatile("s_waitcnt vmcnt(0)" : "+v"(chw));
+    if (!SKIP) asm volatile("s_waitcnt vmcnt(0)" : "+v"(chw));
     int32_t c0 = (int32_t)chw.x, c1 = (int32_t)chw.y, c2 = (int32_t)chw.z, c3 = (int32_t)chw.w;
     RT_CE(k0, c0, k1, c1)
     RT_CE(k2, c2, k3, c3)
@@ -353,14 +358,14 @@
     }
 }
 
-template <bool STATS = false, bool LEAF_BATCH = false>
+template <bool STATS = false, bool LEAF_BATCH = false, bool SKIP = false>
 RT_DEV uint32_t trav_step_wave(const SceneDev& S, Trav& T, const TravStack& stack, const TopTree& top, const TravSigns& sg, WaveStats* ws = nullptr) {
     const bool inner = T.cur >= 0;
     const bool leaf = T.cur < 0 && T.cur != kTravDone;
     const uint32_t ni = (uint32_t)__popcll(__ballot(inner)), nl = (uint32_t)__popcll(__ballot(leaf));
     if (ni * 3u >= nl * 4u && !(LEAF_BATCH && nl >= 64u)) {
-        if (STATS && ni) ws->inner_steps++, ws->inner_lanes += ni, ws->top_lanes += (uint32_t)__popcll(__ballot(inner && T.cur < kTopNodes * 64));
-        if (inner) trav_inner(S, T, stack, top, sg);
+        if (STATS && ni) ws->inner_steps++, ws->inner_lanes += ni, ws->top_lanes += (uint32_t)__popcll(__ballot(inner && T.cur < (SKIP ? top.count : kTopNodes) * 64));
+        if (inner) trav_inner<SKIP>(S, T, stack, top, sg);
     } else {
         if (STATS) ws->leaf_steps++, ws->leaf_lanes += (uint32_t)__popcll(__ballot(leaf));
         if (leaf) trav_leaf<LEAF_BATCH>(S, T, stack);
@@ -597,12 +602,16 @@
 
 RT_DEV uint8_t to_unorm8(float c) { return (uint8_t)__builtin_rintf(clamp01(c) * 255.0f); }
 
-#define RT_TRAVERSAL_LDS(BLOCK)                                                                        \
-    __shared__ u32x4 top_all[4 * kTopNodes];  \
-    u32x4 *const top_w0 = top_all, *const top_w1 = top_all + kTopNodes, *const top_w2 = top_all + 2 * kTopNodes, *const top_ch = top_all + 3 * kTopNodes; \
-    __shared__ int32_t lds_stack[kLdsStack * (BLOCK)];                                                 \
+#define RT_TRAVERSAL_LDS(BLOCK) RT_TRAVERSAL_LDS_(BLOCK, kTopNodes, 0)
+#define RT_TRAVERSAL_LDS_SKIP(BLOCK, ON)                                                               \
+    RT_TRAVERSAL_LDS_(BLOCK, (ON) ? kTopNodes - (int)(BLOCK) / 16 : kTopNodes, (ON) ? 1 : 0)           \
+    if (ON) lds_stack[kLdsStack * (BLOCK) + threadIdx.x] = (int32_t)kSkipNone;
+#define RT_TRAVERSAL_LDS_(BLOCK, NTOP, EXTRA)                                                          \
+    __shared__ u32x4 top_all[4 * (NTOP)];  \
+    u32x4 *const top_w0 = top_all, *const top_w1 = top_all + (NTOP), *const top_w2 = top_all + 2 * (NTOP), *const top_ch = top_all + 3 * (NTOP); \
+    __shared__ int32_t lds_stack[(kLdsStack + (EXTRA)) * (BLOCK)];                                     \
     int32_t spill[kStackSize - kLdsStack];                                                             \
-    const int32_t top_count = (int32_t)S.n_nodes < kTopNodes ? (int32_t)S.n_nodes : kTopNodes;         \
+    const int32_t top_count = (int32_t)S.n_nodes < (NTOP) ? (int32_t)S.n_nodes : (NTOP);               \
     top_tree_fill(S, top_w0, top_w1, top_w2, top_ch, top_count);                                       \
     __syncthreads();                                                                                   \
     const TopTree top{(lds_u32x4*)top_w0, (lds_u32x4*)top_w1, (lds_u32x4*)top_w2, (lds_u32x4*)top_ch, top_count}; \
diff --git a/sycl-ray-tracer_amd/csrc/rt_kernels.h b/sycl-ray-tracer_amd/csrc/rt_kernels.h
--- a/sycl-ray-tracer_amd/csrc/rt_kernels.h
+++ b/sycl-ray-tracer_amd/csrc/rt_kernels.h
@@ -205,7 +205,7 @@
     Trav T;
     if (SLICED) *slice_looks_word(color_r, (lds_f32*)color_lds) = 0u;
     RT_SHADE_LDS
-    RT_TRAVERSAL_LDS(kMegaBlock)
+    RT_TRAVERSAL_LDS_SKIP(kMegaBlock, true)
     T.cur = kTravDone;
     constexpr uint32_t kPend = 0x40000000u;
     bool live = false;
@@ -239,6 +239,7 @@
                     r = camera_ray(cam, x, gy, rng);
                 }
                 trav_begin(T, r.org, ray_dir(r), stack);
+                origin_skip_none(stack);
             } else {
                 depth = kPend;
             }
@@ -297,11 +298,11 @@
             if (STATS >= 2) ws.live_lane_steps += n_live;
             if (STATS == 1) ws.inner_steps += (uint32_t)kMegaUnroll;
             refill.stepped();
-            (void)trav_step_wave<(STATS >= 2), true>(S, T, stack, top, sg, &ws);
+            (void)trav_step_wave<(STATS >= 2), true, true>(S, T, stack, top, sg, &ws);
 #pragma unroll
             for (int k = 1; k < kMegaUnroll; ++k) {
                 if (STATS >= 2) ws.live_lane_steps += n_live;
-                (void)trav_step_wave<(STATS >= 2), true>(S, T, stack, top, sg, &ws);
+                (void)trav_step_wave<(STATS >= 2), true, true>(S, T, stack, top, sg, &ws);
             }
         }
         if (STATS) {
@@ -315,6 +316,7 @@
         if (STATS >= 2) ck[7] = (long long)__builtin_readcyclecounter();
 #endif
         bool pixel_finished = false;
+        bool bounced = false;
         {
             const unsigned long long traced = __ballot(live && T.cur == kTravDone && depth < kPend);
             wave_rays += (unsigned long long)__popcll(traced);
@@ -380,6 +382,8 @@
                         pixel_end(color_r, color_g, color_b, n, pix, out_f32, out_u8);
                         if constexpr (CARRY != 0) frame_carry(frame)[pix] = carry_word(*color_r, *color_g, *color_b, rng);
                     }
+                } else {
+                    bounced = true;
                 }
             }
             if (start) {
@@ -388,7 +392,11 @@
                 asm volatile("" : "+v"(cx), "+v"(cy));
                 r = camera_ray(frame_camera(frame, width, height), cx, cy, rng);
             }
-            if (live && depth < kPend) trav_begin(T, r.org, ray_dir(r), stack);
+            if (live && depth < kPend) {
+                const uint32_t from = bounced ? T.best.tri : kNoTri;
+                trav_begin(T, r.org, ray_dir(r), stack);
+                origin_skip(S, from, T, stack);
+            }
             RT_STAMP_AFTER((STATS >= 2 ? ck : nullptr), 5, T.ox);
         }
         refill.round(pixel_finished);
@@ -716,7 +724,8 @@
     const uint32_t wave_id = blockIdx.x * kWavesPerBlock + (threadIdx.x >> 6);
     const uint32_t n_waves = gridDim.x * kWavesPerBlock;
     RT_SHADE_LDS
-    RT_TRAVERSAL_LDS(kMegaBlock)
+    constexpr bool kSkip = !LIMIT;
+    RT_TRAVERSAL_LDS_SKIP(kMegaBlock, kSkip)
     __shared__ unsigned long long rq_stage_mem[REQ ? kWavesPerBlock * kRqStage : 1u];
     typedef __attribute__((address_space(3))) unsigned long long lds_u64_t;
     lds_u64_t* stage = (lds_u64_t*)rq_stage_mem + (threadIdx.x >> 6) * kRqStage;
@@ -806,6 +815,7 @@
             r = camera_ray(cam, x, tile_global_row(tile, ly), rng);
             depth = 0, first_counted = false;
             trav_begin(T, r.org, ray_dir(r), stack);
+            if constexpr (kSkip) origin_skip_none(stack);
             live = true, waiting = false;
         }
         if (!(REQ ? drained : exhausted)) {
@@ -889,6 +899,7 @@
                                         *xg_word() = (id % w) | ((uint32_t)tile_global_row(tile, (int)(id / w)) << 16);
                                     }
                                     trav_begin(T, r.org, ray_dir(r), stack);
+                                    if constexpr (kSkip) origin_skip_none(stack);
                                     live = true;
                                 }
                             }
@@ -930,9 +941,9 @@
             if ((uint32_t)__popcll(__ballot(done_trav)) * 100u >= shade_at) break;
             if (STATS) ws.live_lane_steps += n_live * kMegaUnroll;
             refill.stepped();
-            (void)trav_step_wave<STATS, true>(S, T, stack, top, sg, &ws);
+            (void)trav_step_wave<STATS, true, kSkip>(S, T, stack, top, sg, &ws);
 #pragma unroll
-            for (int k = 1; k < kMegaUnroll; ++k) (void)trav_step_wave<STATS, true>(S, T, stack, top, sg, &ws);
+            for (int k = 1; k < kMegaUnroll; ++k) (void)trav_step_wave<STATS, true, kSkip>(S, T, stack, top, sg, &ws);
         }
         if (STATS) ws.shade_rounds++, ws.shade_lanes += (uint32_t)__popcll(__ballot(live && T.cur == kTravDone));
         __builtin_amdgcn_s_setprio(0);
@@ -963,12 +974,14 @@
                 r = camera_ray(cam, x, gy, rng);
                 depth = 0;
                 trav_begin(T, r.org, ray_dir(r), stack);
+                if constexpr (kSkip) origin_skip_none(stack);
             }
         } else if (live && T.cur == kTravDone) {
             f3 res;
             const bool done = shade_bounce<true>(S, rng, r, T.best, res, &T, &tab);
             depth++;
             bool ends = done;
+            bool bounced = !done;
             if (SLICED && done) {
                 *sum_r = *sum_r + clamp01(res.x), *sum_g = *sum_g + clamp01(res.y), *sum_b = *sum_b + clamp01(res.z);
             } else if (done) {
@@ -1019,7 +1032,7 @@
                 }
                 r = camera_ray(cam, x, gy, rng);
                 depth = 0, first_counted = false;
-                ends = false;
+                ends = false, bounced = false;
             }
             if (ends && !handed && cost_out) cost_out[id] = (uint8_t)(depth < 255u ? depth : 255u);
             if (SLICED && ends && !handed) accum[id] = make_float4(*sum_r, *sum_g, *sum_b, 0.0f);
@@ -1030,7 +1043,9 @@
             } else if (LIMIT && depth - first_depth >= bounce_limit) {
                 hand_on = true, live = false, slot_finished = true;
             } else {
+                const uint32_t from = bounced ? T.best.tri : kNoTri;
                 trav_begin(T, r.org, ray_dir(r), stack);
+                if constexpr (kSkip) origin_skip(S, from, T, stack);
             }
         }
         if (LIMIT) {
diff --git a/sycl-ray-tracer_amd/csrc/rt_types.h b/sycl-ray-tracer_amd/csrc/rt_types.h
--- a/sycl-ray-tracer_amd/csrc/rt_types.h
+++ b/sycl-ray-tracer_amd/csrc/rt_types.h
@@ -109,6 +109,32 @@
 };
 static_assert(sizeof(MatRec) == 48, "MatRec must be 48 bytes");
 
+constexpr uint32_t kSkipNone = 1u;
+constexpr float kSkipDist = 40400.0f;
+constexpr float kSkipTilt = 1.0f / 256.0f;
+struct alignas(16) SkipRec {
+    uint32_t ref;
+    float n[3];
+    float p[3];
+    uint32_t a;
+};
+static_assert(sizeof(SkipRec) == 32, "SkipRec must be 32 bytes");
+RT_HD float skip_half(uint32_t bits16) {
+    const uint16_t b = (uint16_t)bits16;
+    _Float16 h;
+    __builtin_memcpy(&h, &b, 2);
+    return (float)h;
+}
+RT_HD uint32_t origin_skip_word(const SkipRec& e, const float o[3], const float d[3]) {
+    const float wx = o[0] - e.p[0], wy = o[1] - e.p[1], wz = o[2] - e.p[2];
+    const float s = __builtin_fmaf(e.n[2], wz, __builtin_fmaf(e.n[1], wy, e.n[0] * wx));
+    const float nd = __builtin_fabsf(__builtin_fmaf(e.n[2], d[2], __builtin_fmaf(e.n[1], d[1], e.n[0] * d[0])));
+    const float l = (__builtin_fabsf(wx) + __builtin_fabsf(wy)) + __builtin_fabsf(wz);
+    const float ld = (__builtin_fabsf(d[0]) + __builtin_fabsf(d[1])) + __builtin_fabsf(d[2]);
+    const float thr = __builtin_fmaf(skip_half(e.a >> 16), l, __builtin_fmaf(kSkipDist, __builtin_fabsf(s), skip_half(e.a & 0xffffu)));
+    return (nd > thr && nd > kSkipTilt * ld) ? e.ref : kSkipNone;
+}
+
 struct SceneDev {
     const BvhNode* nodes;
     const uint8_t* tris;
@@ -122,6 +148,7 @@
     float cell_lo[3], cell_scale[3];
     uint32_t packed_mat;
     uint32_t lds_nm, lds_mats;
+    const SkipRec* skip;
 };
 
 struct CameraDev {
diff --git a/sycl-ray-tracer_amd/csrc/scene_build.cpp b/sycl-ray-tracer_amd/csrc/scene_build.cpp
--- a/sycl-ray-tracer_amd/csrc/scene_build.cpp
+++ b/sycl-ray-tracer_amd/csrc/scene_build.cpp
@@ -948,4 +948,61 @@
     return true;
 }
 
-}
+void clear_skip_table(HostScene& hs) {
+    SkipRec none{};
+    none.ref = kSkipNone;
+    hs.skip.assign(hs.wverts.size() / 9, none);
+}
+
+void build_skip_table(HostScene& hs) {
+    clear_skip_table(hs);
+    const size_t T = hs.skip.size();
+    if (T == 0 || hs.nodes.empty()) return;
+    std::vector<int32_t> parent(hs.nodes.size(), -1);
+    std::vector<int32_t> rec_node(hs.tris.size(), -1);
+    std::vector<uint8_t> rec_slot(hs.tris.size(), 0);
+    for (size_t i = 0; i < hs.nodes.size(); ++i)
+        for (int k = 0; k < 4; ++k) {
+            const int32_t c = hs.nodes[i].child[k];
+            if (c == kChildEmpty) continue;
+            if (c >= 0) {
+                if ((size_t)c < hs.nodes.size()) parent[(size_t)c] = (int32_t)i;
+                continue;
+            }
+            const LeafRange leaf = leaf_range(c);
+            for (uint32_t r = leaf.first; r < leaf.first + leaf.count && r < hs.tris.size(); ++r) rec_node[r] = (int32_t)i, rec_slot[r] = (uint8_t)k;
+        }
+    std::vector<int32_t> first_rec(T, -1);
+    for (size_t r = hs.tris.size(); r-- > 0;)
+        if (hs.tris[r].global_index < T && rec_node[r] >= 0) first_rec[hs.tris[r].global_index] = (int32_t)r;
+    for (size_t t = 0; t < T; ++t) {
+        if (first_rec[t] < 0) continue;
+        const float* w = &hs.wverts[9 * t];
+        double e1[3], e2[3];
+        for (int a = 0; a < 3; ++a) e1[a] = (double)w[3 + a] - (double)w[a], e2[a] = (double)w[6 + a] - (double)w[a];
+        const double c[3] = {e1[1] * e2[2] - e1[2] * e2[1], e1[2] * e2[0] - e1[0] * e2[2], e1[0] * e2[1] - e1[1] * e2[0]};
+        const double len = std::sqrt(c[0] * c[0] + c[1] * c[1] + c[2] * c[2]);
+        if (!(len > 0.0) || !std::isfinite(len)) continue;
+        SkipRec e{};
+        for (int a = 0; a < 3; ++a) e.n[a] = (float)(c[a] / len), e.p[a] = w[a];
+        int32_t at = rec_node[(size_t)first_rec[t]];
+        int32_t child = hs.nodes[(size_t)at].child[rec_slot[(size_t)first_rec[t]]];
+        double a0 = 0.0, a2 = 0.0, b0, b2;
+        bool any = false;
+        while (skip_bounds(hs, e.n, e.p, child, b0, b2) && b0 < 1.0) {
+            any = true, a0 = b0, a2 = b2;
+            e.ref = device_child_word(child);
+            if (at <= 0) break;
+            child = at, at = parent[(size_t)at];
+            if (at < 0) break;
+        }
+        if (!any) continue;
+        const uint16_t h0 = half_up(a0), h2 = half_up(a2);
+        if (h0 == 0x7C00 || h2 == 0x7C00) continue;
+        e.a = (uint32_t)h0 | ((uint32_t)h2 << 16);
+        hs.skip[t] = e;
+    }
+}
+
+
+}
diff --git a/sycl-ray-tracer_amd/csrc/scene_build.h b/sycl-ray-tracer_amd/csrc/scene_build.h
--- a/sycl-ray-tracer_amd/csrc/scene_build.h
+++ b/sycl-ray-tracer_amd/csrc/scene_build.h
@@ -16,6 +16,7 @@
     std::vector<MatRec> mats;
     std::vector<uint8_t> tex;
     std::vector<float> wverts;
+    std::vector<SkipRec> skip;
     std::vector<float> rec_lo, rec_hi;
     uint32_t n_split_triangles = 0;
     uint32_t n_layers = 0;
@@ -54,6 +55,14 @@
 double refit_sah_cost(const HostScene& hs, const std::vector<float>& box);
 double decoded_sah_cost(const HostScene& hs);
 
+inline uint32_t device_child_word(int32_t child) { return child >= 0 ? (uint32_t)child * 64u : (uint32_t)child; }
+constexpr uint32_t kSkipMaxRecords = 128;
+bool skip_bounds(const HostScene& hs, const float n[3], const float p[3], int32_t child, double& a0, double& a2);
+uint16_t half_up(double x);
+float half_value(uint16_t bits);
+void clear_skip_table(HostScene& hs);
+void build_skip_table(HostScene& hs);
+
 int check_bvh(const HostScene& hs, std::string& err);
 
 int count_visits(const HostScene& hs, uint32_t n, const float* org, const float* dir, int mode, uint64_t* node_visits, uint64_t* tri_tests, float* t_out,
diff --git a/sycl-ray-tracer_amd/csrc/scene_check.cpp b/sycl-ray-tracer_amd/csrc/scene_check.cpp
--- a/sycl-ray-tracer_amd/csrc/scene_check.cpp
+++ b/sycl-ray-tracer_amd/csrc/scene_check.cpp
@@ -2,6 +2,7 @@
 
 #include <algorithm>
 #include <cmath>
+#include <cstring>
 #include <limits>
 
 namespace rt {
@@ -65,6 +66,110 @@
             }
         }
     return 1.0 + cost;
+}
+
+uint16_t half_up(double x) {
+    if (!(x >= 0.0)) return 0x7C00;
+    if (x > 65504.0) return 0x7C00;
+    const _Float16 h = (_Float16)x;
+    uint16_t b;
+    std::memcpy(&b, &h, 2);
+    if ((double)h < x) b++;
+    return b;
+}
+float half_value(uint16_t bits) {
+    _Float16 h;
+    std::memcpy(&h, &bits, 2);
+    return (float)h;
+}
+
+namespace {
+bool records_below(const HostScene& hs, int32_t child, uint32_t depth, std::vector<uint32_t>& out) {
+    if (child == kChildEmpty) return true;
+    if (child < 0) {
+        const LeafRange leaf = leaf_range(child);
+        if ((size_t)leaf.first + leaf.count > hs.tris.size()) return false;
+        for (uint32_t k = 0; k < leaf.count; ++k) out.push_back(leaf.first + k);
+        return out.size() <= kSkipMaxRecords;
+    }
+    if ((size_t)child >= hs.nodes.size() || depth >= (uint32_t)kStackSize) return false;
+    for (int k = 0; k < 4; ++k)
+        if (!records_below(hs, hs.nodes[(size_t)child].child[k], depth + 1, out)) return false;
+    return true;
+}
+}
+
+bool skip_bounds(const HostScene& hs, const float nf[3], const float pf[3], int32_t child, double& a0, double& a2) {
+    std::vector<uint32_t> recs;
+    if (!records_below(hs, child, 0, recs) || recs.empty()) return false;
+    const double n[3] = {nf[0], nf[1], nf[2]}, p[3] = {pf[0], pf[1], pf[2]};
+    const double nn = std::sqrt(n[0] * n[0] + n[1] * n[1] + n[2] * n[2]);
+    if (!(std::fabs(nn - 1.0) <= 1e-6)) return false;
+    double dev = 0.0, reach = 0.0, kappa = 1.0;
+    for (uint32_t r : recs) {
+        const TriRec& tr = hs.tris[r];
+        const double e1[3] = {tr.e1[0], tr.e1[1], tr.e1[2]}, e2[3] = {tr.e2[0], tr.e2[1], tr.e2[2]};
+        const double c[3] = {e1[1] * e2[2] - e1[2] * e2[1], e1[2] * e2[0] - e1[0] * e2[2], e1[0] * e2[1] - e1[1] * e2[0]};
+        const double area2 = std::sqrt(c[0] * c[0] + c[1] * c[1] + c[2] * c[2]);
+        const double l1 = std::sqrt(e1[0] * e1[0] + e1[1] * e1[1] + e1[2] * e1[2]), l2 = std::sqrt(e2[0] * e2[0] + e2[1] * e2[1] + e2[2] * e2[2]);
+        if (!(area2 >= 1e-24) || !std::isfinite(area2)) return false;
+        kappa = std::max(kappa, l1 * l2 / area2);
+        double plus = 0.0, minus = 0.0;
+        for (int a = 0; a < 3; ++a) plus += (c[a] / area2 - n[a]) * (c[a] / area2 - n[a]), minus += (c[a] / area2 + n[a]) * (c[a] / area2 + n[a]);
+        if (!(std::sqrt(std::min(plus, minus)) <= 0.9 / 1024.0)) return false;
+        for (int v = 0; v < 3; ++v) {
+            double s = 0.0, d2 = 0.0;
+            for (int a = 0; a < 3; ++a) {
+                const double x = (double)tr.v0[a] + (v == 1 ? e1[a] : (v == 2 ? e2[a] : 0.0)) - p[a];
+                s += n[a] * x, d2 += x * x;
+            }
+            dev = std::max(dev, std::fabs(s)), reach = std::max(reach, std::sqrt(d2));
+        }
+    }
+    if (!(kappa <= 256.0) || !std::isfinite(dev) || !std::isfinite(reach)) return false;
+    const double u = std::ldexp(1.0, -24), tn = (double)kTNear;
+    a0 = std::max(1.01 * (4.0 * dev + 2.0 * 16.0 * u * kappa * reach / 0.75) / tn, std::ldexp(1.0, -20));
+    a2 = 1.01 * (4.0 * 4.1 * u + 2.0 * 16.0 * u * kappa / 0.75) / tn;
+    return true;
+}
+
+namespace {
+bool check_skip_table(const HostScene& hs, std::string& err) {
+    const size_t T = hs.wverts.size() / 9;
+    if (hs.skip.empty()) return true;
+    if (hs.skip.size() != T) { err = "origin-skip table: one entry per triangle expected"; return false; }
+    std::vector<uint8_t> is_word;
+    is_word.assign(hs.nodes.size(), 0);
+    for (const BvhNode& n : hs.nodes)
+        for (int k = 0; k < 4; ++k)
+            if (n.child[k] >= 0 && (size_t)n.child[k] < hs.nodes.size()) is_word[(size_t)n.child[k]] = 1;
+    for (size_t t = 0; t < T; ++t) {
+        const SkipRec& e = hs.skip[t];
+        if (e.ref == kSkipNone) continue;
+        const std::string at = "origin-skip entry of triangle " + std::to_string(t);
+        int32_t child;
+        if ((int32_t)e.ref < 0) {
+            child = (int32_t)e.ref;
+        } else {
+            if (e.ref % 64u || e.ref / 64u >= hs.nodes.size() || !is_word[e.ref / 64u]) { err = at + ": not a child word"; return false; }
+            child = (int32_t)(e.ref / 64u);
+        }
+        std::vector<uint32_t> recs;
+        if (!records_below(hs, child, 0, recs)) { err = at + ": names no subtree of at most " + std::to_string(kSkipMaxRecords) + " records"; return false; }
+        bool member = false;
+        for (uint32_t r : recs) member = member || hs.tris[r].global_index == t;
+        if (!member) { err = at + ": the triangle is not in the subtree"; return false; }
+        const float* w = &hs.wverts[9 * t];
+        if (e.p[0] != w[0] || e.p[1] != w[1] || e.p[2] != w[2]) { err = at + ": p is not the triangle's first vertex"; return false; }
+        double a0, a2;
+        if (!skip_bounds(hs, e.n, e.p, child, a0, a2)) { err = at + ": the subtree is not coplanar with the triangle"; return false; }
+        if (!((double)half_value((uint16_t)(e.a & 0xffffu)) >= a0) || !((double)half_value((uint16_t)(e.a >> 16)) >= a2) || !(a0 < 1.0)) {
+            err = at + ": thresholds below what the subtree's flatness proves";
+            return false;
+        }
+    }
+    return true;
+}
 }
 
 int check_bvh(const HostScene& hs, std::string& err) {
@@ -129,12 +234,20 @@
                 }
         }
     }
+    if (!check_skip_table(hs, err)) return RT_ERR_INVALID;
     return RT_OK;
 }
 
 int count_visits(const HostScene& hs, uint32_t n, const float* org, const float* dir, int mode, uint64_t* node_visits, uint64_t* tri_tests, float* t_out,
                  uint32_t* tri_out, std::string& err) {
-    if (mode < 0 || mode > 2) { err = "mode: 0 quantised, 1 exact, 2 quantised with two more bits"; return RT_ERR_INVALID; }
+    if (mode != 4 && (mode < 0 || mode > 2)) { err = "mode: 0 quantised, 1 exact, 2 quantised with two more bits, 4 quantised with the origin skip"; return RT_ERR_INVALID; }
+    const bool skipping = mode == 4;
+    if (skipping) {
+        mode = 0;
+        if (!tri_out) { err = "mode 4: tri holds the triangle every ray starts on"; return RT_ERR_INVALID; }
+        for (uint32_t i = 0; i < n; ++i)
+            if (tri_out[i] != kNoTri && tri_out[i] >= hs.skip.size()) { err = "mode 4: start triangle out of range"; return RT_ERR_INVALID; }
+    }
     if (hs.nodes.empty()) { err = "no tree"; return RT_ERR_INVALID; }
     const float inf = std::numeric_limits<float>::infinity();
     std::vector<Box3> box(hs.nodes.size() * 4);
@@ -162,6 +275,8 @@
         for (int a = 0; a < 3; ++a) inv[a] = 1.0f / (std::fabs(d[a]) < 1e-30f ? std::copysign(1e-30f, d[a]) : d[a]);
         float best = inf;
         uint32_t best_tri = kNoTri;
+        uint32_t skip = kSkipNone;
+        if (skipping && tri_out[i] != kNoTri) skip = origin_skip_word(hs.skip[tri_out[i]], o, d);
         int32_t stack[kStackSize * 4];
         int sp = 0;
         int32_t cur = 0;
@@ -173,7 +288,7 @@
                 int32_t ch[4];
                 int m = 0;
                 for (int k = 0; k < 4; ++k) {
-                    if (nd.child[k] == kChildEmpty) continue;
+                    if (nd.child[k] == kChildEmpty || device_child_word(nd.child[k]) == skip) continue;
                     const Box3& b = box[(size_t)cur * 4 + k];
                     float tn = 0.0f, tf = best;
                     for (int a = 0; a < 3; ++a) {
diff --git a/sycl-ray-tracer_amd/rtamd/abi.py b/sycl-ray-tracer_amd/rtamd/abi.py
--- a/sycl-ray-tracer_amd/rtamd/abi.py
+++ b/sycl-ray-tracer_amd/rtamd/abi.py
@@ -431,6 +431,7 @@
                                       _P(C.c_uint32)]),
     "rt_dev_scene_tree": (C.c_int, [C.c_void_p, _P(C.c_uint32), _P(C.c_uint32), _P(C.c_uint32), _P(C.c_uint32), _P(C.c_int32), _P(C.c_float),
                                     _P(C.c_float), C.c_void_p, _P(C.c_uint32), _P(C.c_float), C.c_uint32]),
+    "rt_dev_scene_skip_table": (C.c_int, [C.c_void_p, _P(C.c_uint32), _P(C.c_uint32), C.c_uint32, C.c_int]),
     "rt_dev_renderer_graph_captures": (C.c_int, [C.c_void_p, _P(C.c_uint32)]),
     "rt_dev_quantise_node": (C.c_int, [C.c_uint32, _P(C.c_int32), _P(C.c_float), _P(C.c_float), C.c_void_p, _P(C.c_uint8)]),
 }
```

After: 10470, median of 6. 1.07x the previous value.
